# DearCaat/MHIM-MIL

Measured on AMD Instinct MI355X. Metric: patch-instances/sec through MHIM fwd+bwd, N=10k D=1024, higher is better.
Workload: dtype f32; 1 GPU; c2: MHIM(ABMIL) train step, one bag N=10000 D=1024 per GPU per step (teacher fwd + select + student fwd + bwd + Adam + EMA); rotating_bags_per_gpu=8, matrix_core_form=bf16x3, parallelism=dp1, launch=hipGraph replay, one graph per resident bag

## Files before the change

mhim_mil_amd/csrc/optim.hip:

```cpp
#include <math.h>
#include <stdlib.h>

#include "common.hpp"

namespace mhimx {

int reduce_flush(hipStream_t st, mhimx_reduce_list* list);

constexpr int HEAD_THREADS = 256;

MHIMX_DEV float blk_sum(float v, float* red) {
  v = wave_sum(v);
  __syncthreads();
  if ((threadIdx.x & 63) == 0) red[threadIdx.x >> 6] = v;
  __syncthreads();
  return red[0] + red[1] + red[2] + red[3];
}
MHIMX_DEV float blk_max(float v, float* red) {
  v = wave_max(v);
  __syncthreads();
  if ((threadIdx.x & 63) == 0) red[threadIdx.x >> 6] = v;
  __syncthreads();
  return fmaxf(fmaxf(red[0], red[1]), fmaxf(red[2], red[3]));
}

__global__ __launch_bounds__(HEAD_THREADS) void head_kernel(const float* __restrict__ z, const float* __restrict__ t,
                                                            const float* __restrict__ wp, const float* __restrict__ bp,
                                                            const int64_t* __restrict__ label, int E, int C, float temp_t,
                                                            float main_alpha, float aux_alpha, float inv_accum,
                                                            float* __restrict__ logits, float* __restrict__ losses,
                                                            float* __restrict__ g_z, float* __restrict__ d_wp,
                                                            float* __restrict__ d_bp, int accumulate,
                                                            const float* __restrict__ g_logits_in,
                                                            const float* __restrict__ g_cl_in) {
  __shared__ float red[4];
  __shared__ float lg[16], gl[16];
  const int tid = threadIdx.x;
  for (int c = 0; c < C; ++c) {
    float p = 0.f;
    for (int e = tid; e < E; e += HEAD_THREADS) p += wp[c * E + e] * z[e];
    p = blk_sum(p, red);
    if (tid == 0) lg[c] = p + (bp ? bp[c] : 0.f);
// ... 35 lines not shown
    losses[0] = main_alpha * ce + aux_alpha * cl;
    losses[1] = ce;
    losses[2] = cl;
  }
  for (int e = tid; e < E; e += HEAD_THREADS) {
    float g = 0.f;
    for (int c = 0; c < C; ++c) g += wp[c * E + e] * gl[c];
    if (aux) g += aux_alpha * inv_accum * (expf(z[e] - zmx) / zden - expf(t[e] / temp_t - tmx) / tden);
    g_z[e] = g;
    if (d_wp)
      for (int c = 0; c < C; ++c) {
        const float v = gl[c] * z[e];
        d_wp[c * E + e] = accumulate ? d_wp[c * E + e] + v : v;
      }
  }
  if (d_bp && tid < C) d_bp[tid] = accumulate ? d_bp[tid] + gl[tid] : gl[tid];
}

template <int Q>
__global__ __launch_bounds__(HEAD_THREADS) void head_fast_kernel(const float* __restrict__ z, const float* __restrict__ t,
                                                                 const float* __restrict__ wp, const float* __restrict__ bp,
                                                                 const int64_t* __restrict__ label, int E, int C, float temp_t,
                                                                 float main_alpha, float aux_alpha, float inv_accum,
                                                                 float* __restrict__ logits, float* __restrict__ losses,
                                                                 float* __restrict__ g_z, float* __restrict__ d_wp,
                                                                 float* __restrict__ d_bp, int accumulate,
                                                                 const float* __restrict__ g_logits_in,
                                                                 const float* __restrict__ g_cl_in, BagBatch bb) {
  __shared__ float red[8][4];
  if (blockIdx.z) {
    MHIMX_BAG(z); MHIMX_BAG(t); MHIMX_BAG(label); MHIMX_BAG(logits); MHIMX_BAG(losses); MHIMX_BAG(g_z); MHIMX_BAG(d_wp); MHIMX_BAG(d_bp);
    MHIMX_BAG(g_logits_in); MHIMX_BAG(g_cl_in);
  }
  const int tid = threadIdx.x, lane = tid & 63, wave = tid >> 6;
  const bool aux = (t != nullptr);
  float zv[Q], tv[Q], wv[4][Q], dw_old[4][Q];
#pragma unroll
  for (int q = 0; q < Q; ++q) {
    const int e = tid + q * HEAD_THREADS;
    const bool in = e < E;
    zv[q] = in ? z[e] : 0.f;
    tv[q] = (in && aux) ? t[e] : 0.f;
#pragma unroll
    for (int c = 0; c < 4; ++c) {
      wv[c][q] = (in && c < C) ? wp[c * E + e] : 0.f;
      dw_old[c][q] = (in && c < C && d_wp && accumulate) ? d_wp[c * E + e] : 0.f;
    }
  }
  const int y = label ? (int)label[0] : 0;
  float bpv[4], glin[4], dbp_old[4];
#pragma unroll
  for (int c = 0; c < 4; ++c) {
    bpv[c] = (bp && c < C) ? bp[c] : 0.f;
    glin[c] = (!label && g_logits_in && c < C) ? g_logits_in[c] : 0.f;
    dbp_old[c] = (d_bp && accumulate && c < C) ? d_bp[c] : 0.f;
  }
  if (g_cl_in) aux_alpha = g_cl_in[0];
  float p[4] = {0.f, 0.f, 0.f, 0.f}, a = -INFINITY, b = -INFINITY;
#pragma unroll
  for (int q = 0; q < Q; ++q) {
    const bool in = tid + q * HEAD_THREADS < E;
#pragma unroll
    for (int c = 0; c < 4; ++c) p[c] += wv[c][q] * zv[q];
    if (in) { a = fmaxf(a, zv[q]); b = fmaxf(b, tv[q] / temp_t); }
  }
#pragma unroll
  for (int c = 0; c < 4; ++c) p[c] = wave_sum(p[c]);
  a = wave_max(a);
  b = wave_max(b);
  if (lane == 0) {
#pragma unroll
    for (int c = 0; c < 4; ++c) red[c][wave] = p[c];
    red[4][wave] = a;
    red[5][wave] = b;
  }
  __syncthreads();
  float lg[4];
#pragma unroll
  for (int c = 0; c < 4; ++c) lg[c] = (red[c][0] + red[c][1] + red[c][2] + red[c][3]) + bpv[c];
  const float zmx = aux ? fmaxf(fmaxf(red[4][0], red[4][1]), fmaxf(red[4][2], red[4][3])) : 0.f;
  const float tmx = aux ? fmaxf(fmaxf(red[5][0], red[5][1]), fmaxf(red[5][2], red[5][3])) : 0.f;
  float ce = 0.f, gl[4] = {0.f, 0.f, 0.f, 0.f};
  if (label) {
    float mx = -INFINITY;
#pragma unroll
    for (int c = 0; c < 4; ++c) if (c < C) mx = fmaxf(mx, lg[c]);
    float den = 0.f;
#pragma unroll
    for (int c = 0; c < 4; ++c) if (c < C) den += expf(lg[c] - mx);
    float ly = lg[0];
#pragma unroll
    for (int c = 1; c < 4; ++c) if (c == y) ly = lg[c];
    ce = -(ly - mx - logf(den));
#pragma unroll
    for (int c = 0; c < 4; ++c) if (c < C) gl[c] = main_alpha * inv_accum * (expf(lg[c] - mx) / den - (c == y ? 1.f : 0.f));
  } else {
#pragma unroll
    for (int c = 0; c < 4; ++c) gl[c] = glin[c];
  }
  float cl = 0.f, zden = 1.f, tden = 1.f;
  float ez[Q], et[Q];
  if (aux) {
    float sa = 0.f, sb = 0.f;
#pragma unroll
    for (int q = 0; q < Q; ++q) {
      const bool in = tid + q * HEAD_THREADS < E;
      ez[q] = in ? expf(zv[q] - zmx) : 0.f;
      et[q] = in ? expf(tv[q] / temp_t - tmx) : 0.f;
      sa += ez[q];
      sb += et[q];
    }
    sa = wave_sum(sa);
    sb = wave_sum(sb);
    if (lane == 0) { red[6][wave] = sa; red[7][wave] = sb; }
    __syncthreads();
    zden = red[6][0] + red[6][1] + red[6][2] + red[6][3];
    tden = red[7][0] + red[7][1] + red[7][2] + red[7][3];
    const float lz = logf(zden);
    float acc = 0.f;
#pragma unroll
    for (int q = 0; q < Q; ++q)
      if (tid + q * HEAD_THREADS < E) acc += (et[q] / tden) * (zv[q] - zmx - lz);
    acc = wave_sum(acc);
    if (lane == 0) red[0][wave] = acc;
    __syncthreads();
    cl = -(red[0][0] + red[0][1] + red[0][2] + red[0][3]);
  }
  if (tid == 0) {
    for (int c = 0; c < C; ++c) logits[c] = lg[c];
    losses[0] = main_alpha * ce + aux_alpha * cl;
    losses[1] = ce;
    losses[2] = cl;
  }
#pragma unroll
  for (int q = 0; q < Q; ++q) {
    const int e = tid + q * HEAD_THREADS;
    if (e >= E) continue;
    float g = 0.f;
#pragma unroll
    for (int c = 0; c < 4; ++c) if (c < C) g += wv[c][q] * gl[c];
    if (aux) g += aux_alpha * inv_accum * (ez[q] / zden - et[q] / tden);
    g_z[e] = g;
    if (d_wp) {
#pragma unroll
      for (int c = 0; c < 4; ++c)
        if (c < C) {
          const float v = gl[c] * zv[q];
          d_wp[c * E + e] = accumulate ? dw_old[c][q] + v : v;
        }
    }
  }
  if (d_bp && tid < C) {
    float gv = gl[0], ov = dbp_old[0];
#pragma unroll
    for (int c = 1; c < 4; ++c) if (c == tid) { gv = gl[c]; ov = dbp_old[c]; }
    d_bp[tid] = accumulate ? ov + gv : gv;
  }
}

__global__ __launch_bounds__(HEAD_THREADS) void dsmil_head_kernel(const float* __restrict__ lb, const float* __restrict__ li,
                                                                  const int64_t* __restrict__ label, const float* __restrict__ Bs,
                                                                  const float* __restrict__ Bt, int C, int V, float temp_t,
                                                                  float main_alpha, float aux_alpha, float inv_accum,
                                                                  float* __restrict__ losses, float* __restrict__ g_lb,
                                                                  float* __restrict__ g_li, float* __restrict__ g_B,
                                                                  const float* __restrict__ g_cl_in) {
  __shared__ float red[4];
  const int tid = threadIdx.x;
  float ce = 0.f;
  if (label) {
    float mx = -INFINITY;
    for (int c = 0; c < C; ++c) mx = fmaxf(mx, 0.5f * (lb[c] + li[c]));
    float den = 0.f;
    for (int c = 0; c < C; ++c) den += expf(0.5f * (lb[c] + li[c]) - mx);
    const int y = (int)label[0];
    ce = -(0.5f * (lb[y] + li[y]) - mx - logf(den));
    if (tid < C) {
      const float g = 0.5f * main_alpha * inv_accum * (expf(0.5f * (lb[tid] + li[tid]) - mx) / den - (tid == y ? 1.f : 0.f));
      g_lb[tid] = g;
      g_li[tid] = g;
    }
  }
  if (g_cl_in) aux_alpha = g_cl_in[0];
  float cl = 0.f;
  if (Bt) {
    for (int c = 0; c < C; ++c) {
      const float* s = Bs + (int64_t)c * V;
      const float* t = Bt + (int64_t)c * V;
      float a = -INFINITY, b = -INFINITY;
      for (int e = tid; e < V; e += HEAD_THREADS) { a = fmaxf(a, s[e]); b = fmaxf(b, t[e] / temp_t); }
      const float smx = blk_max(a, red), tmx = blk_max(b, red);
      float sa = 0.f, sb = 0.f;
      for (int e = tid; e < V; e += HEAD_THREADS) { sa += expf(s[e] - smx); sb += expf(t[e] / temp_t - tmx); }
      const float sden = blk_sum(sa, red), tden = blk_sum(sb, red);
      const float ls = logf(sden);
      float acc = 0.f;
      for (int e = tid; e < V; e += HEAD_THREADS) {
        const float pt = expf(t[e] / temp_t - tmx) / tden;
        acc += pt * (s[e] - smx - ls);
        if (g_B) g_B[(int64_t)c * V + e] = aux_alpha * inv_accum / (float)C * (expf(s[e] - smx) / sden - pt);
      }
      cl -= blk_sum(acc, red) / (float)C;
    }
  } else if (g_B) {
    for (int i = tid; i < C * V; i += HEAD_THREADS) g_B[i] = 0.f;
  }
  if (tid == 0) {
    losses[0] = main_alpha * ce + aux_alpha * cl;
    losses[1] = ce;
    losses[2] = cl;
  }
}

constexpr int FOLD_MAX = 4;
struct FoldJobs { const float* parts[FOLD_MAX]; int64_t off[FOLD_MAX], n[FOLD_MAX]; int G[FOLD_MAX], accumulate[FOLD_MAX]; int count; };
struct OptimExtra { const float* lr_table; int64_t lr_len; const float* g_extra; int64_t n_extra, extra_pitch; float clip_norm;
                    const float* sq_parts; int n_parts; FoldJobs fold; int64_t extra_lo; int extra_only; };

MHIMX_DEV float4 fold_sum4(const float* __restrict__ parts, int64_t n, int64_t idx, int G) {
  float4 s0 = make_float4(0.f, 0.f, 0.f, 0.f), s1 = s0, s2 = s0, s3 = s0;
  auto ld = [&](int z) { return *reinterpret_cast<const float4*>(parts + (int64_t)z * n + idx); };
  auto add = [](float4& a, const float4& b) { a.x += b.x; a.y += b.y; a.z += b.z; a.w += b.w; };
  int z = 0;
  for (; z + 8 <= G; z += 8) {
    const float4 p0 = ld(z), p1 = ld(z + 1), p2 = ld(z + 2), p3 = ld(z + 3), p4 = ld(z + 4), p5 = ld(z + 5), p6 = ld(z + 6), p7 = ld(z + 7);
    add(s0, p0); add(s1, p1); add(s2, p2); add(s3, p3);
    add(s0, p4); add(s1, p5); add(s2, p6); add(s3, p7);
  }
  for (; z + 4 <= G; z += 4) { add(s0, ld(z)); add(s1, ld(z + 1)); add(s2, ld(z + 2)); add(s3, ld(z + 3)); }
  for (; z < G; ++z) add(s0, ld(z));
  return make_float4((s0.x + s1.x) + (s2.x + s3.x), (s0.y + s1.y) + (s2.y + s3.y), (s0.z + s1.z) + (s2.z + s3.z), (s0.w + s1.w) + (s2.w + s3.w));
}

__global__ __launch_bounds__(256) void grad_sumsq_kernel(const float* __restrict__ g, int64_t n, float gscale, OptimExtra ex, float* __restrict__ parts) {
  __shared__ float red[256];
  float a = 0.f;
  for (int64_t i = (int64_t)blockIdx.x * 256 + threadIdx.x; i < n; i += (int64_t)gridDim.x * 256) {
    const bool slabs = i >= ex.extra_lo;
    float v = (slabs && ex.extra_only) ? 0.f : g[i];
    if (slabs)
      for (int64_t z = 0; z < ex.n_extra; ++z) v += ex.g_extra[z * ex.extra_pitch + i];
    v *= gscale;
    a += v * v;
  }
  red[threadIdx.x] = a;
  __syncthreads();
  for (int o = 128; o > 0; o >>= 1) {
    if ((int)threadIdx.x < o) red[threadIdx.x] += red[threadIdx.x + o];
    __syncthreads();
  }
// ... 26 lines not shown
    }
  }
  if (threadIdx.x == 0) {
    int64_t step = step_host;
    if (step_dev) step = (int64_t)step_dev[0];
    if (ex.lr_table) {
      int64_t i = step - 1;
      i = i < 0 ? 0 : (i >= ex.lr_len ? ex.lr_len - 1 : i);
      lr = ex.lr_table[i];
    }
    if (step_dev || ex.lr_table) {
      const double t = (double)step;
      lr_over_bc1 = (float)((double)lr / (1.0 - exp(t * ln_beta1)));
      bc2s = (float)sqrt(1.0 - exp(t * ln_beta2));
    }
    float coef = 1.f;
    if (ex.clip_norm > 0.f) {
      coef = ex.clip_norm / (sqrtf(clip_red[0]) + 1e-6f);
      coef = coef > 1.f ? 1.f : coef;
    }
    sc[3] = coef;
    if (mm_table) {
      int64_t i = step - 1;
      i = i < 0 ? 0 : (i >= mm_len ? mm_len - 1 : i);
      mm = mm_table[i];
    }
    sc[0] = lr_over_bc1; sc[1] = bc2s; sc[2] = mm;
  }
  __syncthreads();
  lr_over_bc1 = sc[0];
  bc2s = sc[1];
  mm = sc[2];
  gscale *= sc[3];
  const int64_t n4 = n_all / 4;
  const bool vec_ok = ((reinterpret_cast<uintptr_t>(p) | reinterpret_cast<uintptr_t>(g) | reinterpret_cast<uintptr_t>(m) |
                        reinterpret_cast<uintptr_t>(v) | reinterpret_cast<uintptr_t>(teacher)) & 15) == 0;
  for (int64_t q = (int64_t)blockIdx.x * blockDim.x + threadIdx.x; q * 4 < n_all; q += (int64_t)gridDim.x * blockDim.x) {
    const int64_t i0 = q * 4;
    if (vec_ok && q < n4 && (i0 + 4 <= n_train || i0 >= n_train)) {
      float4 w = reinterpret_cast<float4*>(p)[q];
      if (i0 < n_train) {
        const bool slabs = i0 >= ex.extra_lo;
        float4 gi = (slabs && ex.extra_only) ? make_float4(0.f, 0.f, 0.f, 0.f) : reinterpret_cast<float4*>(g)[q];
        float4 mi = reinterpret_cast<float4*>(m)[q], vi = reinterpret_cast<float4*>(v)[q];
        for (int f = 0; f < ex.fold.count; ++f)
          if (i0 >= ex.fold.off[f] && i0 < ex.fold.off[f] + ex.fold.n[f]) {
            const float4 sv = fold_sum4(ex.fold.parts[f], ex.fold.n[f], i0 - ex.fold.off[f], ex.fold.G[f]);
            if (ex.fold.accumulate[f]) { gi.x += sv.x; gi.y += sv.y; gi.z += sv.z; gi.w += sv.w; }
            else gi = sv;
          }
        for (int64_t z = 0; slabs && z < ex.n_extra; ++z) {
          const float4 e = *reinterpret_cast<const float4*>(ex.g_extra + z * ex.extra_pitch + i0);
          gi.x += e.x; gi.y += e.y; gi.z += e.z; gi.w += e.w;
        }
        adam_one(w.x, gi.x, mi.x, vi.x, lr_over_bc1, bc2s, beta1, beta2, eps, wd, gscale);
        adam_one(w.y, gi.y, mi.y, vi.y, lr_over_bc1, bc2s, beta1, beta2, eps, wd, gscale);
        adam_one(w.z, gi.z, mi.z, vi.z, lr_over_bc1, bc2s, beta1, beta2, eps, wd, gscale);
        adam_one(w.w, gi.w, mi.w, vi.w, lr_over_bc1, bc2s, beta1, beta2, eps, wd, gscale);
        reinterpret_cast<float4*>(m)[q] = mi;
        reinterpret_cast<float4*>(v)[q] = vi;
        reinterpret_cast<float4*>(p)[q] = w;
        if (zero_grad) reinterpret_cast<float4*>(g)[q] = make_float4(0.f, 0.f, 0.f, 0.f);
      }
      if (teacher) {
        float4 t = reinterpret_cast<float4*>(teacher)[q];
        t.x = t.x * mm + w.x * (1.f - mm); t.y = t.y * mm + w.y * (1.f - mm);
        t.z = t.z * mm + w.z * (1.f - mm); t.w = t.w * mm + w.w * (1.f - mm);
        reinterpret_cast<float4*>(teacher)[q] = t;
      }
      continue;
    }
    for (int64_t i = i0; i < i0 + 4 && i < n_all; ++i) {
      float w = p[i];
      if (i < n_train) {
        const bool slabs = i >= ex.extra_lo;
        float gi = (slabs && ex.extra_only) ? 0.f : g[i], mi = m[i], vi = v[i];
        for (int64_t z = 0; slabs && z < ex.n_extra; ++z) gi += ex.g_extra[z * ex.extra_pitch + i];
        adam_one(w, gi, mi, vi, lr_over_bc1, bc2s, beta1, beta2, eps, wd, gscale);
        m[i] = mi;
        v[i] = vi;
        p[i] = w;
        if (zero_grad) g[i] = 0.f;
      }
      if (teacher) teacher[i] = teacher[i] * mm + w * (1.f - mm);
    }
  }
}

}

using namespace mhimx;

extern "C" int mhimx_head_fwd_bwd(void* stream, const float* z, const float* t, const float* wp, const float* bp,
                                  const int64_t* label_dev, int64_t E, int64_t C, float temp_t, float main_alpha,
                                  float aux_alpha, float inv_accum, float* logits, float* losses, float* g_z, float* d_wp,
                                  float* d_bp, int32_t accumulate, const float* g_logits_in, const float* g_cl_in) {
  MHIMX_CHECK_ARG(z && wp && logits && losses && g_z, "head: null args");
  MHIMX_CHECK_ARG(C > 0 && C <= 16 && E > 0, "head: bad dims");
  static const bool slow_head = getenv("MHIMX_HEAD_GENERIC") != nullptr;
  if (!slow_head && C <= 4 && E <= 2 * HEAD_THREADS)
    hipLaunchKernelGGL(head_fast_kernel<2>, bgrid(1), dim3(HEAD_THREADS), 0, (hipStream_t)stream, z, t, wp, bp, label_dev, (int)E, (int)C,
                     temp_t, main_alpha, aux_alpha, inv_accum, logits, losses, g_z, d_wp, d_bp, accumulate, g_logits_in, g_cl_in, cur_batch());
  else if (!slow_head && C <= 4 && E <= 4 * HEAD_THREADS)
    hipLaunchKernelGGL(head_fast_kernel<4>, bgrid(1), dim3(HEAD_THREADS), 0, (hipStream_t)stream, z, t, wp, bp, label_dev, (int)E, (int)C,
                     temp_t, main_alpha, aux_alpha, inv_accum, logits, losses, g_z, d_wp, d_bp, accumulate, g_logits_in, g_cl_in, cur_batch());
  else if (cur_batch().n > 0)
    return fail(-1, "head: a bag-batched launch takes the short-chain head (C <= 4, E <= 1024)");
  else
  hipLaunchKernelGGL(head_kernel, dim3(1), dim3(HEAD_THREADS), 0, (hipStream_t)stream, z, t, wp, bp, label_dev, (int)E, (int)C,
                     temp_t, main_alpha, aux_alpha, inv_accum, logits, losses, g_z, d_wp, d_bp, accumulate, g_logits_in, g_cl_in);
  MHIMX_LAUNCH_CHECK();
  return 0;
}

extern "C" int mhimx_dsmil_head(void* stream, const float* logits_bag, const float* logits_ins, const int64_t* label_dev,
                                const float* Bs, const float* Bt, int64_t C, int64_t V, float temp_t, float main_alpha,
                                float aux_alpha, float inv_accum, float* losses, float* g_logits_bag, float* g_logits_ins,
                                float* g_B, const float* g_cl_in) {
  MHIMX_CHECK_ARG(losses && Bs && C > 0 && C <= 16 && V > 0, "dsmil_head: bad args");
  MHIMX_CHECK_ARG(!label_dev || (logits_bag && logits_ins && g_logits_bag && g_logits_ins), "dsmil_head: label needs the logits and their gradients");
  hipLaunchKernelGGL(dsmil_head_kernel, dim3(1), dim3(HEAD_THREADS), 0, (hipStream_t)stream, logits_bag, logits_ins, label_dev, Bs, Bt,
                     (int)C, (int)V, temp_t, main_alpha, aux_alpha, inv_accum, losses, g_logits_bag, g_logits_ins, g_B, g_cl_in);
  MHIMX_LAUNCH_CHECK();
  return 0;
}

extern "C" int mhimx_optim_step(void* stream, const mhimx_optim_args* a) {
  MHIMX_CHECK_ARG(a, "optim_step: null args");
  MHIMX_CHECK_ARG(!a->mm_table || a->mm_len > 0, "optim_step: empty momentum schedule");
  MHIMX_CHECK_ARG(!a->lr_table || a->lr_len > 0, "optim_step: empty learning-rate schedule");
  MHIMX_CHECK_ARG(a->p && a->g && a->m && a->v && a->n_train >= 0 && a->n_all >= a->n_train && (a->step >= 1 || a->step_dev), "optim_step: bad args");
  MHIMX_CHECK_ARG(a->n_extra >= 0 && (a->n_extra == 0 || (a->g_extra && a->extra_pitch >= a->n_train && a->extra_pitch % 4 == 0 && aligned16(a->g_extra))),
                  "optim_step: gradient slabs need a 16-byte aligned base and a pitch >= n_train that is a multiple of 4");
  MHIMX_CHECK_ARG(!(a->clip_norm > 0.f) || (a->ws && a->ws_floats >= 1024), "optim_step: clipping needs a workspace of 1024 floats");
  MHIMX_CHECK_ARG(a->extra_lo >= 0 && a->extra_lo % 4 == 0 && (a->n_extra > 0 || (a->extra_lo == 0 && !a->extra_only)),
                  "optim_step: extra_lo (a multiple of 4) / extra_only describe the gradient slabs of g_extra");
  int64_t step = a->step < 1 ? 1 : a->step;
  if (a->n_all == 0) return 0;
  OptimExtra ex{a->lr_table, a->lr_len, a->g_extra, a->n_extra, a->extra_pitch, a->clip_norm > 0.f ? a->clip_norm : 0.f, a->ws, 0, {}, a->extra_lo, a->extra_only};
  if (a->fold) {
    mhimx_reduce_list* l = a->fold;
    MHIMX_CHECK_ARG(l->n >= 0 && l->n <= MHIMX_REDUCE_MAX, "optim_step: bad reduction list");
    const bool vec_ok = aligned16(a->p) && aligned16(a->g) && aligned16(a->m) && aligned16(a->v) && (!a->teacher || aligned16(a->teacher));
    if (!(a->clip_norm > 0.f) && vec_ok) {
      int kept = 0;
      for (int i = 0; i < l->n; ++i) {
        const mhimx_reduce_job& j = l->j[i];
        const int64_t n = j.K1 * j.K2, off = j.out - a->g;
        const bool take = j.kind == 1 && ex.fold.count < FOLD_MAX && j.G >= 1 && j.G <= 64 && j.ldo == j.K2 && n > 0 && n % 4 == 0 && aligned16(j.parts) &&
                          j.out >= a->g && off % 4 == 0 && off + n <= a->n_train / 4 * 4;
        if (take) {
          const int f = ex.fold.count++;
          ex.fold.parts[f] = j.parts; ex.fold.off[f] = off; ex.fold.n[f] = n; ex.fold.G[f] = (int)j.G; ex.fold.accumulate[f] = j.accumulate;
        } else {
          l->j[kept++] = j;
        }
      }
      l->n = kept;
    }
    if (l->n > 0 || l->side.pending || l->parked.pending)
      if (int r = reduce_flush((hipStream_t)stream, l)) return r;
  }
  if (ex.clip_norm > 0.f && a->n_train > 0) {
    const int64_t nb = cdiv(a->n_train, 1024) < 1024 ? cdiv(a->n_train, 1024) : 1024;
    ex.n_parts = (int)nb;
    hipLaunchKernelGGL(grad_sumsq_kernel, dim3((unsigned)nb), dim3(256), 0, (hipStream_t)stream, a->g, a->n_train, a->grad_scale, ex, a->ws);
    MHIMX_LAUNCH_CHECK();
  } else {
    ex.clip_norm = 0.f;
  }
  const double bc1 = 1.0 - pow((double)a->beta1, (double)step);
  const double bc2 = 1.0 - pow((double)a->beta2, (double)step);
  const int64_t blocks = cdiv(a->n_all, 1024) < 2048 ? cdiv(a->n_all, 1024) : 2048;
  hipLaunchKernelGGL(adam_ema_kernel, dim3((unsigned)blocks), dim3(256), 0, (hipStream_t)stream, a->p, a->g, a->m, a->v,
                     a->teacher, a->n_train, a->n_all, (float)((double)a->lr / bc1), (float)sqrt(bc2), a->beta1, a->beta2, a->eps, a->weight_decay,
                     a->grad_scale, a->ema_mm, a->zero_grad, a->step_dev, a->lr, a->mm_table, a->mm_len, step, log((double)a->beta1),
                     log((double)a->beta2), ex);
  MHIMX_LAUNCH_CHECK();
  return 0;
}

extern "C" int mhimx_adam_ema(void* stream, float* p, const float* g, float* m, float* v, float* teacher, int64_t n_train,
                              int64_t n_all, int64_t step, float lr, float beta1, float beta2, float eps, float weight_decay,
                              float grad_scale, float ema_mm, int32_t zero_grad, const uint64_t* step_dev,
                              const float* mm_table, int64_t mm_len) {
  mhimx_optim_args a{};
  a.p = p; a.g = const_cast<float*>(g); a.m = m; a.v = v; a.teacher = teacher; a.n_train = n_train; a.n_all = n_all; a.step = step;
  a.step_dev = step_dev; a.lr = lr; a.beta1 = beta1; a.beta2 = beta2; a.eps = eps; a.weight_decay = weight_decay; a.grad_scale = grad_scale;
  a.ema_mm = ema_mm; a.mm_table = mm_table; a.mm_len = mm_len; a.zero_grad = zero_grad;
  return mhimx_optim_step(stream, &a);
}

typedef float sc_f4 __attribute__((ext_vector_type(4)));
__global__ __launch_bounds__(256) void stream_copy_kernel(const sc_f4* __restrict__ src, sc_f4* __restrict__ dst, int64_t n4) {
  const int64_t stride = (int64_t)gridDim.x * 256;
  for (int64_t i = (int64_t)blockIdx.x * 256 + threadIdx.x; i < n4; i += stride) __builtin_nontemporal_store(__builtin_nontemporal_load(src + i), dst + i);
}
extern "C" int mhimx_stream_copy(void* stream, const float* src, float* dst, int64_t n_floats) {
  MHIMX_CHECK_ARG(src && dst && n_floats >= 0 && n_floats % 4 == 0 && aligned16(src) && aligned16(dst), "stream_copy: 16-byte aligned buffers, n % 4 == 0");
  if (n_floats == 0) return 0;
  const int64_t n4 = n_floats / 4;
  const int64_t blocks = cdiv(n4, 256) < (1 << 20) ? cdiv(n4, 256) : (1 << 20);
  hipLaunchKernelGGL(stream_copy_kernel, dim3((unsigned)blocks), dim3(256), 0, (hipStream_t)stream, reinterpret_cast<const sc_f4*>(src),
                     reinterpret_cast<sc_f4*>(dst), n4);
  MHIMX_LAUNCH_CHECK();
  return 0;
}

__global__ void tick_kernel(uint64_t* c) { c[0] += 1; }
extern "C" int mhimx_tick(void* stream, uint64_t* counter) {
  MHIMX_CHECK_ARG(counter, "tick: null counter");
  hipLaunchKernelGGL(tick_kernel, dim3(1), dim3(1), 0, (hipStream_t)stream, counter);
  MHIMX_LAUNCH_CHECK();
  return 0;
// ... 2 lines not shown
```

mhim_mil_amd/csrc/prep_jobs.hpp:

```cpp
#pragma once
#include "mma_tile.hpp"
#include "mca2_prep.hpp"

namespace mhimx {

typedef float pj_f4 __attribute__((ext_vector_type(4)));
typedef __bf16 pj_b8 __attribute__((ext_vector_type(8)));
MHIMX_DEV void pj_split(const float (&x)[8], pj_b8& hi, pj_b8& lo) {
#pragma unroll
  for (int i = 0; i < 8; ++i) {
    const __bf16 h = (__bf16)x[i];
    hi[i] = h;
    lo[i] = (__bf16)(x[i] - (float)h);
  }
}
MHIMX_DEV void pj_split2(const pj_f4& a, const pj_f4& b, pj_b8& hi, pj_b8& lo) {
  const float x[8] = {a[0], a[1], a[2], a[3], b[0], b[1], b[2], b[3]};
  pj_split(x, hi, lo);
}

constexpr int PREP_MERGE_MAX = 8;
struct PrepJobs { mhimx_prep_job j[MHIMX_PREP_MAX]; int first[MHIMX_PREP_MAX + 1]; int n; Merge2PrepArgs m2; int64_t m2_shift[PREP_MERGE_MAX]; };
constexpr int PREP_LDS_FLOATS = 6 * M2_E + 6 * 64;
static_assert(PREP_LDS_FLOATS >= 32 * 33, "the transpose tile fits the job LDS");

MHIMX_DEV void prep_job_block(const PrepJobs& pj, int block, float* lds) {
  int q = 0;
  while (q + 1 < pj.n && block >= pj.first[q + 1]) ++q;
  const mhimx_prep_job jb = pj.j[q];
  const int bid = block - pj.first[q], nblk = pj.first[q + 1] - pj.first[q];
  const int64_t R = jb.R, C = jb.C;
  if (jb.kind == 0) {
    float (*tile)[33] = reinterpret_cast<float(*)[33]>(lds);
    const int tx = threadIdx.x & 31, ty = threadIdx.x >> 5;
    const int64_t tiles_c = (C + 31) / 32, ntiles = ((R + 31) / 32) * tiles_c;
    for (int64_t t = bid; t < ntiles; t += nblk) {
      const int64_t r0 = (t / tiles_c) * 32, c0 = (t % tiles_c) * 32;
      for (int i = ty; i < 32; i += 8) {
        const int64_t r = r0 + i, c = c0 + tx;
        tile[i][tx] = (r < R && c < C) ? jb.in[r * C + c] : 0.f;
      }
      __syncthreads();
      for (int i = ty; i < 32; i += 8) {
        const int64_t c = c0 + i, r = r0 + tx;
        if (r < R && c < C) jb.out[c * R + r] = tile[tx][i];
      }
      __syncthreads();
    }
  } else if (jb.kind == 1) {
    const int64_t K8 = C / 8, n = R * K8;
    for (int64_t i = (int64_t)bid * 256 + threadIdx.x; i < n; i += (int64_t)nblk * 256) {
// ... 106 lines not shown
```

mhim_mil_amd/csrc/rows.hip:

```cpp
#include <math.h>
#include <string.h>

#include "mca2_rows.hpp"
#include "reduce_jobs.hpp"

namespace mhimx {

int gemm_nt(hipStream_t st, const mhimx_gemm_nt_args& g);
int gemm_tn(hipStream_t st, const mhimx_gemm_tn_args& g);
bool scorer_fused_ok(int64_t E, int64_t A, int gated, int prec, const float* T, const float* wa, const float* wp, int64_t C);
int scorer_fused_fwd(hipStream_t st, const float* T, int64_t M, const float* wa, const float* wa_frag, const float* ba, int act, const float* wc,
                     const float* bc, const float* wp, int C, float* u_pre, float* s_out, float* cproj, float* pm, float* pl,
                     float* pz, int max_parts, const int64_t* rows, const uint8_t* excl, const mhimx_prep_job* ride_jobs, int n_ride_jobs,
                     const void* merge_rows);
int merge2_fwd_rows_args(const mhimx_merge* m, const float* X, int64_t R, void* ws, int64_t ws_bytes, M2RowsFwd* out);
int prep_batch(hipStream_t st, const mhimx_prep_job* jobs, int n);
int scorer_fused_bwd(hipStream_t st, const float* T, int64_t M, const float* u_pre, const float* s_in, const float* stats,
                     const float* g_z, const float* z, const float* wc, int act, const float* wa_t, const float* wa_t_frag, float* du,
                     float* dT, float* dwc_part, float* dbc_part, int max_parts, const int64_t* rows, const void* pre_side, int64_t gate_row0,
                     void* img, const void* img_dact, float* img_part, int64_t img_rows);

constexpr int ROWS_THREADS = 256;
constexpr int MAX_PART = 512;
constexpr int TN_SLABS = 128;

MHIMX_DEV float sigmoidf_(float x) { return 1.f / (1.f + __expf(-x)); }

constexpr int FWD_WAVES = 16;
template <int EPL>
__global__ __launch_bounds__(64 * FWD_WAVES) void score_rows_fwd_kernel(
    const float* __restrict__ T, int64_t M, int E, int A, int act, int gated, const float* __restrict__ u_pre,
    const float* __restrict__ wc, const float* __restrict__ bc, const float* __restrict__ wp, int C,
    float* __restrict__ s_out, float* __restrict__ cproj, float* __restrict__ pm, float* __restrict__ pl,
    float* __restrict__ pz, float gdrop_p, uint64_t gdrop_seed, int64_t row0 ) {
  extern __shared__ __attribute__((aligned(16))) float sm[];
  constexpr int NWV = FWD_WAVES;
  const int lane = threadIdx.x & 63, wave = threadIdx.x >> 6;
  const int ldu = A * (1 + gated);
  const float bias_c = bc ? bc[0] : 0.f;

  float mw = -INFINITY, lw = 0.f, zacc[EPL];
#pragma unroll
  for (int q = 0; q < EPL; ++q) zacc[q] = 0.f;

  for (int64_t n = (int64_t)blockIdx.x * NWV + wave; n < M; n += (int64_t)gridDim.x * NWV) {
    const float* up = u_pre + n * ldu;
    float part = 0.f;
    const bool gdrop = gated && gdrop_p > 0.f;
    const uint32_t rkey = gdrop ? drop_row_key(gdrop_seed, (uint64_t)(row0 + n)) : 0u;
    const float ginv = gdrop ? 1.f / (1.f - gdrop_p) : 1.f;
    for (int j = lane; j < A; j += 64) {
      float u = act_fwd(up[j], act);
      if (gated) {
// ... 32 lines not shown
      lw += p;
#pragma unroll
      for (int q = 0; q < EPL; ++q) zacc[q] += p * hv[q];
    }
  }
  float* zs = sm;
  float* ms = sm + NWV * E;
  float* ls = ms + NWV;
#pragma unroll
  for (int q = 0; q < EPL; ++q) zs[wave * E + lane + 64 * q] = zacc[q];
  if (lane == 0) { ms[wave] = mw; ls[wave] = lw; }
  __syncthreads();
  float mb = ms[0];
#pragma unroll
  for (int i = 1; i < NWV; ++i) mb = fmaxf(mb, ms[i]);
  float w[NWV];
#pragma unroll
  for (int i = 0; i < NWV; ++i) w[i] = (ms[i] == -INFINITY) ? 0.f : __expf(ms[i] - mb);
  for (int e = threadIdx.x; e < E; e += 64 * NWV) {
    float a = 0.f;
#pragma unroll
    for (int i = 0; i < NWV; ++i) a += zs[i * E + e] * w[i];
    pz[(int64_t)blockIdx.x * E + e] = a;
  }
  if (threadIdx.x == 0) {
    float l = 0.f;
#pragma unroll
    for (int i = 0; i < NWV; ++i) l += ls[i] * w[i];
    pm[blockIdx.x] = mb;
    pl[blockIdx.x] = l;
  }
}

constexpr int FIN_THREADS = 1024;
__global__ __launch_bounds__(FIN_THREADS) void pool_finalize_kernel(const float* __restrict__ pm, const float* __restrict__ pl,
                                                                     const float* __restrict__ pz, int G, int E,
                                                                     float* __restrict__ stats, float* __restrict__ z,
                                                                     const float* __restrict__ s, const float* __restrict__ cproj,
                                                                     const float* __restrict__ bp, int C, int64_t M1,
                                                                     float* __restrict__ pscore, BagBatch bb) {
  __shared__ float red[16];
  __shared__ float wgt[2 * MAX_PART];
  __shared__ float acc16[16][64];
  if (blockIdx.z) {
    MHIMX_BAG(pm); MHIMX_BAG(pl); MHIMX_BAG(pz); MHIMX_BAG(stats); MHIMX_BAG(z); MHIMX_BAG(s); MHIMX_BAG(cproj); MHIMX_BAG(pscore);
  }
  const int lane = threadIdx.x & 63, wave = threadIdx.x >> 6;
  const int b1 = threadIdx.x;
  const float pm1 = b1 < G ? pm[b1] : -INFINITY, pl1 = b1 < G ? pl[b1] : 0.f;
  float m = wave_max(pm1);
  if (lane == 0) red[wave] = m;
  __syncthreads();
  float mx = red[0];
#pragma unroll
  for (int w = 1; w < 16; ++w) mx = fmaxf(mx, red[w]);
  __syncthreads();
  float lp = 0.f;
  if (b1 < G) {
    const float w = (pm1 == -INFINITY) ? 0.f : __expf(pm1 - mx);
    wgt[b1] = w;
    lp = pl1 * w;
  }
  lp = wave_sum(lp);
  if (lane == 0) red[wave] = lp;
  __syncthreads();
  float L = 0.f;
#pragma unroll
  for (int w = 0; w < 16; ++w) L += red[w];
  const int zblocks = (E + 63) / 64;
  if ((int)blockIdx.x >= zblocks) {
    const float invL = 1.f / L, b0 = bp ? bp[0] : 0.f;
    const int nb = (int)gridDim.x - zblocks;
    for (int64_t n = (int64_t)((int)blockIdx.x - zblocks) * FIN_THREADS + threadIdx.x; n < M1; n += (int64_t)nb * FIN_THREADS) {
      const float an = __expf(s[n] - mx) * invL;
      float cm = -INFINITY;
      for (int c = 0; c < C; ++c) cm = fmaxf(cm, an * cproj[n * C + c] + b0);
      float den = 0.f;
      for (int c = 0; c < C; ++c) den += expf((an * cproj[n * C + c] + b0) - cm);
      pscore[n] = 1.f / den;
    }
    return;
  }
  const int e = blockIdx.x * 64 + lane;
  float acc = 0.f;
  if (e < E) {
#pragma unroll 8
    for (int b = wave; b < G; b += 16) acc += pz[(int64_t)b * E + e] * wgt[b];
  }
  acc16[wave][lane] = acc;
  __syncthreads();
  if (wave == 0 && e < E) {
    float a = 0.f;
#pragma unroll
    for (int w = 0; w < 16; ++w) a += acc16[w][lane];
    z[e] = a / L;
  }
  if (blockIdx.x == 0 && threadIdx.x == 0) { stats[0] = mx; stats[1] = L; }
}

constexpr int FIN_MAXTOK = 6;
#ifdef MHIMX_FT_PROF
__device__ unsigned long long ft_prof[16];
#define FT_STAMP(i) do { __syncthreads(); if (threadIdx.x == 0 && blockIdx.x == 0) ft_prof[i] = wall_clock64(); } while (0)
#else
#define FT_STAMP(i)
#endif
__global__ __launch_bounds__(FIN_THREADS) void pool_finalize_tok_kernel(const float* __restrict__ pm, const float* __restrict__ pl,
                                                                         const float* __restrict__ pz, int G, int E, float* __restrict__ stats,
                                                                         float* __restrict__ z, const float* __restrict__ T,
                                                                         const int64_t* __restrict__ rows_tail, int64_t row0, int K,
                                                                         const float* __restrict__ wa, const float* __restrict__ wa_t,
                                                                         const float* __restrict__ ba, const float* __restrict__ wc,
                                                                         const float* __restrict__ bc, int A, int act,
                                                                         float* __restrict__ u_pre_tail, float* __restrict__ s_tail, BagBatch bb) {
  if (blockIdx.z) {
    MHIMX_BAG(pm); MHIMX_BAG(pl); MHIMX_BAG(pz); MHIMX_BAG(stats); MHIMX_BAG(z); MHIMX_BAG(T); MHIMX_BAG(rows_tail); MHIMX_BAG(wa_t); MHIMX_BAG(u_pre_tail);
    MHIMX_BAG(s_tail);
  }
  __shared__ float red[16];
  __shared__ float wgt[2 * MAX_PART];
  __shared__ float acc16[16][64];
  __shared__ __attribute__((aligned(16))) float tks[FIN_MAXTOK][512];
  __shared__ float up[8][FIN_MAXTOK][128];
  __shared__ float us[FIN_MAXTOK][128];
  __shared__ float stok[8];
  const int tid = threadIdx.x, lane = tid & 63, wave = tid >> 6;
  FT_STAMP(0);
  const float pm1 = tid < G ? pm[tid] : -INFINITY, pl1 = tid < G ? pl[tid] : 0.f;
  const int e = blockIdx.x * 64 + lane;
  float pzv[8];
// ... 642 lines not shown
  const int64_t G = 2 * MAX_PART;
  PoolWs t;
  t.pm = ar.take<float>(G);
  t.pl = ar.take<float>(G);
  t.pz = ar.take<float>(G * E);
  t.attn = ar.take<float>(M);
  t.du = ar.take<float>(M * A * (1 + gated));
  t.dwc_part = ar.take<float>(G * A);
  t.dbc_part = ar.take<float>(G);
  t.u_pre = ar.take<float>(M * A * (1 + gated));
  t.tn_ws = ar.take<float>((int64_t)TN_SLABS * A * E);
  t.nt_ws = ar.take<float>(4 * M * A);
  if (w) *w = t;
  return ar.off;
}

template <typename F>
static int dispatch_epl(int64_t E, F&& f) {
  switch (E) {
    case 256: return f(std::integral_constant<int, 4>());
    case 512: return f(std::integral_constant<int, 8>());
    case 1024: return f(std::integral_constant<int, 16>());
    default: return fail(-1, "token width E=%lld unsupported (256, 512 or 1024)", (long long)E);
  }
}

static int check_scorer(const mhimx_scorer* sc) {
  MHIMX_CHECK_ARG(sc && sc->wa && sc->wc, "scorer: null weights");
  MHIMX_CHECK_ARG(sc->A > 0 && sc->A <= 512 && sc->A % 4 == 0, "scorer: A must be a multiple of 4, <= 512");
  MHIMX_CHECK_ARG(!sc->gated || sc->wb, "scorer: gated needs wb");
  return 0;
}

int abmil_pool_fwd(hipStream_t st, const mhimx_scorer* sc, mhimx_pool_io* io) {
  if (int r = check_scorer(sc)) return r;
  MHIMX_CHECK_ARG(io && io->T1 && io->M1 > 0 && io->s && io->stats && io->z, "pool_fwd: null io");
  MHIMX_CHECK_ARG(io->M2 == 0 || io->T2, "pool_fwd: M2>0 needs T2");
  MHIMX_CHECK_ARG(!io->cproj || (io->wp && io->C > 0), "pool_fwd: cproj needs wp, C");
  MHIMX_CHECK_ARG(!io->rows1 || (io->M2 == 0 && scorer_fused_ok(sc->E, sc->A, sc->gated, sc->prec, io->T1, sc->wa, io->cproj ? io->wp : nullptr, io->C)),
                  "pool_fwd: gathered tokens (rows1) need the one-pass scorer (E = 512, A = 128, plain form, not f32) and a single segment");
  MHIMX_CHECK_ARG(!io->excl || scorer_fused_ok(sc->E, sc->A, sc->gated, sc->prec, io->T1, sc->wa, io->cproj ? io->wp : nullptr, io->C),
                  "pool_fwd: excluded rows (excl) need the one-pass scorer (E = 512, A = 128, plain form, not f32)");
  const int64_t M = io->M1 + io->M2, E = sc->E, A = sc->A;
  const int gated = sc->gated ? 1 : 0;
  Arena ar(io->ws, io->ws_bytes);
  PoolWs w;
  pool_ws_layout(ar, M, E, A, gated, &w);
  MHIMX_CHECK_ARG(ar.ok(), "pool_fwd: workspace too small (%lld < %lld)", (long long)io->ws_bytes, (long long)ar.off);
  float* u_pre = io->u_pre ? io->u_pre : w.u_pre;
  const int64_t ldu = A * (1 + gated);
  if (io->phase != 0) {
    const int64_t K = io->tail_tokens, Ms1 = io->M1 - K;
    MHIMX_CHECK_ARG((io->phase == 1 || io->phase == 2) && K >= 1 && K <= FIN_MAXTOK && Ms1 >= 1 && io->M2 == 0 && !io->cproj && !io->pscore && !io->excl &&
                        E == 512 && A == 128 && scorer_fused_ok(E, A, gated, sc->prec, io->T1, sc->wa, nullptr, 0),
                    "pool_fwd: the two-call forward takes the one-pass scorer shapes, one segment, 1..%d tail tokens, no class projections", FIN_MAXTOK);
    const int tiles = (int)cdiv(Ms1, 32);
    const int G1 = tiles < MAX_PART ? tiles : MAX_PART;
    if (io->phase == 1) {
      M2RowsFwd mfbuf;
      const void* mf = nullptr;
      io->rode_merge = 0;
      static const bool ride_ok = getenv("MHIMX_MERGE_FWD_RIDE") == nullptr || atoi(getenv("MHIMX_MERGE_FWD_RIDE")) != 0;
      if (io->ride_merge && ride_ok) {
        const int rc = merge2_fwd_rows_args(reinterpret_cast<const mhimx_merge*>(io->ride_merge), io->ride_X, io->ride_R, io->ride_ws, io->ride_ws_bytes,
                                            &mfbuf);
        if (rc < 0) return rc;
        if (rc == 0) { mf = &mfbuf; io->rode_merge = 1; }
      }
      const int g1 = scorer_fused_fwd(st, io->T1, Ms1, sc->wa, sc->wa_frag, sc->ba, sc->act, sc->wc, sc->bc, nullptr, 0, u_pre, io->s, nullptr, w.pm, w.pl,
                                      w.pz, MAX_PART, io->rows1, nullptr, io->ride_jobs, io->n_ride_jobs, mf);
      return g1 < 0 ? g1 : 0;
    }
    hipLaunchKernelGGL(pool_finalize_tok_kernel, bgrid((unsigned)cdiv(E, 64)), dim3(FIN_THREADS), 0, st, w.pm, w.pl, w.pz, G1, (int)E, io->stats, io->z, io->T1,
                       (io->rows1 && io->tail_row0 < 0) ? io->rows1 + Ms1 : nullptr, io->rows1 ? io->tail_row0 : Ms1, (int)K, sc->wa, io->tail_wa_t, sc->ba, sc->wc,
                       sc->bc, (int)A, sc->act, u_pre + Ms1 * ldu, io->s + Ms1, cur_batch());
    MHIMX_LAUNCH_CHECK();
    return 0;
  }

  const float* Ts[2] = {io->T1, io->T2};
  const int64_t Ms[2] = {io->M1, io->M2};
  int64_t off = 0;
  int G = 0;
  bool rode = false;
  for (int seg = 0; seg < 2; ++seg) {
    if (Ms[seg] == 0) continue;
    if (scorer_fused_ok(E, A, gated, sc->prec, Ts[seg], sc->wa, io->cproj ? io->wp : nullptr, io->C)) {
      const int g1 = scorer_fused_fwd(st, Ts[seg], Ms[seg], sc->wa, sc->wa_frag, sc->ba, sc->act, sc->wc, sc->bc, io->cproj ? io->wp : nullptr,
                                      (int)io->C, io->no_backward ? nullptr : u_pre + off * ldu, io->s + off, io->cproj ? io->cproj + off * io->C : nullptr,
                                      w.pm + G, w.pl + G, w.pz + (int64_t)G * E, MAX_PART, seg == 0 ? io->rows1 : nullptr,
                                      seg == 0 ? io->excl : nullptr, rode ? nullptr : io->ride_jobs, rode ? 0 : io->n_ride_jobs, nullptr);
      if (g1 < 0) return g1;
      rode = true;
      G += g1;
      off += Ms[seg];
      continue;
    }
    MHIMX_CHECK_ARG(cur_batch().n == 0, "pool_fwd: a bag-batched launch needs the one-pass scorer");
    mhimx_gemm_nt_args g = {};
    g.A = Ts[seg]; g.lda = E; g.B = sc->wa; g.ldb = E; g.C = u_pre + off * ldu; g.ldc = ldu;
    g.M = Ms[seg]; g.N = A; g.K = E; g.bias = sc->ba;
    g.ws = w.nt_ws; g.ws_floats = 4 * M * A;
    g.prec = sc->prec == MHIMX_PREC_F32 ? MHIMX_PREC_F32 : MHIMX_PREC_BF16X3;
    if (int r = gemm_nt(st, g)) return r;
    if (gated) {
      g.B = sc->wb; g.bias = sc->bb; g.C = u_pre + off * ldu + A;
      if (int r = gemm_nt(st, g)) return r;
    }
    int grid = (int)cdiv(Ms[seg], 5 * FWD_WAVES);
    if (grid < 1) grid = 1;
    if (grid > MAX_PART) grid = MAX_PART;
    const float* Tseg = Ts[seg];
    const int64_t Mseg = Ms[seg];
    int r = dispatch_epl(E, [&](auto epl) {
      constexpr int EPL = decltype(epl)::value;
      const size_t smem = (size_t)(FWD_WAVES * E + 2 * FWD_WAVES) * sizeof(float);
      if (smem > 48 * 1024)
        MHIMX_ONCE_PER_DEVICE(MHIMX_HIP(hipFuncSetAttribute((const void*)score_rows_fwd_kernel<EPL>, hipFuncAttributeMaxDynamicSharedMemorySize, (int)smem)));
      hipLaunchKernelGGL(score_rows_fwd_kernel<EPL>, dim3(grid), dim3(64 * FWD_WAVES), smem, st, Tseg, Mseg, (int)E, (int)A,
                         sc->act, gated, u_pre + off * ldu, sc->wc, sc->bc, io->cproj ? io->wp : nullptr, (int)io->C,
                         io->s + off, io->cproj ? io->cproj + off * io->C : nullptr, w.pm + G, w.pl + G,
                         w.pz + (int64_t)G * E, sc->gate_drop_p, sc->gate_drop_seed, off);
      MHIMX_LAUNCH_CHECK();
      return 0;
    });
    if (r) return r;
    G += grid;
    off += Ms[seg];
  }
  if (!rode && io->ride_jobs && io->n_ride_jobs > 0)
    if (int r = prep_batch(st, io->ride_jobs, io->n_ride_jobs)) return r;
  MHIMX_CHECK_ARG(!io->pscore || io->cproj, "pool_fwd: pscore needs cproj (and wp)");
  static_assert(2 * MAX_PART <= FIN_THREADS, "pool_finalize_kernel reads one partial per thread");
  const int64_t ps_blocks = io->pscore ? (cdiv(io->M1, FIN_THREADS) < 64 ? cdiv(io->M1, FIN_THREADS) : 64) : 0;
  hipLaunchKernelGGL(pool_finalize_kernel, bgrid((unsigned)(cdiv(E, 64) + ps_blocks)), dim3(FIN_THREADS), 0, st, w.pm, w.pl, w.pz, G, (int)E, io->stats,
                     io->z, io->s, io->cproj, io->bp, (int)io->C, io->M1, io->pscore, cur_batch());
  MHIMX_LAUNCH_CHECK();
  return 0;
}

int abmil_pool_bwd(hipStream_t st, const mhimx_scorer* sc, const mhimx_pool_io* io, const mhimx_pool_grad* gr) {
  if (int r = check_scorer(sc)) return r;
  MHIMX_CHECK_ARG(io && gr && gr->g_z && gr->dT1 && gr->d_wa && gr->d_wc && gr->wa_t, "pool_bwd: null args");
  MHIMX_CHECK_ARG(io->M2 == 0 || gr->dT2, "pool_bwd: M2>0 needs dT2");
  const int64_t M = io->M1 + io->M2, E = sc->E, A = sc->A;
  const int gated = sc->gated ? 1 : 0;
  MHIMX_CHECK_ARG(!gated || (gr->d_wb && gr->wb_t), "pool_bwd: gated needs d_wb, wb_t");
  Arena ar(io->ws, io->ws_bytes);
  PoolWs w;
  pool_ws_layout(ar, M, E, A, gated, &w);
  MHIMX_CHECK_ARG(ar.ok(), "pool_bwd: workspace too small");
  const float* u_pre = io->u_pre ? io->u_pre : w.u_pre;
  const int64_t ldu = A * (1 + gated);
  const float* Ts[2] = {io->T1, io->T2};
  float* dTs[2] = {gr->dT1, gr->dT2};
  const int64_t Ms[2] = {io->M1, io->M2};

  int64_t off = 0;
  int G = 0;
  const bool fused = scorer_fused_ok(E, A, gated, sc->prec, io->T1, gr->wa_t, nullptr, 0) && aligned16(gr->dT1) &&
                     (io->M2 == 0 || (aligned16(io->T2) && aligned16(gr->dT2))) && aligned16(u_pre) && aligned16(w.du);
  MHIMX_CHECK_ARG(!io->rows1 || (fused && io->M2 == 0), "pool_bwd: gathered tokens (rows1) need the one-pass backward and a single segment");
  MHIMX_CHECK_ARG(!gr->img || (fused && io->M2 == 0 && E == 512), "pool_bwd: the dPRE image (img) needs the one-pass backward and a single segment");
  MHIMX_CHECK_ARG(cur_batch().n == 0 || (fused && io->M2 == 0 && !gated && gr->defer && !gr->d_bc && !gr->d_ba && !gr->d_bb),
                  "pool_bwd: a bag-batched launch needs the one-pass backward with its reductions queued");
  for (int seg = 0; seg < 2 && fused; ++seg) {
    if (Ms[seg] == 0) continue;
    const void* pre_side = nullptr;
    int64_t gate_row0 = -1;
    if (seg == 0 && io->M2 == 0 && gr->defer && gr->defer->pre.pending == 1) {
      Merge2Side psd;
      memcpy(&psd, gr->defer->pre.blob, sizeof(psd));
      const int64_t d = psd.dz - dTs[0];
      if (psd.dz >= dTs[0] && d % E == 0) {
        pre_side = gr->defer->pre.blob;
        gate_row0 = d / E;
        gr->defer->pre.pending = 2;
      }
    }
    const int g1 = scorer_fused_bwd(st, Ts[seg], Ms[seg], u_pre + off * ldu, io->s + off, io->stats, gr->g_z, io->z, sc->wc, sc->act,
                                    gr->wa_t, gr->wa_t_frag, w.du + off * ldu, dTs[seg], w.dwc_part + (int64_t)G * A, w.dbc_part + G,
                                    MAX_PART, seg == 0 ? io->rows1 : nullptr, pre_side, gate_row0, seg == 0 ? gr->img : nullptr, gr->img_dact, gr->img_part,
                                    gr->img_rows);
    if (g1 < 0) return g1;
    G += g1;
    off += Ms[seg];
  }
  for (int seg = 0; seg < 2 && !fused; ++seg) {
    if (Ms[seg] == 0) continue;
    const int grid = grid_for_rows(Ms[seg]);
    const float* Tseg = Ts[seg];
    const int64_t Mseg = Ms[seg];
    int r = dispatch_epl(E, [&](auto epl) {
      constexpr int EPL = decltype(epl)::value;
      const size_t smem = (size_t)(4 * A + 8) * sizeof(float);
      hipLaunchKernelGGL(score_rows_bwd_kernel<EPL>, dim3(grid), dim3(ROWS_THREADS), smem, st, Tseg, Mseg, (int)E, (int)A,
                         sc->act, gated, u_pre + off * ldu, sc->wc, io->s + off, io->stats, gr->g_z, io->z,
                         w.du + off * ldu, w.attn + off, w.dwc_part + (int64_t)G * A, w.dbc_part + G, sc->gate_drop_p,
                         sc->gate_drop_seed, off);
      MHIMX_LAUNCH_CHECK();
      return 0;
    });
    if (r) return r;
    G += grid;
    off += Ms[seg];
  }
  if (!defer_push(gr->defer, reduce_job_parts(w.dwc_part, G, A, A, gr->d_wc, gr->accumulate)))
    hipLaunchKernelGGL(reduce_parts_kernel, dim3((unsigned)cdiv(A, 32)), dim3(RP_THREADS), 0, st, w.dwc_part, G, (int)A, (int)A, gr->d_wc, gr->accumulate);
  MHIMX_LAUNCH_CHECK();
  if (gr->d_bc) {
    if (!defer_push(gr->defer, reduce_job_parts(w.dbc_part, G, 1, 1, gr->d_bc, gr->accumulate)))
      hipLaunchKernelGGL(reduce_parts_kernel, dim3(1), dim3(RP_THREADS), 0, st, w.dbc_part, G, 1, 1, gr->d_bc, gr->accumulate);
    MHIMX_LAUNCH_CHECK();
  }
  off = 0;
  for (int seg = 0; seg < 2; ++seg) {
// ... 154 lines not shown
  MHIMX_LAUNCH_CHECK();
  return 0;
}

int colsum(hipStream_t st, const float* X, int64_t M, int64_t E, float* out, int accumulate, void* ws, int64_t ws_bytes) {
  MHIMX_CHECK_ARG(X && out && E > 0 && M >= 0, "colsum: bad args");
  const int64_t nrows = M > 0 ? M : 1, avail = ws ? ws_bytes / (E * 4) : 0;
  int64_t want = cdiv(nrows, 16) < 512 ? cdiv(nrows, 16) : 512;
  MHIMX_CHECK_ARG(avail >= (want < 128 ? want : 128), "colsum: workspace too small (need %lld bytes)", (long long)((want < 128 ? want : 128) * E * 4));
  if (want > avail) want = avail;
  const int64_t chunk = cdiv(M > 0 ? M : 1, want);
  const int gy = (int)cdiv(M > 0 ? M : 1, chunk);
  hipLaunchKernelGGL(colsum_part_kernel, dim3((unsigned)cdiv(E, 128), gy), dim3(128), 0, st, X, M, (int)E, chunk, (float*)ws);
  MHIMX_LAUNCH_CHECK();
  hipLaunchKernelGGL(reduce_parts_kernel, dim3((unsigned)cdiv(E, 32)), dim3(RP_THREADS), 0, st, (const float*)ws, gy, (int)E, (int)E, out, accumulate);
  MHIMX_LAUNCH_CHECK();
  return 0;
}

}

using namespace mhimx;

extern "C" int64_t mhimx_abmil_pool_ws_bytes(int64_t M, int64_t E, int64_t A, int32_t gated) {
  Arena ar(nullptr, 0);
  return pool_ws_layout(ar, M, E, A, gated ? 1 : 0, nullptr);
}
extern "C" int mhimx_abmil_pool_fwd(void* stream, const mhimx_scorer* sc, mhimx_pool_io* io) {
  return abmil_pool_fwd((hipStream_t)stream, sc, io);
}
extern "C" int mhimx_abmil_pool_bwd(void* stream, const mhimx_scorer* sc, const mhimx_pool_io* io, const mhimx_pool_grad* g) {
  return abmil_pool_bwd((hipStream_t)stream, sc, io, g);
}
extern "C" int mhimx_softmax_from_stats(void* stream, const float* s, const float* stats, float* attn, int64_t M) {
  if (M <= 0) return 0;
  hipLaunchKernelGGL(softmax_from_stats_kernel, bgrid((unsigned)(cdiv(M, 256) < 1024 ? cdiv(M, 256) : 1024)), dim3(256), 0,
                     (hipStream_t)stream, s, stats, attn, M, cur_batch());
  MHIMX_LAUNCH_CHECK();
  return 0;
}
extern "C" int mhimx_lse_merge(void* stream, const float* parts, int64_t W, int64_t E, float* stats, float* z) {
  MHIMX_CHECK_ARG(parts && stats && z && W >= 1 && E >= 1, "lse_merge: bad args");
  hipLaunchKernelGGL(lse_merge_kernel, dim3((unsigned)cdiv(E, 256)), dim3(256), 0, (hipStream_t)stream, parts, (int)W, (int)E, stats, z);
  MHIMX_LAUNCH_CHECK();
  return 0;
}
extern "C" int mhimx_pseudo_score(void* stream, const float* s, const float* stats, const float* cproj, const float* bp,
                                  float* score, float* attn_out, int64_t M, int64_t C) {
  MHIMX_CHECK_ARG((!s || stats) && cproj && score && C > 0, "pseudo_score: null args");
  if (M <= 0) return 0;
  hipLaunchKernelGGL(pseudo_score_kernel, dim3((unsigned)(cdiv(M, 256) < 1024 ? cdiv(M, 256) : 1024)), dim3(256), 0,
                     (hipStream_t)stream, s, stats, cproj, bp, score, attn_out, M, (int)C);
  MHIMX_LAUNCH_CHECK();
  return 0;
}
extern "C" int mhimx_act_bwd(void* stream, float* dH, const float* H, const float* pre, int64_t M, int64_t E, int32_t act,
                             float drop_p, uint64_t drop_seed, const uint8_t* drop_mask, const int64_t* rows, float* colsum_out,
                             int32_t accumulate, void* ws, int64_t ws_bytes, const uint64_t* drop_tick) {
  MHIMX_CHECK_ARG(dH && (H || pre), "act_bwd: null args");
  MHIMX_CHECK_ARG(act == MHIMX_ACT_NONE || act == MHIMX_ACT_RELU || pre, "act_bwd: gelu/tanh need the pre-activation");
  if (M <= 0) return 0;
  int64_t nblk = cdiv(M, 16);
  if (nblk > 1024) nblk = 1024;
  const int64_t chunk = cdiv(M, nblk);
  nblk = cdiv(M, chunk);
  MHIMX_CHECK_ARG(!colsum_out || (ws && ws_bytes >= nblk * E * 4), "act_bwd: workspace too small for the column sums (%lld bytes)",
// ... 133 lines not shown
```

mhim_mil_amd/csrc/scorer_fused.hip:

```cpp
#include <math.h>

#include "common.hpp"
#include "mca2_rows.hpp"
#include "prep_jobs.hpp"

namespace mhimx {

typedef float sf_f32x16 __attribute__((ext_vector_type(16)));
typedef float sf_f4 __attribute__((ext_vector_type(4)));
typedef __bf16 sf_b8 __attribute__((ext_vector_type(8)));

#ifdef MHIMX_SF_PROF
__device__ unsigned long long sf_prof[16];
#define SF_STAMP(i) do { __syncthreads(); if (threadIdx.x == 0 && blockIdx.x == 7) sf_prof[i] = wall_clock64(); } while (0)
#else
#define SF_STAMP(i)
#endif

constexpr int SF_ROWS = 32, SF_E = 512, SF_A = 128, SF_LD = SF_E + 4, SF_THREADS = 256;
constexpr int SF_MAXC = 4;
constexpr size_t SF_SMEM = (size_t)(SF_ROWS * SF_LD + 4 * SF_ROWS + 2 * SF_ROWS + SF_MAXC * SF_E + 2 * SF_ROWS) * sizeof(float);

MHIMX_DEV void sf_split(const sf_f4& a, const sf_f4& b, sf_b8& hi, sf_b8& lo) {
  const float x[8] = {a[0], a[1], a[2], a[3], b[0], b[1], b[2], b[3]};
#pragma unroll
  for (int i = 0; i < 8; ++i) {
    const __bf16 h = (__bf16)x[i];
    hi[i] = h;
    lo[i] = (__bf16)(x[i] - (float)h);
  }
}

MHIMX_DEV float sf_sum32(float v) {
  v += dpp_mov<0xB1, 0xf>(0.f, v);
  v += dpp_mov<0x4E, 0xf>(0.f, v);
// ... 220 lines not shown
        for (int q = 0; q < 16; ++q) {
          const sf_f4 hv = hr[8 * q], ww = w[8 * q];
          d += hv[0] * ww[0] + hv[1] * ww[1] + hv[2] * ww[2] + hv[3] * ww[3];
        }
        d += dpp_mov<0xB1, 0xf>(0.f, d);
        d += dpp_mov<0x4E, 0xf>(0.f, d);
        d += dpp_mov<0x141, 0xf>(0.f, d);
        if (seg == 0 && n < M) cproj[n * C + c] = d;
      }
    }
    __syncthreads();
    SF_STAMP(5);
  }
  if (tid == 0) { pm[bid] = m_run; pl[bid] = l_run; }
  pz[(int64_t)bid * SF_E + tid] = z0;
  pz[(int64_t)bid * SF_E + tid + SF_THREADS] = z1;
}

constexpr int SB_LD = SF_A + 4;
constexpr size_t SB_SMEM = (size_t)(SF_ROWS * SB_LD + SF_E + 3 * SF_ROWS + 2 * SF_A + 8 + 2 * SF_ROWS) * sizeof(float);
constexpr int SB_DLD = 1040;
constexpr size_t SB_SMEM_IMG = SB_SMEM + (size_t)SF_ROWS * SB_DLD;
MHIMX_DEV void sb_swap(float& a, float& b) { asm("s_nop 1\n\tv_permlane32_swap_b32 %0, %1" : "+v"(a), "+v"(b)); }

__global__ __launch_bounds__(SF_THREADS, 2) void scorer_fused_bwd_kernel(
    const float* __restrict__ T, int64_t M, const float* __restrict__ u_pre, const float* __restrict__ s_in,
    const float* __restrict__ stats, const float* __restrict__ g_z, const float* __restrict__ z, const float* __restrict__ wc, int act,
    const float* __restrict__ wat, const float* __restrict__ wat_frag, float* __restrict__ du, float* __restrict__ dT,
    float* __restrict__ dwc_part, float* __restrict__ dbc_part, int tiles,
    const int64_t* __restrict__ rows ,
    int n_main , Merge2Side pre,
    int64_t gate_row0 ,
    char* __restrict__ img ,
    const _Float16* __restrict__ dact, float* __restrict__ img_part, int64_t img_rows, BagBatch bb) {
  extern __shared__ __attribute__((aligned(16))) float sb_sm[];
  if (blockIdx.z) {
    MHIMX_BAG(T); MHIMX_BAG(u_pre); MHIMX_BAG(s_in); MHIMX_BAG(stats); MHIMX_BAG(g_z); MHIMX_BAG(z); MHIMX_BAG(du); MHIMX_BAG(dT); MHIMX_BAG(dwc_part);
    MHIMX_BAG(dbc_part); MHIMX_BAG(rows); MHIMX_BAG(wat); MHIMX_BAG(wat_frag); MHIMX_BAG(img); MHIMX_BAG(dact); MHIMX_BAG(img_part);
    bag_move(pre, bb);
  }
  if ((int)blockIdx.x >= n_main) {
    merge2_bwd_pre_body((int)blockIdx.x - n_main, sb_sm, pre.dz, pre.wo_t, pre.wkv, pre.k, pre.drop_p, pre.oseed, pre.tick, pre.d_bo, pre.accumulate,
                        pre.w, pre.rep, pre.w.gate + 1, (unsigned)pre.k);
    return;
  }
  const bool gated = gate_row0 >= 0;
  float* Ds = sb_sm;
  float* gzs = Ds + SF_ROWS * SB_LD;
  float* an_s = gzs + SF_E;
  float* gs_s = an_s + SF_ROWS;
  float* red = gs_s + SF_ROWS;
  float* dwc_s = red + SF_ROWS;
  int64_t* ridx = reinterpret_cast<int64_t*>(dwc_s + 2 * SF_A + 8);
  char* dact_s = reinterpret_cast<char*>(sb_sm) + SB_SMEM;
  const int tid = threadIdx.x, lane = tid & 63, wave = tid >> 6;
  const int r32 = lane & 31, kg = lane >> 5;
  float c0p = 0.f;
  for (int e = tid; e < SF_E; e += SF_THREADS) {
    const float g = g_z[e];
    gzs[e] = g;
    c0p += g * z[e];
  }
  c0p = wave_sum(c0p);
  if (lane == 0) red[wave] = c0p;
  __syncthreads();
  const float c0 = (red[0] + red[1]) + (red[2] + red[3]);
  const float mx = stats[0], invL = 1.f / stats[1];
  const int a_col = tid & (SF_A - 1), half = tid >> 7;
  const float wca = wc[a_col];
  float dwc_run = 0.f, dbc_run = 0.f;

  for (int tile = blockIdx.x; tile < tiles; tile += n_main) {
    const int64_t row0 = (int64_t)tile * SF_ROWS;
    if (rows) {
      if (tid < SF_ROWS) { const int64_t n = row0 + tid; ridx[tid] = rows[n < M ? n : M - 1]; }
      __syncthreads();
    }
    if (img) {
#pragma unroll
      for (int q = 0; q < SF_ROWS / 4; ++q) {
        const int r = wave + 4 * q;
        const int64_t n = row0 + r;
        const int64_t src = rows ? ridx[r] : (n < M ? n : M - 1);
        __builtin_amdgcn_global_load_lds((gptr_f)(reinterpret_cast<const char*>(dact + src * SF_E) + lane * 16), (lptr_f)(dact_s + r * SB_DLD), 16, 0, 0);
      }
    }
    float up[SF_ROWS / 2];
    {
      const int r = tid >> 3, seg = tid & 7;
      const int64_t n = row0 + r;
      const int64_t nc = n < M ? n : M - 1;
      const sf_f4* tr = reinterpret_cast<const sf_f4*>(T + (rows ? ridx[r] : nc) * SF_E) + seg;
      const sf_f4* gr = reinterpret_cast<const sf_f4*>(gzs) + seg;
      sf_f4 tv[16];
#pragma unroll
      for (int q = 0; q < 16; ++q) tv[q] = tr[8 * q];
#pragma unroll
      for (int k = 0; k < SF_ROWS / 2; ++k) {
        const int64_t nu = row0 + half + 2 * k;
// ... 191 lines not shown
  MHIMX_ONCE_PER_DEVICE(MHIMX_HIP(hipFuncSetAttribute((const void*)scorer_fused_kernel<true>, hipFuncAttributeMaxDynamicSharedMemorySize, (int)SF_SMEM)));
  MHIMX_ONCE_PER_DEVICE(MHIMX_HIP(hipFuncSetAttribute((const void*)scorer_fused_kernel<false>, hipFuncAttributeMaxDynamicSharedMemorySize, (int)SF_SMEM)));
  const int tiles = (int)cdiv(M, SF_ROWS);
  const int grid = tiles < max_parts ? tiles : max_parts;
  static_assert(SF_SMEM >= PREP_LDS_FLOATS * sizeof(float), "the riders' LDS is the scorer's");
  static_assert(SF_SMEM >= m2_fwd_smem(16), "the Merge row tiles' LDS is the scorer's");
  static_assert(SF_THREADS == 256 && SF_THREADS == M2_THREADS, "the preparation jobs and the Merge row tiles are written for 256 threads");
  PrepJobs rider = {};
  int ride_blocks = 0;
  MHIMX_CHECK_ARG(!(ride_jobs && n_ride_jobs > 0 && cur_batch().n > 0), "scorer: preparation jobs do not ride in a bag-batched launch");
  if (ride_jobs && n_ride_jobs > 0) {
    ride_blocks = prep_jobs_fill(ride_jobs, n_ride_jobs, &rider);
    if (ride_blocks < 0) return ride_blocks;
  }
  M2RowsFwd mf = {};
  int n_front = 0;
  if (merge_rows) {
    mf = *reinterpret_cast<const M2RowsFwd*>(merge_rows);
    n_front = mf.w.T;
  }
  if (wa_frag)
    hipLaunchKernelGGL(scorer_fused_kernel<true>, bgrid(n_front + grid + ride_blocks), dim3(SF_THREADS), SF_SMEM, st, T, M, wa, wa_frag, ba, act, wc, bc, wp, C, u_pre,
                       s_out, cproj, pm, pl, pz, tiles, rows, excl, grid, rider, n_front, mf, cur_batch());
  else
    hipLaunchKernelGGL(scorer_fused_kernel<false>, bgrid(n_front + grid + ride_blocks), dim3(SF_THREADS), SF_SMEM, st, T, M, wa, wa_frag, ba, act, wc, bc, wp, C, u_pre,
                       s_out, cproj, pm, pl, pz, tiles, rows, excl, grid, rider, n_front, mf, cur_batch());
  MHIMX_LAUNCH_CHECK();
  return grid;
}

int scorer_fused_bwd(hipStream_t st, const float* T, int64_t M, const float* u_pre, const float* s_in, const float* stats,
                     const float* g_z, const float* z, const float* wc, int act, const float* wa_t, const float* wa_t_frag, float* du,
                     float* dT, float* dwc_part, float* dbc_part, int max_parts, const int64_t* rows, const void* pre_side, int64_t gate_row0,
                     void* img, const void* img_dact, float* img_part, int64_t img_rows) {
    MHIMX_ONCE_PER_DEVICE(MHIMX_HIP(hipFuncSetAttribute((const void*)scorer_fused_bwd_kernel, hipFuncAttributeMaxDynamicSharedMemorySize, (int)SB_SMEM_IMG)));
  MHIMX_CHECK_ARG(!img || (img_dact && aligned16(img) && aligned16(img_dact) && img_rows >= 0 && img_rows <= M),
                  "scorer backward: the dPRE image needs the d out / d pre rows, 16-byte aligned buffers and img_rows <= M");
  const int tiles = (int)cdiv(M, SF_ROWS);
  const int grid = tiles < max_parts ? tiles : max_parts;
  static_assert(SB_SMEM >= M2_BWD_PRE_LDS * sizeof(float), "the riding Merge stage's LDS is the backward's");
  static_assert(SF_THREADS == M2_THREADS, "the riding Merge stage is written for 256 threads");
  Merge2Side pre = {};
  int ride = 0;
  if (pre_side) {
    pre = *reinterpret_cast<const Merge2Side*>(pre_side);
    ride = M2_BWD_PRE_BLOCKS;
  } else {
    gate_row0 = -1;
  }
  hipLaunchKernelGGL(scorer_fused_bwd_kernel, bgrid(grid + ride), dim3(SF_THREADS), img ? SB_SMEM_IMG : SB_SMEM, st, T, M, u_pre, s_in, stats, g_z, z, wc, act, wa_t,
                     wa_t_frag, du, dT, dwc_part, dbc_part, tiles, rows, grid, pre, gate_row0, (char*)img, (const _Float16*)img_dact, img_part, img_rows, cur_batch());
  MHIMX_LAUNCH_CHECK();
  return grid;
}

}
```

mhim_mil_amd/csrc/select.hip:

```cpp
#include "common.hpp"

namespace mhimx {

#ifdef MHIMX_SEL_PROF
__device__ unsigned long long sel_prof[32];
#define SEL_STAMP(i) do { __syncthreads(); if (threadIdx.x == 0) sel_prof[i] = wall_clock64(); } while (0)
#else
#define SEL_STAMP(i)
#endif

constexpr int SEL_THREADS = 1024;
constexpr int SEL_WAVES = SEL_THREADS / 64;

MHIMX_DEV uint32_t mono32(float f, bool largest) {
  uint32_t b = __float_as_uint(f);
  b = (b & 0x80000000u) ? ~b : (b | 0x80000000u);
  return largest ? b : ~b;
}

MHIMX_DEV uint32_t block_prefix(bool pred, uint32_t* wave_tot , uint32_t* total) {
  const int lane = threadIdx.x & 63, wave = threadIdx.x >> 6;
  const unsigned long long bal = __ballot(pred);
  const uint32_t in_wave = __popcll(bal & ((1ull << lane) - 1ull));
  if (lane == 0) wave_tot[wave] = __popcll(bal);
  __syncthreads();
  uint32_t base = 0, tot = 0;
#pragma unroll
  for (int w = 0; w < SEL_WAVES; ++w) {
    const uint32_t c = wave_tot[w];
    if (w < wave) base += c;
    tot += c;
  }
  __syncthreads();
// ... 293 lines not shown
    if (shift == 0) break;
    if (n_eq <= (uint32_t)SEL_LIST) {
      if (tid == 0) misc[4] = 0;
      __syncthreads();
#pragma unroll
      for (int j = 0; j < KPT; ++j)
        if (valid[j] && (key[j] & fixed_mask) == prefix) hist[atomicAdd(&misc[4], 1u)] = key[j];
      __syncthreads();
      for (uint32_t j = tid; j < n_eq; j += SEL_THREADS) {
        const uint32_t mine = hist[j];
        uint32_t g = 0, e = 0;
        for (uint32_t q = 0; q < n_eq; ++q) {
          const uint32_t o = hist[q];
          g += o > mine ? 1u : 0u;
          e += o == mine ? 1u : 0u;
        }
        if (g < remaining && remaining <= g + e) { misc[5] = mine; misc[6] = remaining - g; misc[7] = e; }
      }
      __syncthreads();
      prefix = misc[5];
      remaining = misc[6];
      n_eq = misc[7];
      break;
    }
    __syncthreads();
    shift = shift - SEL_DIGIT < 0 ? 0 : shift - SEL_DIGIT;
  }
  __syncthreads();
  *remaining_out = remaining;
  *n_eq_out = n_eq;
  return prefix;
}

template <int KPT, bool LEAN = false>
__global__ __launch_bounds__(SEL_THREADS) void select_small_kernel(
    const float* __restrict__ score, int N, int k, int n_sel, int largest, const int64_t* __restrict__ perm,
    const int64_t* __restrict__ other, int64_t n_other, int64_t* __restrict__ mask_ids, int64_t* __restrict__ len_keep_dev,
    int64_t* __restrict__ topk_out, int P, int use_rand, uint64_t rand_seed0, const uint64_t* __restrict__ tick, int merge_R,
    int64_t* __restrict__ rows_out,
    int64_t* __restrict__ rows_img ,
    int img_off, BagBatch bb ) {
  extern __shared__ __attribute__((aligned(16))) char smem_raw[];
  if (blockIdx.z) {
    MHIMX_BAG(score); MHIMX_BAG(perm); MHIMX_BAG(other); MHIMX_BAG(mask_ids); MHIMX_BAG(len_keep_dev); MHIMX_BAG(topk_out); MHIMX_BAG(rows_out);
    MHIMX_BAG(rows_img);
    rand_seed0 = bag_sel_seed(rand_seed0, bb);
  }
  const uint64_t rand_seed = eff_seed(rand_seed0, tick);
  uint64_t* keys = reinterpret_cast<uint64_t*>(smem_raw);
  uint64_t* sorted = keys + P;
  uint32_t* hist = reinterpret_cast<uint32_t*>(sorted + P);
  uint32_t* wave_tot = hist + SEL_COPIES * SEL_BINS;
  uint32_t* misc = wave_tot + SEL_WAVES;
  uint32_t* bitmap = misc + 8;
  uint32_t* rank = bitmap + 512;
  uint16_t* klist = reinterpret_cast<uint16_t*>(rank + P);
  uint16_t* stage = reinterpret_cast<uint16_t*>(smem_raw);
  const int tid = threadIdx.x;
  const bool lg = largest != 0;
  const int i0 = tid * KPT;

  SEL_STAMP(8);
  uint32_t key[KPT];
  bool valid[KPT];
#pragma unroll
  for (int j = 0; j < KPT; ++j) {
    valid[j] = (i0 + j) < N;
    key[j] = valid[j] ? mono32(score[i0 + j], lg) : 0u;
  }
  SEL_STAMP(0);
  for (int i = tid; i < 512; i += SEL_THREADS) bitmap[i] = 0;
  if (tid == 0) misc[2] = 0;

  uint32_t remaining, n_eq;
  const uint32_t T = radix_select_regs<KPT, false>(key, valid, (uint32_t)k, hist, wave_tot, misc, &remaining, &n_eq);

  SEL_STAMP(1);
  uint32_t eq_rank = 0;
  if (remaining != n_eq) {
    uint32_t neq = 0;
#pragma unroll
    for (int j = 0; j < KPT; ++j) neq += (valid[j] && key[j] == T) ? 1u : 0u;
    uint32_t tot;
    eq_rank = block_scan_excl(neq, wave_tot, &tot);
  }
  bool take[KPT];
  uint32_t ntake = 0;
#pragma unroll
  for (int j = 0; j < KPT; ++j) {
    bool t = valid[j] && key[j] > T;
    if (valid[j] && key[j] == T) { t = remaining == n_eq || eq_rank < remaining; ++eq_rank; }
    take[j] = t;
    ntake += t ? 1u : 0u;
  }
  {
    uint32_t tot;
    uint32_t pos = block_scan_excl(ntake, wave_tot, &tot);
#pragma unroll
    for (int j = 0; j < KPT; ++j)
      if (take[j]) keys[pos++] = ((uint64_t)key[j] << 32) | (uint64_t)(0xFFFFFFFFu - (uint32_t)(i0 + j));
  }
// ... 412 lines not shown
  hipLaunchKernelGGL(selm_hist_kernel<2>, dim3(G), dim3(SEL_THREADS), 0, st, score, N, largest, k, w);
  hipLaunchKernelGGL(selm_count_kernel, dim3(G), dim3(SEL_THREADS), 0, st, score, N, largest, k, chunk, w);
  hipLaunchKernelGGL(selm_gather_kernel, dim3(G), dim3(SEL_THREADS), 0, st, score, N, largest, chunk, w);
  (void)P;
  hipLaunchKernelGGL(selm_rank_kernel, dim3((unsigned)cdiv(k, SEL_THREADS), (unsigned)cdiv(k, SELM_SEG)), dim3(SEL_THREADS), 0, st, k, n_sel, perm, w);
  hipLaunchKernelGGL(selm_finish_kernel, dim3((unsigned)(cdiv(k, SEL_THREADS) < 16 ? 16 : cdiv(k, SEL_THREADS))), dim3(SEL_THREADS), 0, st, k, n_sel, N,
                     other, n_other, mask_ids, topk_sorted, w);
  hipLaunchKernelGGL(selm_keepcount_kernel, dim3(G), dim3(SEL_THREADS), 0, st, N, chunk, w);
  hipLaunchKernelGGL(selm_compact_kernel, dim3(G), dim3(SEL_THREADS), 0, st, N, chunk, (other != nullptr && n_other > 0) ? 1 : 0, mask_ids,
                     len_keep_dev, w);
  MHIMX_LAUNCH_CHECK();
  return 0;
}

static int select_impl(void* stream, const float* score, int64_t N, int64_t k, int64_t n_sel, int32_t largest,
                       const int64_t* perm, const int64_t* other, int64_t n_other, int64_t* mask_ids,
                       int64_t* len_keep_dev, int64_t* topk_sorted, void* ws, int64_t ws_bytes, int g_use_rand,
                       uint64_t g_rand_seed, const uint64_t* g_tick, int g_merge_R, int64_t* g_rows_out, int64_t* g_rows_img = nullptr,
                       int g_img_off = 0) {
  MHIMX_CHECK_ARG(score && (mask_ids || g_rows_out) && ws, "select_mask: null args");
  MHIMX_CHECK_ARG(!g_rows_img || (g_rows_out && N <= 16384 && next_pow2((int)k < 2 ? 2 : (int)k) <= 4096),
                  "select_rows_img: the image-order list comes from the one-workgroup select (N <= 16384, k <= 4096)");
  MHIMX_CHECK_ARG(!g_rows_out || N <= 16384, "select_rows: fused row list needs N <= 16384 (use select_mask + compose_ids)");
  MHIMX_CHECK_ARG(N > 0 && N <= (1ll << 24), "select_mask: N out of range");
  MHIMX_CHECK_ARG(k >= 1 && k <= N && k <= 16384, "select_mask: k=%lld out of range (1..min(N,16384))", (long long)k);
  MHIMX_CHECK_ARG(n_sel >= 0 && n_sel <= k, "select_mask: n_sel out of range");
  MHIMX_CHECK_ARG(ws_bytes >= N, "select_mask: workspace too small");
  const int P = next_pow2((int)k < 2 ? 2 : (int)k);
  if (N <= 16384 && P <= 4096) {
    const size_t sm = select_small_smem(P);
#define MHIMX_SEL_SMALL(KPT)                                                                                                   \
    hipLaunchKernelGGL(select_small_kernel<KPT>, bgrid(1), dim3(SEL_THREADS), sm, (hipStream_t)stream, score, (int)N, (int)k,   \
                       (int)n_sel, largest, perm, other, n_other, mask_ids, len_keep_dev, topk_sorted, P, g_use_rand,          \
                       g_rand_seed, g_tick, g_merge_R, g_rows_out, g_rows_img, g_img_off, cur_batch())
    MHIMX_ONCE_PER_DEVICE(
        MHIMX_HIP(hipFuncSetAttribute((const void*)select_small_kernel<16>, hipFuncAttributeMaxDynamicSharedMemorySize, (int)select_small_smem(4096)));
        MHIMX_HIP(hipFuncSetAttribute((const void*)select_small_kernel<10>, hipFuncAttributeMaxDynamicSharedMemorySize, (int)select_small_smem(4096)));
        MHIMX_HIP(hipFuncSetAttribute((const void*)select_small_kernel<4>, hipFuncAttributeMaxDynamicSharedMemorySize, (int)select_small_smem(4096))));
    const bool lean = g_use_rand && g_rows_out && !perm && !other && !mask_ids && !len_keep_dev && !topk_sorted && n_sel < k;
    if (lean) {
#define MHIMX_SEL_LEAN(KPT)                                                                                                    \
      hipLaunchKernelGGL((select_small_kernel<KPT, true>), bgrid(1), dim3(SEL_THREADS), sm, (hipStream_t)stream, score, (int)N, (int)k,   \
                         (int)n_sel, largest, perm, other, n_other, mask_ids, len_keep_dev, topk_sorted, P, g_use_rand,        \
                         g_rand_seed, g_tick, g_merge_R, g_rows_out, g_rows_img, g_img_off, cur_batch())
      MHIMX_ONCE_PER_DEVICE(
          MHIMX_HIP(hipFuncSetAttribute((const void*)select_small_kernel<16, true>, hipFuncAttributeMaxDynamicSharedMemorySize, (int)select_small_smem(4096)));
          MHIMX_HIP(hipFuncSetAttribute((const void*)select_small_kernel<10, true>, hipFuncAttributeMaxDynamicSharedMemorySize, (int)select_small_smem(4096)));
          MHIMX_HIP(hipFuncSetAttribute((const void*)select_small_kernel<4, true>, hipFuncAttributeMaxDynamicSharedMemorySize, (int)select_small_smem(4096))));
      if (N <= 4096) MHIMX_SEL_LEAN(4);
      else if (N <= 10240) MHIMX_SEL_LEAN(10);
      else MHIMX_SEL_LEAN(16);
#undef MHIMX_SEL_LEAN
    } else if (N <= 4096) MHIMX_SEL_SMALL(4);
    else if (N <= 10240) MHIMX_SEL_SMALL(10);
    else MHIMX_SEL_SMALL(16);
#undef MHIMX_SEL_SMALL
    MHIMX_LAUNCH_CHECK();
    return 0;
  }
  MHIMX_CHECK_ARG(cur_batch().n == 0, "select: a bag-batched launch takes the one-workgroup select (N <= 16384, k <= 4096)");
  const size_t smem = select_smem(P);
    MHIMX_ONCE_PER_DEVICE(MHIMX_HIP(hipFuncSetAttribute((const void*)select_kernel<false>, hipFuncAttributeMaxDynamicSharedMemorySize, (int)select_smem(16384))); MHIMX_HIP(hipFuncSetAttribute((const void*)select_kernel<true>, hipFuncAttributeMaxDynamicSharedMemorySize, (int)select_smem(16384))));
  MHIMX_CHECK_ARG(!g_use_rand && !g_rows_out, "select: the random-subset forms need N <= 16384 and k <= 4096");
  if (N > 16384 && ws_bytes >= mhimx_select_ws_bytes(N) && mask_ids)
    return select_multi((hipStream_t)stream, score, N, (int)k, (int)n_sel, largest, perm, other, n_other, mask_ids, len_keep_dev, topk_sorted, ws, P);
  hipLaunchKernelGGL(select_kernel<false>, dim3(1), dim3(SEL_THREADS), smem, (hipStream_t)stream, score, N, (int)k, (int)n_sel,
                     largest, perm, other, n_other, mask_ids, len_keep_dev, topk_sorted, (uint8_t*)ws, (float*)nullptr, P);
  MHIMX_LAUNCH_CHECK();
  return 0;
}

extern "C" int mhimx_select_mask(void* stream, const float* score, int64_t N, int64_t k, int64_t n_sel, int32_t largest,
                                 const int64_t* perm, const int64_t* other, int64_t n_other, int64_t* mask_ids,
                                 int64_t* len_keep_dev, int64_t* topk_sorted, void* ws, int64_t ws_bytes) {
  return select_impl(stream, score, N, k, n_sel, largest, perm, other, n_other, mask_ids, len_keep_dev, topk_sorted, ws, ws_bytes,
                     0, 0, nullptr, 0, nullptr);
}

extern "C" int mhimx_select_rows(void* stream, const float* score, int64_t N, int64_t k, int64_t n_sel, int32_t largest,
                                 uint64_t rand_seed, const uint64_t* tick, int64_t merge_R, int64_t* rows_out, int64_t* mask_ids,
                                 void* ws, int64_t ws_bytes, int32_t merge_first) {
  MHIMX_CHECK_ARG(rows_out && merge_R >= 0 && merge_R <= N - n_sel, "select_rows: bad args");
  return select_impl(stream, score, N, k, n_sel, largest, nullptr, nullptr, 0, mask_ids, nullptr, nullptr, ws, ws_bytes,
                     merge_first ? 2 : 1, rand_seed, tick, (int)merge_R, rows_out);
}

extern "C" int mhimx_select_rows_img(void* stream, const float* score, int64_t N, int64_t k, int64_t n_sel, int32_t largest, uint64_t rand_seed,
                                     const uint64_t* tick, int64_t merge_R, int64_t* rows_out, int64_t* rows_img, int64_t img_merge_off, void* ws,
                                     int64_t ws_bytes, int32_t merge_first) {
  MHIMX_CHECK_ARG(rows_out && rows_img && merge_R >= 0 && merge_R <= N - n_sel && img_merge_off >= N - n_sel - merge_R && img_merge_off % 32 == 0 &&
                      img_merge_off <= 32768,
                  "select_rows_img: bad args (the merged rows' image position is a multiple of 32 behind the rows that stay)");
  return select_impl(stream, score, N, k, n_sel, largest, nullptr, nullptr, 0, nullptr, nullptr, nullptr, ws, ws_bytes, merge_first ? 2 : 1, rand_seed, tick,
                     (int)merge_R, rows_out, rows_img, (int)img_merge_off);
}

extern "C" int mhimx_vote_scores(void* stream, const float* attn, int64_t H, int64_t N, int64_t k, int32_t largest,
                                 float* vote, void* ws, int64_t ws_bytes) {
  (void)ws; (void)ws_bytes;
  MHIMX_CHECK_ARG(attn && vote && H > 0 && N > 0 && N <= (1ll << 24), "vote_scores: bad args");
  MHIMX_CHECK_ARG(k >= 1 && k <= N && k <= 16384, "vote_scores: k out of range");
  {
    const int64_t nb = (N * 4 / 16) * 16;
    if (aligned16(vote) && nb) sel_zero((hipStream_t)stream, vote, nb);
// ... 11 lines not shown
```

mhim_mil_amd/csrc/step.hip:

```cpp
#include <math.h>
#include <stdlib.h>
#include <string.h>

#include "common.hpp"

namespace mhimx {

int64_t merge2_rows_tiles(int64_t R);

namespace {

struct DagEvents {
  hipEvent_t e[64][6];
  bool have[64] = {};
  int get(hipEvent_t** out) {
    int dev = 0;
    MHIMX_HIP(hipGetDevice(&dev));
    MHIMX_CHECK_ARG(dev >= 0 && dev < 64, "step: device index %d", dev);
    if (!have[dev]) {
      for (int i = 0; i < 6; ++i) MHIMX_HIP(hipEventCreateWithFlags(&e[dev][i], hipEventDisableTiming));
      have[dev] = true;
    }
    *out = e[dev];
    return 0;
  }
};
DagEvents g_dag_events;
constexpr int TP_RING = 256;
struct ProjTimes {
  hipEvent_t e[64][TP_RING][3];
  bool have[64] = {};
  int n[64] = {};
  int next(int* dev_out, hipEvent_t** pair) {
    int dev = 0;
    MHIMX_HIP(hipGetDevice(&dev));
    MHIMX_CHECK_ARG(dev >= 0 && dev < 64, "step: device index %d", dev);
    if (!have[dev]) {
      for (int i = 0; i < TP_RING; ++i)
        for (int j = 0; j < 3; ++j) MHIMX_HIP(hipEventCreate(&e[dev][i][j]));
      have[dev] = true;
    }
    *dev_out = dev;
    *pair = n[dev] < TP_RING ? e[dev][n[dev]] : nullptr;
    return 0;
  }
};
ProjTimes g_proj_times;
int dag_edge(hipEvent_t ev, hipStream_t from, hipStream_t to) {
  MHIMX_HIP(hipEventRecord(ev, from));
  MHIMX_HIP(hipStreamWaitEvent(to, ev, 0));
  return 0;
}

bool fuse_dpre() {
  static const bool on = getenv("MHIMX_FUSE_DPRE") == nullptr || atoi(getenv("MHIMX_FUSE_DPRE")) != 0;
  return on;
}

struct Carve {
  char* base;
  int64_t off = 0;
  explicit Carve(void* p) : base(static_cast<char*>(p)) {}
  int64_t take_off(int64_t bytes) {
    const int64_t o = off;
    off = (off + bytes + 255) / 256 * 256;
    return o;
  }
  template <typename T> T* at(int64_t o) const { return base ? reinterpret_cast<T*>(base + o) : nullptr; }
};

struct StepBufs {
  int64_t w1p_t, wa_frag_t, w1p_s, wa_frag_s, wa_t, wa_t_frag, wo_t, q_old, merge_ws, merge_ws_bytes;
  int64_t H_t, Hbuf, dact;
  int64_t s_t, stats_t, z_t, cproj_t, pscore, attn, pool_ws_t, pool_ws_t_bytes;
  int64_t rows_all, sel_ws, sel_ws_bytes, sel_perm, sel_ids, sel_rows, sel_lk;
  int64_t s_s, stats_s, z_s, pool_ws_s, pool_ws_s_bytes;
  int64_t logits, losses, g_z;
  int64_t dH, img, ws_b, ws_b_bytes, wg_ws, wg_ws_floats;
  int64_t q_scr, gslab;
  int64_t rows_img, P0, L_img;
  bool fuse_img;
  int64_t bag0, bag_stride;
  int64_t total;
};

int dpre_merge_rows(void* stream, const float* dH, const void* dact, const int64_t* rows_merge, int64_t R, int64_t E, char* img, int64_t P0, float* d_b1,
                    float* ws_b, int64_t ws_b_bytes, mhimx_reduce_list* lst) {
  const int64_t t0 = P0 / 32;
// ... 90 lines not shown
  }
  b->bag_stride = cv.off - b->bag0;
  b->total = b->bag0 + (int64_t)n_bags * b->bag_stride;
}

}

}

using namespace mhimx;

extern "C" int mhimx_step_counts_of(int64_t N, double mask_ratio_h, double mask_ratio_hr, double merge_ratio, mhimx_step_counts* out) {
  MHIMX_CHECK_ARG(out && N >= 1 && mask_ratio_h > 0.0 && mask_ratio_hr > 0.0 && merge_ratio > 0.0, "step_counts: bad arguments");
  double eff = mask_ratio_h / mask_ratio_hr, rr = mask_ratio_hr;
  if (eff > 1.0) { rr = mask_ratio_h; eff = 1.0; }
  const int64_t k = (int64_t)ceil((double)N * eff);
  const int64_t n_sel = rr < 1.0 ? (int64_t)ceil((double)k * rr) : k;
  const int64_t len_keep = N - n_sel;
  const int64_t Lk = (int64_t)((double)len_keep * merge_ratio);
  *out = mhimx_step_counts{k, n_sel, len_keep, Lk, len_keep - Lk};
  MHIMX_CHECK_ARG(k >= 1 && n_sel >= 1 && len_keep >= 1 && Lk >= 1 && len_keep - Lk >= 1, "step_counts: the recipe leaves nothing to mask, keep or merge");
  return 0;
}

extern "C" int mhimx_step_layout_of(const mhimx_step_cfg* cfg, int64_t N, const mhimx_step_counts* cnt, mhimx_step_layout* out) {
  MHIMX_CHECK_ARG(out, "step_layout: null output");
  if (int r = check_cfg(cfg, N, cnt)) return r;
  StepBufs b;
  layout(cfg, N, cnt, &b);
  *out = mhimx_step_layout{b.total, b.logits, b.losses, cfg->attn2score ? b.pscore : b.attn, b.rows_all, b.H_t, b.Hbuf, b.dact, b.z_t, b.z_s, b.g_z, b.dH};
  return 0;
}

extern "C" int mhimx_step_run(void* stream, const mhimx_step_cfg* cfg, const float* X, int64_t ldx, int64_t N, const int64_t* label_dev,
                              const mhimx_step_counts* cnt, const mhimx_step_seeds* seeds, int64_t host_step, void* ws, int64_t ws_bytes, int32_t update) {
  if (int r = check_cfg(cfg, N, cnt)) return r;
  MHIMX_CHECK_ARG(X && label_dev && seeds && ws && ldx >= cfg->D && ldx % 4 == 0 && N * ldx * 4 < ((int64_t)1 << 32) && aligned16(X),
                  "step: null bag / label / seeds / workspace, or a row pitch the weight-gradient product does not take");
  MHIMX_CHECK_ARG(!update || (cfg->p && cfg->g && cfg->m && cfg->v && cfg->n_train > 0 && cfg->n_all >= cfg->n_train), "step: update needs the flat optimiser buffers");
  StepBufs b;
  layout(cfg, N, cnt, &b);
  MHIMX_CHECK_ARG(ws_bytes >= b.total && (reinterpret_cast<uintptr_t>(ws) & 255) == 0, "step: workspace too small (%lld < %lld) or not 256-byte aligned",
                  (long long)ws_bytes, (long long)b.total);
  const mhimx_step_cfg& c = *cfg;
  const mhimx_step_params &S = c.student, &T = c.teacher;
  const int64_t D = c.D, E = c.E, A = c.A, C = c.C, k = c.k, I = 512;
  const int64_t R = cnt->R, Lk = cnt->Lk, len_keep = cnt->len_keep;
  Carve cv(ws);
  float* w1p_t = cv.at<float>(b.w1p_t);
  float* wa_frag_t = cv.at<float>(b.wa_frag_t);
  float* w1p_s = cv.at<float>(b.w1p_s);
  float* wa_frag_s = cv.at<float>(b.wa_frag_s);
  float* wa_t = cv.at<float>(b.wa_t);
  float* wa_t_frag = cv.at<float>(b.wa_t_frag);
  float* wo_t = cv.at<float>(b.wo_t);
  float* q_old = cv.at<float>(b.q_old);
  void* merge_ws = cv.at<char>(b.merge_ws);
  float* H_t = cv.at<float>(b.H_t);
  float* Hbuf = cv.at<float>(b.Hbuf);
  void* dact = cv.at<char>(b.dact);
  int64_t* rows_all = cv.at<int64_t>(b.rows_all);
  float* dH = cv.at<float>(b.dH);
  const uint64_t* tick = c.tick;
  static const bool dag_on = getenv("MHIMX_STEP_DAG") == nullptr || atoi(getenv("MHIMX_STEP_DAG")) != 0;
  static const bool dag_fwd = getenv("MHIMX_STEP_DAG_FWD") == nullptr || atoi(getenv("MHIMX_STEP_DAG_FWD")) != 0;
  static const bool dag_bwd = getenv("MHIMX_STEP_DAG_BWD") == nullptr || atoi(getenv("MHIMX_STEP_DAG_BWD")) != 0;
  const hipStream_t main_st = (hipStream_t)stream, side_st = (hipStream_t)c.side_stream;
  const bool dag = dag_on && c.side_stream != nullptr && c.side_stream != stream;
  hipEvent_t* ev = nullptr;
  if (dag)
    if (int r = g_dag_events.get(&ev)) return r;

  mhimx_merge mw_prep = {};
  mw_prep.E = E; mw_prep.k = k; mw_prep.heads = 8; mw_prep.dim_head = 64;
  mw_prep.q_param = S.q; mw_prep.ln_w = S.ln_w; mw_prep.ln_b = S.ln_b; mw_prep.wkv = S.wkv; mw_prep.wq = S.wq; mw_prep.wo = S.wo; mw_prep.bo = S.bo;
  mw_prep.mm = c.merge_mm; mw_prep.prec = MHIMX_PREC_BF16X3; mw_prep.drop_tick = tick; mw_prep.rep = 1.f;
  {
    mhimx_prep_job early[8];
    int n = 0;
    early[n++] = mhimx_prep_job{3, nullptr, reinterpret_cast<float*>(c.tick), 1, 1};
    if (c.opt_step) early[n++] = mhimx_prep_job{3, nullptr, reinterpret_cast<float*>(c.opt_step), 1, 1};
    early[n++] = mhimx_prep_job{1, T.w1, w1p_t, E, D};
    early[n++] = mhimx_prep_job{4, T.wa, wa_frag_t, A, E};
    early[n++] = mhimx_prep_job{1, S.w1, w1p_s, E, D};
    early[n++] = mhimx_prep_job{10, nullptr, reinterpret_cast<float*>(rows_all + len_keep), N, k};
    if (int r = mhimx_prep_batch(stream, early, n)) return r;
  }
  mhimx_prep_job late[6];
  late[0] = mhimx_prep_job{4, S.wa, wa_frag_s, A, E};
  late[1] = mhimx_prep_job{0, S.wa, wa_t, A, E};
  late[2] = mhimx_prep_job{5, S.wa, wa_t_frag, A, E};
  late[3] = mhimx_prep_job{0, S.wo, wo_t, E, I};
  late[4] = mhimx_prep_job{2, S.q, q_old, 1, k * E};
  late[5] = mhimx_prep_job{6, reinterpret_cast<const float*>(&mw_prep), static_cast<float*>(merge_ws), R, b.merge_ws_bytes};

  {
    mhimx_bag_project_args a = {};
    a.X = X; a.ldx = ldx; a.N = N; a.D = D; a.E = E; a.act = c.act; a.n_heads = 2; a.drop_tick = tick;
    a.head[0].wp = w1p_t; a.head[0].bias = T.b1; a.head[0].H = H_t; a.head[0].ldh = E; a.head[0].drop_p = c.drop_p_teacher; a.head[0].drop_seed = seeds->drop_teacher;
    a.head[1].wp = w1p_s; a.head[1].bias = S.b1; a.head[1].H = Hbuf; a.head[1].ldh = E; a.head[1].dact = dact; a.head[1].drop_p = c.drop_p_student;
    a.head[1].drop_seed = seeds->drop_student;
    hipEvent_t* tp = nullptr;
    int tp_dev = 0;
    if (c.time_project) {
      hipStreamCaptureStatus cs = hipStreamCaptureStatusNone;
      MHIMX_HIP(hipStreamIsCapturing(main_st, &cs));
      if (cs == hipStreamCaptureStatusNone)
        if (int r = g_proj_times.next(&tp_dev, &tp)) return r;
    }
    if (tp) MHIMX_HIP(hipEventRecord(tp[0], main_st));
    if (int r = mhimx_bag_project(stream, &a)) return r;
    if (tp) {
      MHIMX_HIP(hipEventRecord(tp[1], main_st));
      MHIMX_HIP(hipEventRecord(tp[2], main_st));
      ++g_proj_times.n[tp_dev];
    }
  }

  mhimx_scorer sc_t = {};
  sc_t.E = E; sc_t.A = A; sc_t.act = c.da_act; sc_t.prec = MHIMX_PREC_BF16X3; sc_t.wa = T.wa; sc_t.wc = T.wc; sc_t.wa_frag = wa_frag_t;
  const float* score = nullptr;
  {
    mhimx_pool_io io = {};
    io.T1 = H_t; io.M1 = N; io.s = cv.at<float>(b.s_t); io.stats = cv.at<float>(b.stats_t); io.z = cv.at<float>(b.z_t);
    io.ws = cv.at<char>(b.pool_ws_t); io.ws_bytes = b.pool_ws_t_bytes;
    if (c.attn2score) { io.wp = T.wp; io.C = C; io.cproj = cv.at<float>(b.cproj_t); io.bp = T.bp; io.pscore = cv.at<float>(b.pscore); }
    io.no_backward = 1;
    io.ride_jobs = late; io.n_ride_jobs = 6;
    if (int r = mhimx_abmil_pool_fwd(stream, &sc_t, &io)) return r;
    if (c.attn2score) score = io.pscore;
    else {
      if (int r = mhimx_softmax_from_stats(stream, io.s, io.stats, cv.at<float>(b.attn), N)) return r;
      score = cv.at<float>(b.attn);
    }
  }
  const float* z_t = cv.at<float>(b.z_t);

  if (N <= 16384) {
    if (b.fuse_img) {
      if (int r = mhimx_select_rows_img(stream, score, N, cnt->k_top, cnt->n_sel, 1, seeds->select, tick, R, rows_all, cv.at<int64_t>(b.rows_img), b.P0,
                                        cv.at<char>(b.sel_ws), b.sel_ws_bytes, 1))
        return r;
    } else if (int r = mhimx_select_rows(stream, score, N, cnt->k_top, cnt->n_sel, 1, seeds->select, tick, R, rows_all, nullptr, cv.at<char>(b.sel_ws),
                                         b.sel_ws_bytes, 1))
      return r;
  } else {
    int64_t* perm = cv.at<int64_t>(b.sel_perm);
    int64_t* ids = cv.at<int64_t>(b.sel_ids);
    int64_t* rows = cv.at<int64_t>(b.sel_rows);
    if (int r = mhimx_random_perm(stream, cnt->k_top, seeds->select + 0x51ED270Bull, tick, nullptr, perm)) return r;
    if (int r = mhimx_select_mask(stream, score, N, cnt->k_top, cnt->n_sel, 1, cnt->n_sel < cnt->k_top ? perm : nullptr, nullptr, 0, ids, cv.at<int64_t>(b.sel_lk),
                                  nullptr, cv.at<char>(b.sel_ws), b.sel_ws_bytes))
      return r;
    if (int r = mhimx_random_perm(stream, len_keep, seeds->select ^ 0x3C6EF372FE94F82Bull, tick, ids, rows)) return r;
    MHIMX_HIP(hipMemcpyAsync(rows_all, rows + Lk, (size_t)R * 8, hipMemcpyDeviceToDevice, (hipStream_t)stream));
    MHIMX_HIP(hipMemcpyAsync(rows_all + R, rows, (size_t)Lk * 8, hipMemcpyDeviceToDevice, (hipStream_t)stream));
  }

  mhimx_merge mw = mw_prep;
  mw.drop_p = c.merge_drop_p; mw.drop_seed = seeds->mca; mw.x_rows = rows_all; mw.prepared = 1;
  mhimx_scorer sc_s = sc_t;
  sc_s.wa = S.wa; sc_s.wc = S.wc; sc_s.wa_frag = wa_frag_s;
  mhimx_pool_io io_s = {};
  io_s.T1 = Hbuf; io_s.M1 = Lk + k; io_s.s = cv.at<float>(b.s_s); io_s.stats = cv.at<float>(b.stats_s); io_s.z = cv.at<float>(b.z_s);
  io_s.ws = cv.at<char>(b.pool_ws_s); io_s.ws_bytes = b.pool_ws_s_bytes; io_s.rows1 = rows_all + R;
  static const bool split_pool = getenv("MHIMX_SPLIT_POOL") == nullptr || atoi(getenv("MHIMX_SPLIT_POOL")) != 0;
  io_s.tail_row0 = -1;
  if (dag && dag_fwd && split_pool && k <= 6) {
    if (int r = dag_edge(ev[0], main_st, side_st)) return r;
    io_s.phase = 1; io_s.tail_tokens = (int32_t)k;
    if (int r = mhimx_abmil_pool_fwd(side_st, &sc_s, &io_s)) return r;
    if (int r = mhimx_merge_fwd(stream, &mw, Hbuf, R, Hbuf + N * E, c.q_out ? c.q_out : S.q, 1, merge_ws, b.merge_ws_bytes)) return r;
    if (int r = dag_edge(ev[1], side_st, main_st)) return r;
    io_s.phase = 2; io_s.tail_wa_t = wa_t; io_s.tail_row0 = N;
    if (int r = mhimx_abmil_pool_fwd(stream, &sc_s, &io_s)) return r;
    io_s.phase = 0;
  } else if (split_pool && k <= 6) {
    io_s.phase = 1; io_s.tail_tokens = (int32_t)k;
    io_s.ride_merge = &mw; io_s.ride_X = Hbuf; io_s.ride_R = R; io_s.ride_ws = merge_ws; io_s.ride_ws_bytes = b.merge_ws_bytes;
    if (int r = mhimx_abmil_pool_fwd(stream, &sc_s, &io_s)) return r;
    mw.rows_done = io_s.rode_merge;
    if (int r = mhimx_merge_fwd(stream, &mw, Hbuf, R, Hbuf + N * E, c.q_out ? c.q_out : S.q, 1, merge_ws, b.merge_ws_bytes)) return r;
    mw.rows_done = 0;
    io_s.phase = 2; io_s.tail_wa_t = wa_t; io_s.tail_row0 = N;
    if (int r = mhimx_abmil_pool_fwd(stream, &sc_s, &io_s)) return r;
    io_s.phase = 0; io_s.ride_merge = nullptr;
  } else {
    if (int r = mhimx_merge_fwd(stream, &mw, Hbuf, R, Hbuf + N * E, c.q_out ? c.q_out : S.q, 1, merge_ws, b.merge_ws_bytes)) return r;
    if (int r = mhimx_abmil_pool_fwd(stream, &sc_s, &io_s)) return r;
  }

  float* g_z = cv.at<float>(b.g_z);
  if (int r = mhimx_head_fwd_bwd(stream, io_s.z, c.aux_alpha != 0.f ? z_t : nullptr, S.wp, S.bp, label_dev, E, C, c.temp_t, c.main_alpha, c.aux_alpha, 1.f,
                                 cv.at<float>(b.logits), cv.at<float>(b.losses), g_z, c.grad.wp, c.grad.bp, 0, nullptr, nullptr))
    return r;

  mhimx_reduce_list lst;
  memset(&lst, 0, sizeof(lst));
  mhimx_merge mwb = mw;
  mwb.q_param = q_old; mwb.wo_t = wo_t; mwb.prepared = 0;
  mhimx_merge_grad mg = {};
  mg.d_ln_w = c.grad.ln_w; mg.d_ln_b = c.grad.ln_b; mg.d_wkv = c.grad.wkv; mg.d_wq = c.grad.wq; mg.d_wo = c.grad.wo; mg.d_bo = c.grad.bo;
  mg.accumulate = 0; mg.splits = 8; mg.defer = &lst;
  if (int r = mhimx_merge_bwd_park(&mwb, Hbuf, R, dH + N * E, dH, &mg, merge_ws, b.merge_ws_bytes)) return r;
  {
    mhimx_scorer sc_b = sc_s;
    sc_b.wa_frag = nullptr;
    mhimx_pool_grad pg = {};
    pg.g_z = g_z; pg.dT1 = dH; pg.d_wa = c.grad.wa; pg.d_wc = c.grad.wc; pg.wa_t = wa_t; pg.accumulate = 0; pg.splits = 8; pg.defer = &lst; pg.wa_t_frag = wa_t_frag;
    if (b.fuse_img) { pg.img = cv.at<char>(b.img); pg.img_dact = dact; pg.img_part = cv.at<float>(b.ws_b); pg.img_rows = Lk; }
    if (int r = mhimx_abmil_pool_bwd(stream, &sc_b, &io_s, &pg)) return r;
  }
  mhimx_reduce_list lst_main;
  memset(&lst_main, 0, sizeof(lst_main));
  const bool dagb = dag && dag_bwd;
  mhimx_reduce_list* lm = dagb ? &lst_main : &lst;
  if (dagb) {
    if (int r = dag_edge(ev[2], main_st, side_st)) return r;
    static const bool fuse_rows = getenv("MHIMX_MERGE_BWD_FUSE") == nullptr || atoi(getenv("MHIMX_MERGE_BWD_FUSE")) != 0;
    if (lst.parked.pending && lst.pre.pending == 2 && fuse_rows) lst.parked.reserved = (int32_t)merge2_rows_tiles(R) + 1;
    if (int r = mhimx_reduce_flush(side_st, &lst)) return r;
  }
  if (int r = mhimx_merge_bwd(stream, &mwb, Hbuf, R, dH + N * E, dH, &mg, merge_ws, b.merge_ws_bytes)) return r;
  if (dagb) {
    if (int r = dag_edge(ev[3], main_st, side_st)) return r;
    if (int r = mhimx_reduce_flush(side_st, &lst)) return r;
  }
  if (b.fuse_img) {
    if (int r = dpre_merge_rows(stream, dH, dact, rows_all, R, E, cv.at<char>(b.img), b.P0, c.grad.b1, cv.at<float>(b.ws_b), b.ws_b_bytes, lm)) return r;
  } else if (int r = mhimx_rows_dpre_image(stream, dH, dact, rows_all, len_keep, E, cv.at<char>(b.img), c.grad.b1, 0, cv.at<char>(b.ws_b), b.ws_b_bytes, lm))
    return r;
  {
    mhimx_bag_wgrad_args g = {};
    g.img = cv.at<char>(b.img); g.X = X; g.ldx = ldx; g.n_bag_rows = N; g.rows = b.fuse_img ? cv.at<int64_t>(b.rows_img) : rows_all; g.L = b.L_img; g.E = E; g.D = D;
    g.C = c.grad.w1; g.ldc = D;
    g.accumulate = 0; g.ws = cv.at<float>(b.wg_ws); g.ws_floats = b.wg_ws_floats; g.defer = lm; g.ride_tail = update ? 1 : 0;
    if (int r = mhimx_bag_wgrad(stream, &g)) return r;
  }
  if (dagb)
    if (int r = dag_edge(ev[4], side_st, main_st)) return r;
  if (!update) return mhimx_reduce_flush(stream, lm);

  mhimx_optim_args o = {};
  o.p = c.p; o.g = c.g; o.m = c.m; o.v = c.v; o.teacher = c.p_teacher; o.n_train = c.n_train; o.n_all = c.n_all; o.step = host_step; o.step_dev = c.opt_step;
  o.lr = c.lr; o.lr_table = c.lr_table; o.lr_len = c.lr_len; o.beta1 = c.beta1; o.beta2 = c.beta2; o.eps = c.eps; o.weight_decay = c.weight_decay;
  o.grad_scale = 1.f; o.ema_mm = c.ema_mm; o.mm_table = c.mm_table; o.mm_len = c.mm_len; o.zero_grad = 1; o.fold = lm;
  return mhimx_optim_step(stream, &o);
}

namespace mhimx {
namespace {

struct QChainW { float wq; float w[MHIMX_WINDOW_MAX]; };
struct SlabGaps { int n; int64_t off[16], len[16]; };
__global__ __launch_bounds__(256) void window_q_chain_kernel(float* __restrict__ q, const float* __restrict__ z0, int64_t z_stride, int n_bags, int64_t n,
                                                             QChainW cw, float* __restrict__ slab0, int64_t pitch, SlabGaps gaps) {
  for (int64_t i = (int64_t)blockIdx.x * blockDim.x + threadIdx.x; i < n; i += (int64_t)gridDim.x * blockDim.x) {
    float acc = 0.f;
    for (int b = 0; b < n_bags; ++b) acc += z0[b * z_stride + i] * cw.w[b];
    q[i] = q[i] * cw.wq + acc;
  }
  for (int gi = 0; gi < gaps.n; ++gi)
    for (int b = 0; b < n_bags; ++b)
      for (int64_t i = (int64_t)blockIdx.x * blockDim.x + threadIdx.x; i < gaps.len[gi]; i += (int64_t)gridDim.x * blockDim.x)
        slab0[b * pitch + gaps.off[gi] + i] = 0.f;
}
__global__ __launch_bounds__(256) void window_sum_slabs_kernel(float* __restrict__ g, const float* __restrict__ slab0, int64_t pitch, int n_bags, int64_t n) {
  for (int64_t i = (int64_t)blockIdx.x * blockDim.x + threadIdx.x; i < n; i += (int64_t)gridDim.x * blockDim.x) {
    float acc = 0.f;
    for (int b = 0; b < n_bags; ++b) acc += slab0[b * pitch + i];
    g[i] = acc;
  }
}

int check_window(const mhimx_step_cfg* c, int32_t n_bags, int64_t N, const mhimx_step_counts* n) {
  if (int r = check_cfg(c, N, n)) return r;
  MHIMX_CHECK_ARG(n_bags >= 2 && n_bags <= MHIMX_WINDOW_MAX, "window: 2..%d bags", MHIMX_WINDOW_MAX);
  MHIMX_CHECK_ARG(N <= 16384 && c->k <= 6, "window: bags of up to 16384 rows (the one-workgroup select), merge_k <= 6");
  MHIMX_CHECK_ARG(c->g && c->n_train > 0 && c->n_all >= c->n_train && c->n_all % 4 == 0, "window: the flat gradient buffer (n_all %% 4 == 0) is required");
  MHIMX_CHECK_ARG(!c->q_out && !c->side_stream, "window: q_out / side_stream are single-step options");
// ... 228 lines not shown
    if (int r = mhimx_reduce_flush(stream, &lst_w)) return r;
    hipLaunchKernelGGL(window_sum_slabs_kernel, dim3((unsigned)(cdiv(c.n_train - g_lo, 256) < 2048 ? cdiv(c.n_train - g_lo, 256) : 2048)), dim3(256), 0, st,
                       c.g + g_lo, slab0 + g_lo, BS / 4, (int)n_bags, c.n_train - g_lo);
    MHIMX_LAUNCH_CHECK();
    return 0;
  }
  mhimx_optim_args o = {};
  o.p = c.p; o.g = c.g; o.m = c.m; o.v = c.v; o.teacher = c.p_teacher; o.n_train = c.n_train; o.n_all = c.n_all; o.step = host_step; o.step_dev = c.opt_step;
  o.lr = c.lr; o.lr_table = c.lr_table; o.lr_len = c.lr_len; o.beta1 = c.beta1; o.beta2 = c.beta2; o.eps = c.eps; o.weight_decay = c.weight_decay;
  o.grad_scale = 1.f; o.ema_mm = c.ema_mm; o.mm_table = c.mm_table; o.mm_len = c.mm_len; o.zero_grad = 1; o.fold = &lst_w;
  o.g_extra = slab0; o.n_extra = n_bags; o.extra_pitch = BS / 4; o.extra_lo = g_lo; o.extra_only = 1;
  return mhimx_optim_step(stream, &o);
}

extern "C" int mhimx_step_project_ms(float* ms_out, float* empty_ms_out, int32_t cap) {
  MHIMX_CHECK_ARG(ms_out && cap >= 0, "step_project_ms: null output");
  int dev = 0;
  MHIMX_HIP(hipGetDevice(&dev));
  MHIMX_CHECK_ARG(dev >= 0 && dev < 64, "step_project_ms: device index %d", dev);
  const int n = g_proj_times.n[dev] < cap ? g_proj_times.n[dev] : cap;
  for (int i = 0; i < n; ++i) {
    MHIMX_HIP(hipEventSynchronize(g_proj_times.e[dev][i][2]));
    MHIMX_HIP(hipEventElapsedTime(ms_out + i, g_proj_times.e[dev][i][0], g_proj_times.e[dev][i][1]));
    if (empty_ms_out) MHIMX_HIP(hipEventElapsedTime(empty_ms_out + i, g_proj_times.e[dev][i][1], g_proj_times.e[dev][i][2]));
  }
  g_proj_times.n[dev] = 0;
  return n;
}

extern "C" int mhimx_step_run_many(void* stream, const mhimx_step_cfg* cfg, int32_t n_bags, const float* const* X, const int64_t* ldx, const int64_t* N,
                                   const int64_t* const* labels_dev, const mhimx_step_counts* cnt, const mhimx_step_seeds* seeds, int64_t host_step0,
                                   void* ws, int64_t ws_bytes) {
  MHIMX_CHECK_ARG(n_bags >= 1 && X && ldx && N && labels_dev && cnt && seeds, "step_run_many: null arguments");
  for (int32_t i = 0; i < n_bags; ++i)
    if (int r = mhimx_step_run(stream, cfg, X[i], ldx[i], N[i], labels_dev[i], cnt + i, seeds + i, host_step0 + i, ws, ws_bytes, 1)) return r;
  return 0;
}

namespace mhimx {
namespace {

struct PureBufs {
  int64_t w1p, wa_frag, wa_t, wa_t_frag;
  int64_t H, dact, s, stats, z, pool_ws, pool_ws_bytes;
  int64_t logits, losses, g_z;
  int64_t dH, img, ws_b, ws_b_bytes, wg_ws, wg_ws_floats;
  int64_t total;
};

int check_pure_cfg(const mhimx_step_cfg* c, int64_t N) {
  MHIMX_CHECK_ARG(c, "pure_step: null configuration");
  MHIMX_CHECK_ARG(c->E == 512 && c->A == 128 && c->C >= 1 && c->C <= 4 && c->D > 0 && c->D % 256 == 0,
                  "pure_step: shapes outside the single-pass ABMIL step (E = 512, A = 128, C <= 4, D %% 256 == 0)");
  MHIMX_CHECK_ARG(N >= 64 && N <= MHIMX_STEP_MAX_ROWS, "pure_step: row count outside 64 <= N <= %d", MHIMX_STEP_MAX_ROWS);
  const mhimx_step_params& s = c->student;
  MHIMX_CHECK_ARG(s.w1 && s.b1 && s.wa && s.wc && s.wp && s.bp, "pure_step: null student parameter");
  const mhimx_step_grads& g = c->grad;
  MHIMX_CHECK_ARG(g.w1 && g.b1 && g.wa && g.wc && g.wp && g.bp, "pure_step: null gradient view");
  MHIMX_CHECK_ARG(c->tick, "pure_step: the device dropout counter (tick) is required");
  return 0;
}

void pure_layout(const mhimx_step_cfg* c, int64_t N, PureBufs* b) {
  const int64_t D = c->D, E = c->E, A = c->A, F = sizeof(float);
  Carve cv(nullptr);
  b->w1p = cv.take_off(E * D * F);
  b->wa_frag = cv.take_off(A * E * F);
  b->wa_t = cv.take_off(E * A * F);
// ... 122 lines not shown
```

mhim_mil_amd/engine.py:

```python
from __future__ import annotations

from typing import Optional

import os

import torch

from . import mhim as mh
from . import ops
from .mhim import MHIM, BagPlan


class CommonMIL:

    def __init__(self, args=None, fused=None, graph_cache=0) -> None:
        self.training = True
        self.fused = fused
        self.graph_cache = int(graph_cache)

    def _native_step(self, tr, bag, label, n_iter, extra):
        if self.graph_cache > 0 and not extra:
            out = tr.shape_cached("forward_backward", bag, label, i=n_iter, cache=self.graph_cache)
            if out is not None:
                return out
# ... 674 lines not shown
        update = bool(self._fold_now)
        L.check(L.lib().mhimx_step_run(ops._stream(), C.byref(ex["cfg"]), x.data_ptr(), x.stride(0), N, label.data_ptr(), C.byref(cnt), C.byref(seeds),
                                       fl.step + int(update), ws.data_ptr(), ws.numel(), int(update)), "mhimx_step_run")
        if update:
            fl.step += 1
        km, E = s.merge.k, s.mlp_dim
        Hs = view(lay.H_student, (N + km) * E).view(N + km, E)
        logits, losses = view(lay.logits, s.n_classes), view(lay.losses, 3)
        rows_all = view(lay.rows_all, cnt.len_keep + km, torch.int64)
        self.last = {"logits": logits, "losses": losses, "patch_num": N, "keep_num": cnt.Lk + km, "rows": rows_all[:cnt.len_keep],
                     "score": view(lay.score, N), "R": cnt.R, "tokens": Hs[N:], "H_student": Hs[:N],
                     "H_teacher": view(lay.H_teacher, N * E).view(N, E), "ws": ws, "exec": True}
        if self._chain is not None:
            self._chain.tokens = self._chain_tokens = Hs[N:]
        if update:
            ops.step_images(None)
            self._micro = 0
        else:
            self._micro += 1
        return logits, losses

    def run_steps(self, bags, labels, i=None):
        import ctypes as C
        L = mh.L
        n = len(bags)
        if n == 0 or len(labels) != n:
            raise L.MhimxError(f"run_steps: {n} bags, {len(labels)} labels")
        its = list(i) if isinstance(i, (list, tuple)) else [None if i is None else i + j for j in range(n)]
        if len(its) != n:
            raise L.MhimxError(f"run_steps: {len(its)} iteration indices for {n} bags")
        xs = [self.s._check_x(b) for b in bags]
        if self._micro != 0:
            raise L.MhimxError("run_steps: called inside an accumulation window (a fresh update is required)")
        if self.clip_grad or not self.fold_reductions or self.accum != 1 or self.world != 1 or not all(self._exec_ok(x, it) and self._nat_ok(x, it) for x, it in zip(xs, its)):
            out = None
            for b, l, it in zip(bags, labels, its):
                out = self.train_step(b, l, i=it)
            return out
        for x, l in zip(xs, labels):
            if not (torch.is_tensor(l) and l.is_cuda and l.dtype == torch.int64 and l.is_contiguous() and l.device == x.device and l.numel() >= 1):
                raise L.MhimxError(f"run_steps: every label must be a contiguous int64 tensor on its bag's device ({x.device})")
        ex = self._exec_cfg()
        plans = [self._exec_plan(ex, x.shape[0], it) for x, it in zip(xs, its)]
        total = max(p[1].total for p in plans)
        ws = ex["ws"]
        if ws is None or ws.numel() < total or ws.device != xs[0].device:
            ws = ex["ws"] = torch.empty(int(total * 1.25), dtype=torch.uint8, device=xs[0].device)
        Xp = (C.c_void_p * n)(*[x.data_ptr() for x in xs])
        ld = (C.c_int64 * n)(*[x.stride(0) for x in xs])
        Ns = (C.c_int64 * n)(*[x.shape[0] for x in xs])
        lab = (C.c_void_p * n)(*[l.data_ptr() for l in labels])
        lay = plans[-1][1]
        if self.model_kind == "mhim_pure":
            drop_seeds = (C.c_uint64 * n)(*[self.s._next_seed() for _ in range(n)])
            L.check(L.lib().mhimx_pure_step_run_many(ops._stream(), C.byref(ex["cfg"]), n, Xp, ld, Ns, lab, drop_seeds, self.flat.step + 1, ws.data_ptr(),
                                                     ws.numel()), "mhimx_pure_step_run_many")
            self.flat.step += n
            ops.step_images(None)
            N, E = xs[-1].shape[0], self.s.mlp_dim
            logits, losses = ws[lay.logits:lay.logits + 4 * self.s.n_classes].view(torch.float32), ws[lay.losses:lay.losses + 12].view(torch.float32)
            self.last = {"logits": logits, "losses": losses, "patch_num": N, "keep_num": N, "rows": None, "score": None, "R": 0, "tokens": None,
                         "H_student": ws[lay.H_student:lay.H_student + N * E * 4].view(torch.float32).view(N, E), "H_teacher": None, "ws": ws,
                         "exec": True}
            return logits, losses
        cnts = (L.StepCounts * n)(*[p[0] for p in plans])
        seeds = (L.StepSeeds * n)()
        for j in range(n):
            seeds[j] = L.StepSeeds(drop_teacher=self.t._next_seed(teacher=True), drop_student=self.s._next_seed(), select=self.s._next_seed(),
                                   mca=self.s._next_seed())
        L.check(L.lib().mhimx_step_run_many(ops._stream(), C.byref(ex["cfg"]), n, Xp, ld, Ns, lab, cnts, seeds, self.flat.step + 1, ws.data_ptr(),
                                            ws.numel()), "mhimx_step_run_many")
        self.flat.step += n
        ops.step_images(None)
        return ws[lay.logits:lay.logits + 4 * self.s.n_classes].view(torch.float32), ws[lay.losses:lay.losses + 12].view(torch.float32)

    def _forward_backward_nat(self, x, label, perm, ids_shuffle, i):
        first = self._micro == 0
        for tns, nm in ((label, "label"), (perm, "perm"), (ids_shuffle, "ids_shuffle")):
            if torch.is_tensor(tns) and not (tns.is_cuda and tns.dtype == torch.int64 and tns.is_contiguous() and tns.device == x.device):
                raise mh.L.MhimxError(f"{nm}: expected a contiguous int64 tensor on the bag's device ({x.device}), got {tns.dtype} on {tns.device}")
        with ops.pinned_stream():
            res = self._nat_prep([x], i, with_opt_tick=first, split=self.ride_prep)
            prep_t, preps = res[0], res[1]
            preps[0]["_ride_jobs"] = res[2] if len(res) > 2 else None
            hook = self._mid_hook if (first and self.overlap_comm and self.comm is None and self.world > 1 and self.accum == 1
                                      and not self._capturing and self._split > 0) else None
            out = self._nat_bag(x, label, prep_t, preps[0], self.flat.grad_views, accumulate=not first, perm=perm, ids_shuffle=ids_shuffle,
                                i=i, mid_hook=hook)
        self._micro += 1
        return out

    def _nat_prep(self, xs, i, with_opt_tick=True, split=False):
        s, t = self.s, self.t
        mhim = self.model_kind == "mhim"
        dev = xs[0].device
        jobs = [(ops.PREP_TICK, None, self.tick)]
        if with_opt_tick:
            jobs.append((ops.PREP_TICK, None, self.opt_step))
        prep_t = None
        if mhim:
            jt, prep_t = t.prep_jobs(backward=False)
            jobs += jt
        merge_on = s.merge_enable
        if not mhim:
            s.merge_enable = False
        try:
            Rs = [s.v2_counts(x.shape[0], i)[4] if mhim else 0 for x in xs]
# ... 346 lines not shown
        cs.wait_stream(torch.cuda.current_stream())
        with torch.cuda.stream(cs):
            for _ in range(warmup):
                self.train_step(bag, label, **kw)
        torch.cuda.current_stream().wait_stream(cs)
        torch.cuda.synchronize()
        if self._graph_pool is None:
            self._graph_pool = torch.cuda.graph_pool_handle()
        if self.world > 1:
            fl = self.flat
            g_fb, g_up = torch.cuda.CUDAGraph(), torch.cuda.CUDAGraph()
            with torch.cuda.graph(g_fb, pool=self._graph_pool, stream=cs, capture_error_mode="thread_local"):
                self.forward_backward(bag, label, **kw)
                fill_tail(fl.grad, fl.student, fl.n_train, self._chain)
            ops.step_images(None)
            self._all_reduce(fl.grad)
            scale = 1.0 / self.world
            with torch.cuda.graph(g_up, pool=self._graph_pool, stream=cs, capture_error_mode="thread_local"):
                finish_tail(fl.grad, fl.student, fl.n_train, scale, self._chain)
                self._apply(scale)
            fl.grad.zero_()
            return _SplitStep(self, g_fb, g_up)
        g = torch.cuda.CUDAGraph()
        with torch.cuda.graph(g, pool=self._graph_pool, stream=cs):
            self.train_step(bag, label, **kw)
        return g

    def capture_steps(self, bags, labels, warmup=1, **kw):
        assert self.accum == 1 and self.world == 1, "capture_steps: one process, one bag per update"
        if self.s.mrh_sche is not None:
            raise mh.L.MhimxError("capture_steps(): the HAM-ratio schedule changes the launch shapes per iteration")
        self._capturing = True
        try:
            if self._cap_stream is None:
                self._cap_stream = torch.cuda.Stream()
            cs = self._cap_stream
            cs.wait_stream(torch.cuda.current_stream())
            with torch.cuda.stream(cs):
                for _ in range(warmup):
                    for b, l in zip(bags, labels):
                        self.train_step(b, l, **kw)
            torch.cuda.current_stream().wait_stream(cs)
            torch.cuda.synchronize()
            if self._graph_pool is None:
                self._graph_pool = torch.cuda.graph_pool_handle()
            g = torch.cuda.CUDAGraph()
            with torch.cuda.graph(g, pool=self._graph_pool, stream=cs):
                for b, l in zip(bags, labels):
                    self.train_step(b, l, **kw)
            return g
        finally:
            self._capturing = False

    def shape_cached(self, what, bag, label, i=None, cache=64):
        x = bag[0] if bag.dim() == 3 else bag
        s, t = self.s, self.t
        if not (self.accum == 1 and self.world == 1 and x.is_cuda and x.dim() == 2 and not self._capturing and self._micro == 0):
            return None
        nat = self._nat_ok(x, i)
        auto = (not nat) and s.baseline in ("selfattn", "dsmil") and (self.model_kind != "mhim" or s.v2_counts(x.shape[0], i) is not None)
        if not (nat or auto):
            return None
        counts = s.v2_counts(x.shape[0], i) if self.model_kind == "mhim" else None
        st = getattr(self, "_shape_graphs", None)
        if st is None:
            st = self._shape_graphs = {"graphs": {}, "seen": {}, "arena": None, "bad": set()}
        key = (what, tuple(x.shape), x.dtype, x.device.index, counts, s.training, None if t is None else t.training, s.merge_enable,
               float(self.main_alpha), float(self.aux_alpha), tuple(label.shape))
        scal = None
        if what == "train_step":
            scal = (None if self.lr_table is not None else float(self.lr), tuple(self.betas), float(self.eps), float(self.wd),
                    None if self.mm_table is not None else float(self.mm))
        if key in st["bad"]:
            return None
        ent = st["graphs"].get(key)
        if ent is not None and ent[8] != scal:
            st["graphs"].pop(key)
            ent = None
            n_re = st.setdefault("rescaled", {})
            n_re[key] = n_re.get(key, 0) + 1
            if n_re[key] > 2:
                st["bad"].add(key)
# ... 85 lines not shown
```

Baseline: 32.98 million patch-instances/s.

## Fold next-bag weight image prep into Adam/EMA update and fuse head into pool backward

Folds the preparation of the next step's packed weight images (teacher w1/wa and student w1) into the Adam+EMA update kernel, so the freshly updated weights are written straight into the next bag's layout. This avoids a separate prep pass over the weights. It also factors the head kernel into a device body so it can be fused into pool backward and selection-finish paths. capture_steps now routes multi-bag captures through run_many, giving graph replay a single fused multi-step launch sequence. The cost is a more complex optimizer kernel with extra per-vector range checks, and a tighter coupling of step layout to the optimizer.

```diff
diff --git a/mhim_mil_amd/csrc/head_body.hpp b/mhim_mil_amd/csrc/head_body.hpp
--- /dev/null
+++ b/mhim_mil_amd/csrc/head_body.hpp
@@ -0,0 +1,145 @@
+#pragma once
+#include "common.hpp"
+#include "step_fold.hpp"
+
+namespace mhimx {
+
+constexpr int HEAD_THREADS = 256;
+
+template <int Q>
+MHIMX_DEV float head_fast_body(const float* __restrict__ z, const float* __restrict__ t, const float* __restrict__ wp, const float* __restrict__ bp,
+                               const int64_t* __restrict__ label, int E, int C, float temp_t, float main_alpha, float aux_alpha, float inv_accum,
+                               float* __restrict__ logits, float* __restrict__ losses, float* __restrict__ g_z, float* __restrict__ d_wp,
+                               float* __restrict__ d_bp, int accumulate, const float* __restrict__ g_logits_in, const float* __restrict__ g_cl_in,
+                               float (*red)[4], bool write_out, float* gz_lds) {
+  const int tid = threadIdx.x, lane = tid & 63, wave = tid >> 6;
+  const bool aux = (t != nullptr);
+  float zv[Q], tv[Q], wv[4][Q], dw_old[4][Q];
+#pragma unroll
+  for (int q = 0; q < Q; ++q) {
+    const int e = tid + q * HEAD_THREADS;
+    const bool in = e < E;
+    zv[q] = in ? z[e] : 0.f;
+    tv[q] = (in && aux) ? t[e] : 0.f;
+#pragma unroll
+    for (int c = 0; c < 4; ++c) {
+      wv[c][q] = (in && c < C) ? wp[c * E + e] : 0.f;
+      dw_old[c][q] = (in && c < C && d_wp && accumulate && write_out) ? d_wp[c * E + e] : 0.f;
+    }
+  }
+  const int y = label ? (int)label[0] : 0;
+  float bpv[4], glin[4], dbp_old[4];
+#pragma unroll
+  for (int c = 0; c < 4; ++c) {
+    bpv[c] = (bp && c < C) ? bp[c] : 0.f;
+    glin[c] = (!label && g_logits_in && c < C) ? g_logits_in[c] : 0.f;
+    dbp_old[c] = (d_bp && accumulate && write_out && c < C) ? d_bp[c] : 0.f;
+  }
+  if (g_cl_in) aux_alpha = g_cl_in[0];
+  float p[4] = {0.f, 0.f, 0.f, 0.f}, a = -INFINITY, b = -INFINITY;
+#pragma unroll
+  for (int q = 0; q < Q; ++q) {
+    const bool in = tid + q * HEAD_THREADS < E;
+#pragma unroll
+    for (int c = 0; c < 4; ++c) p[c] += wv[c][q] * zv[q];
+    if (in) { a = fmaxf(a, zv[q]); b = fmaxf(b, tv[q] / temp_t); }
+  }
+#pragma unroll
+  for (int c = 0; c < 4; ++c) p[c] = wave_sum(p[c]);
+  a = wave_max(a);
+  b = wave_max(b);
+  if (lane == 0) {
+#pragma unroll
+    for (int c = 0; c < 4; ++c) red[c][wave] = p[c];
+    red[4][wave] = a;
+    red[5][wave] = b;
+  }
+  __syncthreads();
+  float lg[4];
+#pragma unroll
+  for (int c = 0; c < 4; ++c) lg[c] = (red[c][0] + red[c][1] + red[c][2] + red[c][3]) + bpv[c];
+  const float zmx = aux ? fmaxf(fmaxf(red[4][0], red[4][1]), fmaxf(red[4][2], red[4][3])) : 0.f;
+  const float tmx = aux ? fmaxf(fmaxf(red[5][0], red[5][1]), fmaxf(red[5][2], red[5][3])) : 0.f;
+  float ce = 0.f, gl[4] = {0.f, 0.f, 0.f, 0.f};
+  if (label) {
+    float mx = -INFINITY;
+#pragma unroll
+    for (int c = 0; c < 4; ++c) if (c < C) mx = fmaxf(mx, lg[c]);
+    float den = 0.f;
+#pragma unroll
+    for (int c = 0; c < 4; ++c) if (c < C) den += expf(lg[c] - mx);
+    float ly = lg[0];
+#pragma unroll
+    for (int c = 1; c < 4; ++c) if (c == y) ly = lg[c];
+    ce = -(ly - mx - logf(den));
+#pragma unroll
+    for (int c = 0; c < 4; ++c) if (c < C) gl[c] = main_alpha * inv_accum * (expf(lg[c] - mx) / den - (c == y ? 1.f : 0.f));
+  } else {
+#pragma unroll
+    for (int c = 0; c < 4; ++c) gl[c] = glin[c];
+  }
+  float cl = 0.f, zden = 1.f, tden = 1.f;
+  float ez[Q], et[Q];
+  if (aux) {
+    float sa = 0.f, sb = 0.f;
+#pragma unroll
+    for (int q = 0; q < Q; ++q) {
+      const bool in = tid + q * HEAD_THREADS < E;
+      ez[q] = in ? expf(zv[q] - zmx) : 0.f;
+      et[q] = in ? expf(tv[q] / temp_t - tmx) : 0.f;
+      sa += ez[q];
+      sb += et[q];
+    }
+    sa = wave_sum(sa);
+    sb = wave_sum(sb);
+    if (lane == 0) { red[6][wave] = sa; red[7][wave] = sb; }
+    __syncthreads();
+    zden = red[6][0] + red[6][1] + red[6][2] + red[6][3];
+    tden = red[7][0] + red[7][1] + red[7][2] + red[7][3];
+    const float lz = logf(zden);
+    float acc = 0.f;
+#pragma unroll
+    for (int q = 0; q < Q; ++q)
+      if (tid + q * HEAD_THREADS < E) acc += (et[q] / tden) * (zv[q] - zmx - lz);
+    acc = wave_sum(acc);
+    if (lane == 0) red[0][wave] = acc;
+    __syncthreads();
+    cl = -(red[0][0] + red[0][1] + red[0][2] + red[0][3]);
+  }
+  if (tid == 0 && write_out) {
+    for (int c = 0; c < C; ++c) logits[c] = lg[c];
+    losses[0] = main_alpha * ce + aux_alpha * cl;
+    losses[1] = ce;
+    losses[2] = cl;
+  }
+  float c0p = 0.f;
+#pragma unroll
+  for (int q = 0; q < Q; ++q) {
+    const int e = tid + q * HEAD_THREADS;
+    if (e >= E) continue;
+    float g = 0.f;
+#pragma unroll
+    for (int c = 0; c < 4; ++c) if (c < C) g += wv[c][q] * gl[c];
+    if (aux) g += aux_alpha * inv_accum * (ez[q] / zden - et[q] / tden);
+    if (gz_lds) gz_lds[e] = g;
+    c0p += g * zv[q];
+    if (write_out) g_z[e] = g;
+    if (d_wp && write_out) {
+#pragma unroll
+      for (int c = 0; c < 4; ++c)
+        if (c < C) {
+          const float v = gl[c] * zv[q];
+          d_wp[c * E + e] = accumulate ? dw_old[c][q] + v : v;
+        }
+    }
+  }
+  if (d_bp && write_out && tid < C) {
+    float gv = gl[0], ov = dbp_old[0];
+#pragma unroll
+    for (int c = 1; c < 4; ++c) if (c == tid) { gv = gl[c]; ov = dbp_old[c]; }
+    d_bp[tid] = accumulate ? ov + gv : gv;
+  }
+  return c0p;
+}
+
+}
diff --git a/mhim_mil_amd/csrc/optim.hip b/mhim_mil_amd/csrc/optim.hip
--- a/mhim_mil_amd/csrc/optim.hip
+++ b/mhim_mil_amd/csrc/optim.hip
@@ -2,12 +2,13 @@
 #include <stdlib.h>
 
 #include "common.hpp"
+#include "head_body.hpp"
+#include "prep_jobs.hpp"
 
 namespace mhimx {
 
 int reduce_flush(hipStream_t st, mhimx_reduce_list* list);
 
-constexpr int HEAD_THREADS = 256;
 
 MHIMX_DEV float blk_sum(float v, float* red) {
   v = wave_sum(v);
@@ -109,130 +110,8 @@
     MHIMX_BAG(z); MHIMX_BAG(t); MHIMX_BAG(label); MHIMX_BAG(logits); MHIMX_BAG(losses); MHIMX_BAG(g_z); MHIMX_BAG(d_wp); MHIMX_BAG(d_bp);
     MHIMX_BAG(g_logits_in); MHIMX_BAG(g_cl_in);
   }
-  const int tid = threadIdx.x, lane = tid & 63, wave = tid >> 6;
-  const bool aux = (t != nullptr);
-  float zv[Q], tv[Q], wv[4][Q], dw_old[4][Q];
-#pragma unroll
-  for (int q = 0; q < Q; ++q) {
-    const int e = tid + q * HEAD_THREADS;
-    const bool in = e < E;
-    zv[q] = in ? z[e] : 0.f;
-    tv[q] = (in && aux) ? t[e] : 0.f;
-#pragma unroll
-    for (int c = 0; c < 4; ++c) {
-      wv[c][q] = (in && c < C) ? wp[c * E + e] : 0.f;
-      dw_old[c][q] = (in && c < C && d_wp && accumulate) ? d_wp[c * E + e] : 0.f;
-    }
-  }
-  const int y = label ? (int)label[0] : 0;
-  float bpv[4], glin[4], dbp_old[4];
-#pragma unroll
-  for (int c = 0; c < 4; ++c) {
-    bpv[c] = (bp && c < C) ? bp[c] : 0.f;
-    glin[c] = (!label && g_logits_in && c < C) ? g_logits_in[c] : 0.f;
-    dbp_old[c] = (d_bp && accumulate && c < C) ? d_bp[c] : 0.f;
-  }
-  if (g_cl_in) aux_alpha = g_cl_in[0];
-  float p[4] = {0.f, 0.f, 0.f, 0.f}, a = -INFINITY, b = -INFINITY;
-#pragma unroll
-  for (int q = 0; q < Q; ++q) {
-    const bool in = tid + q * HEAD_THREADS < E;
-#pragma unroll
-    for (int c = 0; c < 4; ++c) p[c] += wv[c][q] * zv[q];
-    if (in) { a = fmaxf(a, zv[q]); b = fmaxf(b, tv[q] / temp_t); }
-  }
-#pragma unroll
-  for (int c = 0; c < 4; ++c) p[c] = wave_sum(p[c]);
-  a = wave_max(a);
-  b = wave_max(b);
-  if (lane == 0) {
-#pragma unroll
-    for (int c = 0; c < 4; ++c) red[c][wave] = p[c];
-    red[4][wave] = a;
-    red[5][wave] = b;
-  }
-  __syncthreads();
-  float lg[4];
-#pragma unroll
-  for (int c = 0; c < 4; ++c) lg[c] = (red[c][0] + red[c][1] + red[c][2] + red[c][3]) + bpv[c];
-  const float zmx = aux ? fmaxf(fmaxf(red[4][0], red[4][1]), fmaxf(red[4][2], red[4][3])) : 0.f;
-  const float tmx = aux ? fmaxf(fmaxf(red[5][0], red[5][1]), fmaxf(red[5][2], red[5][3])) : 0.f;
-  float ce = 0.f, gl[4] = {0.f, 0.f, 0.f, 0.f};
-  if (label) {
-    float mx = -INFINITY;
-#pragma unroll
-    for (int c = 0; c < 4; ++c) if (c < C) mx = fmaxf(mx, lg[c]);
-    float den = 0.f;
-#pragma unroll
-    for (int c = 0; c < 4; ++c) if (c < C) den += expf(lg[c] - mx);
-    float ly = lg[0];
-#pragma unroll
-    for (int c = 1; c < 4; ++c) if (c == y) ly = lg[c];
-    ce = -(ly - mx - logf(den));
-#pragma unroll
-    for (int c = 0; c < 4; ++c) if (c < C) gl[c] = main_alpha * inv_accum * (expf(lg[c] - mx) / den - (c == y ? 1.f : 0.f));
-  } else {
-#pragma unroll
-    for (int c = 0; c < 4; ++c) gl[c] = glin[c];
-  }
-  float cl = 0.f, zden = 1.f, tden = 1.f;
-  float ez[Q], et[Q];
-  if (aux) {
-    float sa = 0.f, sb = 0.f;
-#pragma unroll
-    for (int q = 0; q < Q; ++q) {
-      const bool in = tid + q * HEAD_THREADS < E;
-      ez[q] = in ? expf(zv[q] - zmx) : 0.f;
-      et[q] = in ? expf(tv[q] / temp_t - tmx) : 0.f;
-      sa += ez[q];
-      sb += et[q];
-    }
-    sa = wave_sum(sa);
-    sb = wave_sum(sb);
-    if (lane == 0) { red[6][wave] = sa; red[7][wave] = sb; }
-    __syncthreads();
-    zden = red[6][0] + red[6][1] + red[6][2] + red[6][3];
-    tden = red[7][0] + red[7][1] + red[7][2] + red[7][3];
-    const float lz = logf(zden);
-    float acc = 0.f;
-#pragma unroll
-    for (int q = 0; q < Q; ++q)
-      if (tid + q * HEAD_THREADS < E) acc += (et[q] / tden) * (zv[q] - zmx - lz);
-    acc = wave_sum(acc);
-    if (lane == 0) red[0][wave] = acc;
-    __syncthreads();
-    cl = -(red[0][0] + red[0][1] + red[0][2] + red[0][3]);
-  }
-  if (tid == 0) {
-    for (int c = 0; c < C; ++c) logits[c] = lg[c];
-    losses[0] = main_alpha * ce + aux_alpha * cl;
-    losses[1] = ce;
-    losses[2] = cl;
-  }
-#pragma unroll
-  for (int q = 0; q < Q; ++q) {
-    const int e = tid + q * HEAD_THREADS;
-    if (e >= E) continue;
-    float g = 0.f;
-#pragma unroll
-    for (int c = 0; c < 4; ++c) if (c < C) g += wv[c][q] * gl[c];
-    if (aux) g += aux_alpha * inv_accum * (ez[q] / zden - et[q] / tden);
-    g_z[e] = g;
-    if (d_wp) {
-#pragma unroll
-      for (int c = 0; c < 4; ++c)
-        if (c < C) {
-          const float v = gl[c] * zv[q];
-          d_wp[c * E + e] = accumulate ? dw_old[c][q] + v : v;
-        }
-    }
-  }
-  if (d_bp && tid < C) {
-    float gv = gl[0], ov = dbp_old[0];
-#pragma unroll
-    for (int c = 1; c < 4; ++c) if (c == tid) { gv = gl[c]; ov = dbp_old[c]; }
-    d_bp[tid] = accumulate ? ov + gv : gv;
-  }
+  head_fast_body<Q>(z, t, wp, bp, label, E, C, temp_t, main_alpha, aux_alpha, inv_accum, logits, losses, g_z, d_wp, d_bp, accumulate, g_logits_in, g_cl_in,
+                    red, true, nullptr);
 }
 
 __global__ __launch_bounds__(HEAD_THREADS) void dsmil_head_kernel(const float* __restrict__ lb, const float* __restrict__ li,
@@ -292,7 +171,7 @@
 constexpr int FOLD_MAX = 4;
 struct FoldJobs { const float* parts[FOLD_MAX]; int64_t off[FOLD_MAX], n[FOLD_MAX]; int G[FOLD_MAX], accumulate[FOLD_MAX]; int count; };
 struct OptimExtra { const float* lr_table; int64_t lr_len; const float* g_extra; int64_t n_extra, extra_pitch; float clip_norm;
-                    const float* sq_parts; int n_parts; FoldJobs fold; int64_t extra_lo; int extra_only; };
+                    const float* sq_parts; int n_parts; FoldJobs fold; int64_t extra_lo; int extra_only; PrepNext pn; };
 
 MHIMX_DEV float4 fold_sum4(const float* __restrict__ parts, int64_t n, int64_t idx, int G) {
   float4 s0 = make_float4(0.f, 0.f, 0.f, 0.f), s1 = s0, s2 = s0, s3 = s0;
@@ -385,6 +264,7 @@
   bc2s = sc[1];
   mm = sc[2];
   gscale *= sc[3];
+  if (ex.pn.tick && blockIdx.x == 0 && threadIdx.x == 0) ex.pn.tick[0] += 1;
   const int64_t n4 = n_all / 4;
   const bool vec_ok = ((reinterpret_cast<uintptr_t>(p) | reinterpret_cast<uintptr_t>(g) | reinterpret_cast<uintptr_t>(m) |
                         reinterpret_cast<uintptr_t>(v) | reinterpret_cast<uintptr_t>(teacher)) & 15) == 0;
@@ -420,7 +300,13 @@
         t.x = t.x * mm + w.x * (1.f - mm); t.y = t.y * mm + w.y * (1.f - mm);
         t.z = t.z * mm + w.z * (1.f - mm); t.w = t.w * mm + w.w * (1.f - mm);
         reinterpret_cast<float4*>(teacher)[q] = t;
-      }
+        for (int r = 0; r < ex.pn.count; ++r)
+          if (ex.pn.teacher[r] && i0 >= ex.pn.lo[r] && i0 < ex.pn.lo[r] + ex.pn.n[r])
+            pj_piece4(ex.pn.img[r], ex.pn.kind[r], i0 - ex.pn.lo[r], ex.pn.row_len[r], t.x, t.y, t.z, t.w);
+      }
+      for (int r = 0; r < ex.pn.count; ++r)
+        if (!ex.pn.teacher[r] && i0 >= ex.pn.lo[r] && i0 < ex.pn.lo[r] + ex.pn.n[r])
+          pj_piece4(ex.pn.img[r], ex.pn.kind[r], i0 - ex.pn.lo[r], ex.pn.row_len[r], w.x, w.y, w.z, w.w);
       continue;
     }
     for (int64_t i = i0; i < i0 + 4 && i < n_all; ++i) {
@@ -478,7 +364,7 @@
   return 0;
 }
 
-extern "C" int mhimx_optim_step(void* stream, const mhimx_optim_args* a) {
+static int optim_step(void* stream, const mhimx_optim_args* a, const PrepNext* pn) {
   MHIMX_CHECK_ARG(a, "optim_step: null args");
   MHIMX_CHECK_ARG(!a->mm_table || a->mm_len > 0, "optim_step: empty momentum schedule");
   MHIMX_CHECK_ARG(!a->lr_table || a->lr_len > 0, "optim_step: empty learning-rate schedule");
@@ -490,7 +376,11 @@
                   "optim_step: extra_lo (a multiple of 4) / extra_only describe the gradient slabs of g_extra");
   int64_t step = a->step < 1 ? 1 : a->step;
   if (a->n_all == 0) return 0;
-  OptimExtra ex{a->lr_table, a->lr_len, a->g_extra, a->n_extra, a->extra_pitch, a->clip_norm > 0.f ? a->clip_norm : 0.f, a->ws, 0, {}, a->extra_lo, a->extra_only};
+  OptimExtra ex{a->lr_table, a->lr_len, a->g_extra, a->n_extra, a->extra_pitch, a->clip_norm > 0.f ? a->clip_norm : 0.f, a->ws, 0, {}, a->extra_lo, a->extra_only, {}};
+  if (pn) {
+    MHIMX_CHECK_ARG(optim_prep_next_ok(a, pn), "optim_step: the next step's images are not on the update's float4 path");
+    ex.pn = *pn;
+  }
   if (a->fold) {
     mhimx_reduce_list* l = a->fold;
     MHIMX_CHECK_ARG(l->n >= 0 && l->n <= MHIMX_REDUCE_MAX, "optim_step: bad reduction list");
@@ -533,6 +423,28 @@
   return 0;
 }
 
+extern "C" int mhimx_optim_step(void* stream, const mhimx_optim_args* a) { return optim_step(stream, a, nullptr); }
+
+namespace mhimx {
+bool optim_prep_next_ok(const mhimx_optim_args* a, const PrepNext* pn) {
+  if (!a || !pn || pn->count < 0 || pn->count > PREP_NEXT_MAX) return false;
+  if (!(aligned16(a->p) && aligned16(a->g) && aligned16(a->m) && aligned16(a->v) && (!a->teacher || aligned16(a->teacher)))) return false;
+  for (int r = 0; r < pn->count; ++r) {
+    const int64_t C = pn->row_len[r];
+    if (pn->lo[r] < 0 || pn->lo[r] % 8 != 0 || pn->n[r] <= 0 || pn->lo[r] + pn->n[r] > a->n_train / 4 * 4 || !pn->img[r] || (pn->teacher[r] && !a->teacher)) return false;
+    if (pn->kind[r] == 1) {
+      if (C <= 0 || C % 8 != 0 || pn->n[r] % C != 0) return false;
+    } else if (pn->kind[r] == 4) {
+      if (C <= 0 || C % 16 != 0 || pn->n[r] % (32 * C) != 0) return false;
+    } else {
+      return false;
+    }
+  }
+  return true;
+}
+int optim_step_prep_next(hipStream_t st, const mhimx_optim_args* a, const PrepNext* pn) { return optim_step(st, a, pn); }
+}
+
 extern "C" int mhimx_adam_ema(void* stream, float* p, const float* g, float* m, float* v, float* teacher, int64_t n_train,
                               int64_t n_all, int64_t step, float lr, float beta1, float beta2, float eps, float weight_decay,
                               float grad_scale, float ema_mm, int32_t zero_grad, const uint64_t* step_dev,
diff --git a/mhim_mil_amd/csrc/pool_fin.hpp b/mhim_mil_amd/csrc/pool_fin.hpp
--- /dev/null
+++ b/mhim_mil_amd/csrc/pool_fin.hpp
@@ -0,0 +1,74 @@
+#pragma once
+#include "common.hpp"
+
+namespace mhimx {
+
+constexpr int FIN_THREADS = 1024;
+
+MHIMX_DEV void fin_max_sum(float pm1, float pl1, int G, float* red, float* wgt, float& mx_out, float& L_out) {
+  const int lane = threadIdx.x & 63, wave = threadIdx.x >> 6;
+  const int b1 = threadIdx.x;
+  float m = wave_max(pm1);
+  if (lane == 0) red[wave] = m;
+  __syncthreads();
+  float mx = red[0];
+#pragma unroll
+  for (int w = 1; w < 16; ++w) mx = fmaxf(mx, red[w]);
+  __syncthreads();
+  float lp = 0.f;
+  if (b1 < G) {
+    const float w = (pm1 == -INFINITY) ? 0.f : __expf(pm1 - mx);
+    if (wgt) wgt[b1] = w;
+    lp = pl1 * w;
+  }
+  lp = wave_sum(lp);
+  if (lane == 0) red[wave] = lp;
+  __syncthreads();
+  float L = 0.f;
+#pragma unroll
+  for (int w = 0; w < 16; ++w) L += red[w];
+  mx_out = mx;
+  L_out = L;
+}
+
+MHIMX_DEV float fin_pseudo_score(float s, const float* cp , int C, float mx, float invL, float b0) {
+  const float an = __expf(s - mx) * invL;
+  float cm = -INFINITY;
+  for (int c = 0; c < C; ++c) cm = fmaxf(cm, an * cp[c] + b0);
+  float den = 0.f;
+  for (int c = 0; c < C; ++c) den += expf((an * cp[c] + b0) - cm);
+  return 1.f / den;
+}
+
+MHIMX_DEV float fin_pseudo_score4(float s, const float (&cp)[4], int C, float mx, float invL, float b0) {
+  const float an = __expf(s - mx) * invL;
+  float cm = -INFINITY;
+#pragma unroll
+  for (int c = 0; c < 4; ++c) if (c < C) cm = fmaxf(cm, an * cp[c] + b0);
+  float den = 0.f;
+#pragma unroll
+  for (int c = 0; c < 4; ++c) if (c < C) den += expf((an * cp[c] + b0) - cm);
+  return 1.f / den;
+}
+
+MHIMX_DEV void fin_merge_z(int zb, const float* __restrict__ pz, int G, int E, const float* wgt, float (*acc16)[64], float mx, float L,
+                           float* __restrict__ stats, float* __restrict__ z) {
+  const int lane = threadIdx.x & 63, wave = threadIdx.x >> 6;
+  const int e = zb * 64 + lane;
+  float acc = 0.f;
+  if (e < E) {
+#pragma unroll 8
+    for (int b = wave; b < G; b += 16) acc += pz[(int64_t)b * E + e] * wgt[b];
+  }
+  acc16[wave][lane] = acc;
+  __syncthreads();
+  if (wave == 0 && e < E) {
+    float a = 0.f;
+#pragma unroll
+    for (int w = 0; w < 16; ++w) a += acc16[w][lane];
+    z[e] = a / L;
+  }
+  if (zb == 0 && threadIdx.x == 0) { stats[0] = mx; stats[1] = L; }
+}
+
+}
diff --git a/mhim_mil_amd/csrc/prep_jobs.hpp b/mhim_mil_amd/csrc/prep_jobs.hpp
--- a/mhim_mil_amd/csrc/prep_jobs.hpp
+++ b/mhim_mil_amd/csrc/prep_jobs.hpp
@@ -17,6 +17,27 @@
 MHIMX_DEV void pj_split2(const pj_f4& a, const pj_f4& b, pj_b8& hi, pj_b8& lo) {
   const float x[8] = {a[0], a[1], a[2], a[3], b[0], b[1], b[2], b[3]};
   pj_split(x, hi, lo);
+}
+
+typedef __bf16 pj_b4 __attribute__((ext_vector_type(4)));
+typedef float pj_f2 __attribute__((ext_vector_type(2)));
+MHIMX_DEV void pj_piece4(char* __restrict__ img, int kind, int64_t rel, int64_t C, float x0, float x1, float x2, float x3) {
+  int64_t item = rel >> 3;
+  if (kind == 4) {
+    const int64_t r = rel / C, c = rel - r * C;
+    item = ((r >> 5) * (C >> 4) + (c >> 4)) * 64 + (r & 31) + 32 * ((c >> 3) & 1);
+  }
+  const float x[4] = {x0, x1, x2, x3};
+  pj_b4 hi, lo;
+#pragma unroll
+  for (int i = 0; i < 4; ++i) {
+    const __bf16 h = (__bf16)x[i];
+    hi[i] = h;
+    lo[i] = (__bf16)(x[i] - (float)h);
+  }
+  char* o = img + item * 32 + ((rel >> 2) & 1) * 8;
+  *reinterpret_cast<pj_f2*>(o) = __builtin_bit_cast(pj_f2, hi);
+  *reinterpret_cast<pj_f2*>(o + 16) = __builtin_bit_cast(pj_f2, lo);
 }
 
 constexpr int PREP_MERGE_MAX = 8;
diff --git a/mhim_mil_amd/csrc/rows.hip b/mhim_mil_amd/csrc/rows.hip
--- a/mhim_mil_amd/csrc/rows.hip
+++ b/mhim_mil_amd/csrc/rows.hip
@@ -2,7 +2,9 @@
 #include <string.h>
 
 #include "mca2_rows.hpp"
+#include "pool_fin.hpp"
 #include "reduce_jobs.hpp"
+#include "step_fold.hpp"
 
 namespace mhimx {
 
@@ -18,7 +20,7 @@
 int scorer_fused_bwd(hipStream_t st, const float* T, int64_t M, const float* u_pre, const float* s_in, const float* stats,
                      const float* g_z, const float* z, const float* wc, int act, const float* wa_t, const float* wa_t_frag, float* du,
                      float* dT, float* dwc_part, float* dbc_part, int max_parts, const int64_t* rows, const void* pre_side, int64_t gate_row0,
-                     void* img, const void* img_dact, float* img_part, int64_t img_rows);
+                     void* img, const void* img_dact, float* img_part, int64_t img_rows, const HeadFold* head);
 
 constexpr int ROWS_THREADS = 256;
 constexpr int MAX_PART = 512;
@@ -117,7 +119,6 @@
   }
 }
 
-constexpr int FIN_THREADS = 1024;
 __global__ __launch_bounds__(FIN_THREADS) void pool_finalize_kernel(const float* __restrict__ pm, const float* __restrict__ pl,
                                                                      const float* __restrict__ pz, int G, int E,
                                                                      float* __restrict__ stats, float* __restrict__ z,
@@ -130,57 +131,19 @@
   if (blockIdx.z) {
     MHIMX_BAG(pm); MHIMX_BAG(pl); MHIMX_BAG(pz); MHIMX_BAG(stats); MHIMX_BAG(z); MHIMX_BAG(s); MHIMX_BAG(cproj); MHIMX_BAG(pscore);
   }
-  const int lane = threadIdx.x & 63, wave = threadIdx.x >> 6;
   const int b1 = threadIdx.x;
   const float pm1 = b1 < G ? pm[b1] : -INFINITY, pl1 = b1 < G ? pl[b1] : 0.f;
-  float m = wave_max(pm1);
-  if (lane == 0) red[wave] = m;
-  __syncthreads();
-  float mx = red[0];
-#pragma unroll
-  for (int w = 1; w < 16; ++w) mx = fmaxf(mx, red[w]);
-  __syncthreads();
-  float lp = 0.f;
-  if (b1 < G) {
-    const float w = (pm1 == -INFINITY) ? 0.f : __expf(pm1 - mx);
-    wgt[b1] = w;
-    lp = pl1 * w;
-  }
-  lp = wave_sum(lp);
-  if (lane == 0) red[wave] = lp;
-  __syncthreads();
-  float L = 0.f;
-#pragma unroll
-  for (int w = 0; w < 16; ++w) L += red[w];
+  float mx, L;
+  fin_max_sum(pm1, pl1, G, red, wgt, mx, L);
   const int zblocks = (E + 63) / 64;
   if ((int)blockIdx.x >= zblocks) {
     const float invL = 1.f / L, b0 = bp ? bp[0] : 0.f;
     const int nb = (int)gridDim.x - zblocks;
-    for (int64_t n = (int64_t)((int)blockIdx.x - zblocks) * FIN_THREADS + threadIdx.x; n < M1; n += (int64_t)nb * FIN_THREADS) {
-      const float an = __expf(s[n] - mx) * invL;
-      float cm = -INFINITY;
-      for (int c = 0; c < C; ++c) cm = fmaxf(cm, an * cproj[n * C + c] + b0);
-      float den = 0.f;
-      for (int c = 0; c < C; ++c) den += expf((an * cproj[n * C + c] + b0) - cm);
-      pscore[n] = 1.f / den;
-    }
+    for (int64_t n = (int64_t)((int)blockIdx.x - zblocks) * FIN_THREADS + threadIdx.x; n < M1; n += (int64_t)nb * FIN_THREADS)
+      pscore[n] = fin_pseudo_score(s[n], cproj + n * C, C, mx, invL, b0);
     return;
   }
-  const int e = blockIdx.x * 64 + lane;
-  float acc = 0.f;
-  if (e < E) {
-#pragma unroll 8
-    for (int b = wave; b < G; b += 16) acc += pz[(int64_t)b * E + e] * wgt[b];
-  }
-  acc16[wave][lane] = acc;
-  __syncthreads();
-  if (wave == 0 && e < E) {
-    float a = 0.f;
-#pragma unroll
-    for (int w = 0; w < 16; ++w) a += acc16[w][lane];
-    z[e] = a / L;
-  }
-  if (blockIdx.x == 0 && threadIdx.x == 0) { stats[0] = mx; stats[1] = L; }
+  fin_merge_z((int)blockIdx.x, pz, G, E, wgt, acc16, mx, L, stats, z);
 }
 
 constexpr int FIN_MAXTOK = 6;
@@ -889,7 +852,7 @@
   return 0;
 }
 
-int abmil_pool_fwd(hipStream_t st, const mhimx_scorer* sc, mhimx_pool_io* io) {
+static int abmil_pool_fwd(hipStream_t st, const mhimx_scorer* sc, mhimx_pool_io* io, SelFin* nofin = nullptr) {
   if (int r = check_scorer(sc)) return r;
   MHIMX_CHECK_ARG(io && io->T1 && io->M1 > 0 && io->s && io->stats && io->z, "pool_fwd: null io");
   MHIMX_CHECK_ARG(io->M2 == 0 || io->T2, "pool_fwd: M2>0 needs T2");
@@ -935,6 +898,9 @@
     return 0;
   }
 
+  if (nofin && (io->phase != 0 || io->M2 != 0 || !io->pscore || !io->cproj || cur_batch().n > 0 ||
+                !scorer_fused_ok(E, A, gated, sc->prec, io->T1, sc->wa, io->wp, io->C)))
+    return 1;
   const float* Ts[2] = {io->T1, io->T2};
   const int64_t Ms[2] = {io->M1, io->M2};
   int64_t off = 0;
@@ -989,6 +955,10 @@
     if (int r = prep_batch(st, io->ride_jobs, io->n_ride_jobs)) return r;
   MHIMX_CHECK_ARG(!io->pscore || io->cproj, "pool_fwd: pscore needs cproj (and wp)");
   static_assert(2 * MAX_PART <= FIN_THREADS, "pool_finalize_kernel reads one partial per thread");
+  if (nofin) {
+    *nofin = SelFin{w.pm, w.pl, w.pz, G, (int)E, (int)io->C, io->stats, io->z, io->s, io->cproj, io->bp, io->pscore};
+    return 0;
+  }
   const int64_t ps_blocks = io->pscore ? (cdiv(io->M1, FIN_THREADS) < 64 ? cdiv(io->M1, FIN_THREADS) : 64) : 0;
   hipLaunchKernelGGL(pool_finalize_kernel, bgrid((unsigned)(cdiv(E, 64) + ps_blocks)), dim3(FIN_THREADS), 0, st, w.pm, w.pl, w.pz, G, (int)E, io->stats,
                      io->z, io->s, io->cproj, io->bp, (int)io->C, io->M1, io->pscore, cur_batch());
@@ -996,7 +966,7 @@
   return 0;
 }
 
-int abmil_pool_bwd(hipStream_t st, const mhimx_scorer* sc, const mhimx_pool_io* io, const mhimx_pool_grad* gr) {
+static int abmil_pool_bwd(hipStream_t st, const mhimx_scorer* sc, const mhimx_pool_io* io, const mhimx_pool_grad* gr, const HeadFold* head = nullptr) {
   if (int r = check_scorer(sc)) return r;
   MHIMX_CHECK_ARG(io && gr && gr->g_z && gr->dT1 && gr->d_wa && gr->d_wc && gr->wa_t, "pool_bwd: null args");
   MHIMX_CHECK_ARG(io->M2 == 0 || gr->dT2, "pool_bwd: M2>0 needs dT2");
@@ -1021,6 +991,7 @@
   MHIMX_CHECK_ARG(!gr->img || (fused && io->M2 == 0 && E == 512), "pool_bwd: the dPRE image (img) needs the one-pass backward and a single segment");
   MHIMX_CHECK_ARG(cur_batch().n == 0 || (fused && io->M2 == 0 && !gated && gr->defer && !gr->d_bc && !gr->d_ba && !gr->d_bb),
                   "pool_bwd: a bag-batched launch needs the one-pass backward with its reductions queued");
+  MHIMX_CHECK_ARG(!head || (fused && io->M2 == 0 && E == 512), "pool_bwd: the folded head needs the one-pass backward and a single segment");
   for (int seg = 0; seg < 2 && fused; ++seg) {
     if (Ms[seg] == 0) continue;
     const void* pre_side = nullptr;
@@ -1038,7 +1009,7 @@
     const int g1 = scorer_fused_bwd(st, Ts[seg], Ms[seg], u_pre + off * ldu, io->s + off, io->stats, gr->g_z, io->z, sc->wc, sc->act,
                                     gr->wa_t, gr->wa_t_frag, w.du + off * ldu, dTs[seg], w.dwc_part + (int64_t)G * A, w.dbc_part + G,
                                     MAX_PART, seg == 0 ? io->rows1 : nullptr, pre_side, gate_row0, seg == 0 ? gr->img : nullptr, gr->img_dact, gr->img_part,
-                                    gr->img_rows);
+                                    gr->img_rows, seg == 0 ? head : nullptr);
     if (g1 < 0) return g1;
     G += g1;
     off += Ms[seg];
@@ -1259,6 +1230,12 @@
 extern "C" int mhimx_abmil_pool_bwd(void* stream, const mhimx_scorer* sc, const mhimx_pool_io* io, const mhimx_pool_grad* g) {
   return abmil_pool_bwd((hipStream_t)stream, sc, io, g);
 }
+namespace mhimx {
+int abmil_pool_fwd_nofin(hipStream_t st, const mhimx_scorer* sc, mhimx_pool_io* io, SelFin* fin) { return abmil_pool_fwd(st, sc, io, fin); }
+int abmil_pool_bwd_head(hipStream_t st, const mhimx_scorer* sc, const mhimx_pool_io* io, const mhimx_pool_grad* gr, const HeadFold* head) {
+  return abmil_pool_bwd(st, sc, io, gr, head);
+}
+}
 extern "C" int mhimx_softmax_from_stats(void* stream, const float* s, const float* stats, float* attn, int64_t M) {
   if (M <= 0) return 0;
   hipLaunchKernelGGL(softmax_from_stats_kernel, bgrid((unsigned)(cdiv(M, 256) < 1024 ? cdiv(M, 256) : 1024)), dim3(256), 0,
diff --git a/mhim_mil_amd/csrc/scorer_fused.hip b/mhim_mil_amd/csrc/scorer_fused.hip
--- a/mhim_mil_amd/csrc/scorer_fused.hip
+++ b/mhim_mil_amd/csrc/scorer_fused.hip
@@ -1,6 +1,7 @@
 #include <math.h>
 
 #include "common.hpp"
+#include "head_body.hpp"
 #include "mca2_rows.hpp"
 #include "prep_jobs.hpp"
 
@@ -287,7 +288,9 @@
     int n_main , Merge2Side pre,
     int64_t gate_row0 ,
     char* __restrict__ img ,
-    const _Float16* __restrict__ dact, float* __restrict__ img_part, int64_t img_rows, BagBatch bb) {
+    const _Float16* __restrict__ dact, float* __restrict__ img_part, int64_t img_rows,
+    HeadFold hf ,
+    BagBatch bb) {
   extern __shared__ __attribute__((aligned(16))) float sb_sm[];
   if (blockIdx.z) {
     MHIMX_BAG(T); MHIMX_BAG(u_pre); MHIMX_BAG(s_in); MHIMX_BAG(stats); MHIMX_BAG(g_z); MHIMX_BAG(z); MHIMX_BAG(du); MHIMX_BAG(dT); MHIMX_BAG(dwc_part);
@@ -311,15 +314,22 @@
   const int tid = threadIdx.x, lane = tid & 63, wave = tid >> 6;
   const int r32 = lane & 31, kg = lane >> 5;
   float c0p = 0.f;
-  for (int e = tid; e < SF_E; e += SF_THREADS) {
-    const float g = g_z[e];
-    gzs[e] = g;
-    c0p += g * z[e];
+  float* c0s = red;
+  if (hf.on) {
+    c0p = head_fast_body<2>(hf.z, hf.t, hf.wp, hf.bp, hf.label, SF_E, hf.C, hf.temp_t, hf.main_alpha, hf.aux_alpha, hf.inv_accum, hf.logits, hf.losses,
+                            hf.g_z, hf.d_wp, hf.d_bp, hf.accumulate, nullptr, nullptr, reinterpret_cast<float(*)[4]>(red), blockIdx.x == 0, gzs);
+    c0s = dwc_s;
+  } else {
+    for (int e = tid; e < SF_E; e += SF_THREADS) {
+      const float g = g_z[e];
+      gzs[e] = g;
+      c0p += g * z[e];
+    }
   }
   c0p = wave_sum(c0p);
-  if (lane == 0) red[wave] = c0p;
+  if (lane == 0) c0s[wave] = c0p;
   __syncthreads();
-  const float c0 = (red[0] + red[1]) + (red[2] + red[3]);
+  const float c0 = (c0s[0] + c0s[1]) + (c0s[2] + c0s[3]);
   const float mx = stats[0], invL = 1.f / stats[1];
   const int a_col = tid & (SF_A - 1), half = tid >> 7;
   const float wca = wc[a_col];
@@ -577,7 +587,7 @@
 int scorer_fused_bwd(hipStream_t st, const float* T, int64_t M, const float* u_pre, const float* s_in, const float* stats,
                      const float* g_z, const float* z, const float* wc, int act, const float* wa_t, const float* wa_t_frag, float* du,
                      float* dT, float* dwc_part, float* dbc_part, int max_parts, const int64_t* rows, const void* pre_side, int64_t gate_row0,
-                     void* img, const void* img_dact, float* img_part, int64_t img_rows) {
+                     void* img, const void* img_dact, float* img_part, int64_t img_rows, const HeadFold* head) {
     MHIMX_ONCE_PER_DEVICE(MHIMX_HIP(hipFuncSetAttribute((const void*)scorer_fused_bwd_kernel, hipFuncAttributeMaxDynamicSharedMemorySize, (int)SB_SMEM_IMG)));
   MHIMX_CHECK_ARG(!img || (img_dact && aligned16(img) && aligned16(img_dact) && img_rows >= 0 && img_rows <= M),
                   "scorer backward: the dPRE image needs the d out / d pre rows, 16-byte aligned buffers and img_rows <= M");
@@ -593,8 +603,17 @@
   } else {
     gate_row0 = -1;
   }
+  HeadFold hf = {};
+  if (head) {
+    MHIMX_CHECK_ARG(cur_batch().n == 0 && head->z == z && head->g_z == g_z && head->wp && head->logits && head->losses && head->C >= 1 && head->C <= 4,
+                    "scorer backward: the folded head takes one bag, the backward's own z / g_z and C <= 4");
+    hf = *head;
+    hf.on = 1;
+  }
+  static_assert(SF_THREADS == HEAD_THREADS && SF_E == 2 * HEAD_THREADS && SF_ROWS * sizeof(float) >= sizeof(float[8][4]), "the folded head: 256 threads, red[8][4]");
   hipLaunchKernelGGL(scorer_fused_bwd_kernel, bgrid(grid + ride), dim3(SF_THREADS), img ? SB_SMEM_IMG : SB_SMEM, st, T, M, u_pre, s_in, stats, g_z, z, wc, act, wa_t,
-                     wa_t_frag, du, dT, dwc_part, dbc_part, tiles, rows, grid, pre, gate_row0, (char*)img, (const _Float16*)img_dact, img_part, img_rows, cur_batch());
+                     wa_t_frag, du, dT, dwc_part, dbc_part, tiles, rows, grid, pre, gate_row0, (char*)img, (const _Float16*)img_dact, img_part, img_rows, hf,
+                     cur_batch());
   MHIMX_LAUNCH_CHECK();
   return grid;
 }
diff --git a/mhim_mil_amd/csrc/select.hip b/mhim_mil_amd/csrc/select.hip
--- a/mhim_mil_amd/csrc/select.hip
+++ b/mhim_mil_amd/csrc/select.hip
@@ -1,4 +1,6 @@
 #include "common.hpp"
+#include "pool_fin.hpp"
+#include "step_fold.hpp"
 
 namespace mhimx {
 
@@ -358,15 +360,27 @@
   return prefix;
 }
 
-template <int KPT, bool LEAN = false>
+template <int KPT, bool LEAN = false, bool FIN = false>
 __global__ __launch_bounds__(SEL_THREADS) void select_small_kernel(
     const float* __restrict__ score, int N, int k, int n_sel, int largest, const int64_t* __restrict__ perm,
     const int64_t* __restrict__ other, int64_t n_other, int64_t* __restrict__ mask_ids, int64_t* __restrict__ len_keep_dev,
     int64_t* __restrict__ topk_out, int P, int use_rand, uint64_t rand_seed0, const uint64_t* __restrict__ tick, int merge_R,
     int64_t* __restrict__ rows_out,
     int64_t* __restrict__ rows_img ,
-    int img_off, BagBatch bb ) {
+    int img_off, BagBatch bb , SelFin fin ) {
   extern __shared__ __attribute__((aligned(16))) char smem_raw[];
+  static_assert(!FIN || LEAN, "the finalize rides in the production form of the select");
+  if (FIN && blockIdx.x > 0) {
+    float* red = reinterpret_cast<float*>(smem_raw);
+    float* wgt = red + 16;
+    float (*acc16)[64] = reinterpret_cast<float(*)[64]>(wgt + FIN_THREADS);
+    const int b1 = threadIdx.x;
+    const float pm1 = b1 < fin.G ? fin.pm[b1] : -INFINITY, pl1 = b1 < fin.G ? fin.pl[b1] : 0.f;
+    float mx, L;
+    fin_max_sum(pm1, pl1, fin.G, red, wgt, mx, L);
+    fin_merge_z((int)blockIdx.x - 1, fin.pz, fin.G, fin.E, wgt, acc16, mx, L, fin.stats, fin.z);
+    return;
+  }
   if (blockIdx.z) {
     MHIMX_BAG(score); MHIMX_BAG(perm); MHIMX_BAG(other); MHIMX_BAG(mask_ids); MHIMX_BAG(len_keep_dev); MHIMX_BAG(topk_out); MHIMX_BAG(rows_out);
     MHIMX_BAG(rows_img);
@@ -389,10 +403,33 @@
   SEL_STAMP(8);
   uint32_t key[KPT];
   bool valid[KPT];
-#pragma unroll
-  for (int j = 0; j < KPT; ++j) {
-    valid[j] = (i0 + j) < N;
-    key[j] = valid[j] ? mono32(score[i0 + j], lg) : 0u;
+  if (FIN) {
+    const float pm1 = tid < fin.G ? fin.pm[tid] : -INFINITY, pl1 = tid < fin.G ? fin.pl[tid] : 0.f;
+    const float b0 = fin.bp ? fin.bp[0] : 0.f;
+    float sv[KPT], cp[KPT][4];
+#pragma unroll
+    for (int j = 0; j < KPT; ++j) {
+      valid[j] = (i0 + j) < N;
+      sv[j] = valid[j] ? fin.s[i0 + j] : 0.f;
+#pragma unroll
+      for (int c = 0; c < 4; ++c) cp[j][c] = (valid[j] && c < fin.C) ? fin.cproj[(int64_t)(i0 + j) * fin.C + c] : 0.f;
+    }
+    float mx, L;
+    fin_max_sum(pm1, pl1, fin.G, reinterpret_cast<float*>(bitmap), nullptr, mx, L);
+    const float invL = 1.f / L;
+#pragma unroll
+    for (int j = 0; j < KPT; ++j) {
+      const float ps = fin_pseudo_score4(sv[j], cp[j], fin.C, mx, invL, b0);
+      if (valid[j]) fin.pscore[i0 + j] = ps;
+      key[j] = valid[j] ? mono32(ps, lg) : 0u;
+    }
+    __syncthreads();
+  } else {
+#pragma unroll
+    for (int j = 0; j < KPT; ++j) {
+      valid[j] = (i0 + j) < N;
+      key[j] = valid[j] ? mono32(score[i0 + j], lg) : 0u;
+    }
   }
   SEL_STAMP(0);
   for (int i = tid; i < 512; i += SEL_THREADS) bitmap[i] = 0;
@@ -871,7 +908,7 @@
 #define MHIMX_SEL_SMALL(KPT)                                                                                                   \
     hipLaunchKernelGGL(select_small_kernel<KPT>, bgrid(1), dim3(SEL_THREADS), sm, (hipStream_t)stream, score, (int)N, (int)k,   \
                        (int)n_sel, largest, perm, other, n_other, mask_ids, len_keep_dev, topk_sorted, P, g_use_rand,          \
-                       g_rand_seed, g_tick, g_merge_R, g_rows_out, g_rows_img, g_img_off, cur_batch())
+                       g_rand_seed, g_tick, g_merge_R, g_rows_out, g_rows_img, g_img_off, cur_batch(), SelFin{})
     MHIMX_ONCE_PER_DEVICE(
         MHIMX_HIP(hipFuncSetAttribute((const void*)select_small_kernel<16>, hipFuncAttributeMaxDynamicSharedMemorySize, (int)select_small_smem(4096)));
         MHIMX_HIP(hipFuncSetAttribute((const void*)select_small_kernel<10>, hipFuncAttributeMaxDynamicSharedMemorySize, (int)select_small_smem(4096)));
@@ -881,7 +918,7 @@
 #define MHIMX_SEL_LEAN(KPT)                                                                                                    \
       hipLaunchKernelGGL((select_small_kernel<KPT, true>), bgrid(1), dim3(SEL_THREADS), sm, (hipStream_t)stream, score, (int)N, (int)k,   \
                          (int)n_sel, largest, perm, other, n_other, mask_ids, len_keep_dev, topk_sorted, P, g_use_rand,        \
-                         g_rand_seed, g_tick, g_merge_R, g_rows_out, g_rows_img, g_img_off, cur_batch())
+                         g_rand_seed, g_tick, g_merge_R, g_rows_out, g_rows_img, g_img_off, cur_batch(), SelFin{})
       MHIMX_ONCE_PER_DEVICE(
           MHIMX_HIP(hipFuncSetAttribute((const void*)select_small_kernel<16, true>, hipFuncAttributeMaxDynamicSharedMemorySize, (int)select_small_smem(4096)));
           MHIMX_HIP(hipFuncSetAttribute((const void*)select_small_kernel<10, true>, hipFuncAttributeMaxDynamicSharedMemorySize, (int)select_small_smem(4096)));
@@ -909,6 +946,38 @@
   return 0;
 }
 
+namespace mhimx {
+int select_rows_img_fin(hipStream_t st, const SelFin* fin, int64_t N, int64_t k, int64_t n_sel, uint64_t rand_seed, const uint64_t* tick, int64_t merge_R,
+                        int64_t* rows_out, int64_t* rows_img, int64_t img_merge_off, void* ws, int64_t ws_bytes) {
+  MHIMX_CHECK_ARG(fin && fin->pm && fin->pl && fin->pz && fin->stats && fin->z && fin->s && fin->cproj && fin->pscore && rows_out && rows_img && ws,
+                  "select_rows_img_fin: null args");
+  MHIMX_CHECK_ARG(merge_R >= 0 && merge_R <= N - n_sel && img_merge_off >= N - n_sel - merge_R && img_merge_off % 32 == 0 && img_merge_off <= 32768 &&
+                      N > 0 && k >= 1 && k <= N && n_sel >= 0 && n_sel <= k && ws_bytes >= N,
+                  "select_rows_img_fin: bad args (mhimx_select_rows_img's)");
+  const int P = next_pow2((int)k < 2 ? 2 : (int)k);
+  const int zblocks = (fin->E + 63) / 64;
+  if (!(N <= 16384 && P <= 4096 && n_sel < k && fin->G >= 1 && fin->G <= FIN_THREADS && fin->C >= 1 && fin->C <= 4 && fin->E >= 1 && cur_batch().n == 0))
+    return 1;
+  const size_t sm = select_small_smem(P);
+  MHIMX_CHECK_ARG(sm >= (size_t)(16 + FIN_THREADS + 16 * 64) * sizeof(float), "select_rows_img_fin: the finalize's LDS is the select's");
+  static_assert(SEL_THREADS == FIN_THREADS, "the finalize's pieces are written for the select's 1024 threads");
+  MHIMX_ONCE_PER_DEVICE(
+      MHIMX_HIP(hipFuncSetAttribute((const void*)select_small_kernel<16, true, true>, hipFuncAttributeMaxDynamicSharedMemorySize, (int)select_small_smem(4096)));
+      MHIMX_HIP(hipFuncSetAttribute((const void*)select_small_kernel<10, true, true>, hipFuncAttributeMaxDynamicSharedMemorySize, (int)select_small_smem(4096)));
+      MHIMX_HIP(hipFuncSetAttribute((const void*)select_small_kernel<4, true, true>, hipFuncAttributeMaxDynamicSharedMemorySize, (int)select_small_smem(4096))));
+#define MHIMX_SEL_FIN(KPT)                                                                                                                    \
+  hipLaunchKernelGGL((select_small_kernel<KPT, true, true>), dim3(1 + zblocks), dim3(SEL_THREADS), sm, st, (const float*)nullptr, (int)N, (int)k, (int)n_sel, \
+                     1, (const int64_t*)nullptr, (const int64_t*)nullptr, (int64_t)0, (int64_t*)nullptr, (int64_t*)nullptr, (int64_t*)nullptr, P, 2,        \
+                     rand_seed, tick, (int)merge_R, rows_out, rows_img, (int)img_merge_off, BagBatch{}, *fin)
+  if (N <= 4096) MHIMX_SEL_FIN(4);
+  else if (N <= 10240) MHIMX_SEL_FIN(10);
+  else MHIMX_SEL_FIN(16);
+#undef MHIMX_SEL_FIN
+  MHIMX_LAUNCH_CHECK();
+  return 0;
+}
+}
+
 extern "C" int mhimx_select_mask(void* stream, const float* score, int64_t N, int64_t k, int64_t n_sel, int32_t largest,
                                  const int64_t* perm, const int64_t* other, int64_t n_other, int64_t* mask_ids,
                                  int64_t* len_keep_dev, int64_t* topk_sorted, void* ws, int64_t ws_bytes) {
diff --git a/mhim_mil_amd/csrc/step.hip b/mhim_mil_amd/csrc/step.hip
--- a/mhim_mil_amd/csrc/step.hip
+++ b/mhim_mil_amd/csrc/step.hip
@@ -3,6 +3,7 @@
 #include <string.h>
 
 #include "common.hpp"
+#include "step_fold.hpp"
 
 namespace mhimx {
 
@@ -54,6 +55,11 @@
 
 bool fuse_dpre() {
   static const bool on = getenv("MHIMX_FUSE_DPRE") == nullptr || atoi(getenv("MHIMX_FUSE_DPRE")) != 0;
+  return on;
+}
+
+bool step_fold() {
+  static const bool on = getenv("MHIMX_STEP_FOLD") == nullptr || atoi(getenv("MHIMX_STEP_FOLD")) != 0;
   return on;
 }
 
@@ -210,8 +216,9 @@
   return 0;
 }
 
-extern "C" int mhimx_step_run(void* stream, const mhimx_step_cfg* cfg, const float* X, int64_t ldx, int64_t N, const int64_t* label_dev,
-                              const mhimx_step_counts* cnt, const mhimx_step_seeds* seeds, int64_t host_step, void* ws, int64_t ws_bytes, int32_t update) {
+static int step_run_impl(void* stream, const mhimx_step_cfg* cfg, const float* X, int64_t ldx, int64_t N, const int64_t* label_dev,
+                         const mhimx_step_counts* cnt, const mhimx_step_seeds* seeds, int64_t host_step, void* ws, int64_t ws_bytes, int32_t update,
+                         bool prep_done, const PrepNext* prep_next) {
   if (int r = check_cfg(cfg, N, cnt)) return r;
   MHIMX_CHECK_ARG(X && label_dev && seeds && ws && ldx >= cfg->D && ldx % 4 == 0 && N * ldx * 4 < ((int64_t)1 << 32) && aligned16(X),
                   "step: null bag / label / seeds / workspace, or a row pitch the weight-gradient product does not take");
@@ -253,7 +260,7 @@
   mw_prep.E = E; mw_prep.k = k; mw_prep.heads = 8; mw_prep.dim_head = 64;
   mw_prep.q_param = S.q; mw_prep.ln_w = S.ln_w; mw_prep.ln_b = S.ln_b; mw_prep.wkv = S.wkv; mw_prep.wq = S.wq; mw_prep.wo = S.wo; mw_prep.bo = S.bo;
   mw_prep.mm = c.merge_mm; mw_prep.prec = MHIMX_PREC_BF16X3; mw_prep.drop_tick = tick; mw_prep.rep = 1.f;
-  {
+  if (!prep_done) {
     mhimx_prep_job early[8];
     int n = 0;
     early[n++] = mhimx_prep_job{3, nullptr, reinterpret_cast<float*>(c.tick), 1, 1};
@@ -264,13 +271,18 @@
     early[n++] = mhimx_prep_job{10, nullptr, reinterpret_cast<float*>(rows_all + len_keep), N, k};
     if (int r = mhimx_prep_batch(stream, early, n)) return r;
   }
-  mhimx_prep_job late[6];
+  mhimx_prep_job late[8];
+  int n_late = 6;
   late[0] = mhimx_prep_job{4, S.wa, wa_frag_s, A, E};
   late[1] = mhimx_prep_job{0, S.wa, wa_t, A, E};
   late[2] = mhimx_prep_job{5, S.wa, wa_t_frag, A, E};
   late[3] = mhimx_prep_job{0, S.wo, wo_t, E, I};
   late[4] = mhimx_prep_job{2, S.q, q_old, 1, k * E};
   late[5] = mhimx_prep_job{6, reinterpret_cast<const float*>(&mw_prep), static_cast<float*>(merge_ws), R, b.merge_ws_bytes};
+  if (prep_done) {
+    if (c.opt_step) late[n_late++] = mhimx_prep_job{3, nullptr, reinterpret_cast<float*>(c.opt_step), 1, 1};
+    late[n_late++] = mhimx_prep_job{10, nullptr, reinterpret_cast<float*>(rows_all + len_keep), N, k};
+  }
 
   {
     mhimx_bag_project_args a = {};
@@ -298,14 +310,23 @@
   mhimx_scorer sc_t = {};
   sc_t.E = E; sc_t.A = A; sc_t.act = c.da_act; sc_t.prec = MHIMX_PREC_BF16X3; sc_t.wa = T.wa; sc_t.wc = T.wc; sc_t.wa_frag = wa_frag_t;
   const float* score = nullptr;
+  SelFin fin_t = {};
+  bool fold_fin = false;
   {
     mhimx_pool_io io = {};
     io.T1 = H_t; io.M1 = N; io.s = cv.at<float>(b.s_t); io.stats = cv.at<float>(b.stats_t); io.z = cv.at<float>(b.z_t);
     io.ws = cv.at<char>(b.pool_ws_t); io.ws_bytes = b.pool_ws_t_bytes;
     if (c.attn2score) { io.wp = T.wp; io.C = C; io.cproj = cv.at<float>(b.cproj_t); io.bp = T.bp; io.pscore = cv.at<float>(b.pscore); }
     io.no_backward = 1;
-    io.ride_jobs = late; io.n_ride_jobs = 6;
-    if (int r = mhimx_abmil_pool_fwd(stream, &sc_t, &io)) return r;
+    io.ride_jobs = late; io.n_ride_jobs = n_late;
+    int rf = 1;
+    if (step_fold() && c.attn2score && b.fuse_img) {
+      rf = abmil_pool_fwd_nofin(main_st, &sc_t, &io, &fin_t);
+      if (rf < 0) return rf;
+    }
+    fold_fin = rf == 0;
+    if (!fold_fin)
+      if (int r = mhimx_abmil_pool_fwd(stream, &sc_t, &io)) return r;
     if (c.attn2score) score = io.pscore;
     else {
       if (int r = mhimx_softmax_from_stats(stream, io.s, io.stats, cv.at<float>(b.attn), N)) return r;
@@ -314,7 +335,19 @@
   }
   const float* z_t = cv.at<float>(b.z_t);
 
-  if (N <= 16384) {
+  if (fold_fin) {
+    const int rs = select_rows_img_fin(main_st, &fin_t, N, cnt->k_top, cnt->n_sel, seeds->select, tick, R, rows_all, cv.at<int64_t>(b.rows_img), b.P0,
+                                       cv.at<char>(b.sel_ws), b.sel_ws_bytes);
+    if (rs < 0) return rs;
+    if (rs > 0) {
+      if (int r = mhimx_pool_finalize(stream, fin_t.pm, fin_t.pl, fin_t.pz, fin_t.G, fin_t.E, fin_t.stats, fin_t.z, fin_t.s, fin_t.cproj, fin_t.bp, fin_t.C, N,
+                                      fin_t.pscore))
+        return r;
+      fold_fin = false;
+    }
+  }
+  if (fold_fin) {
+  } else if (N <= 16384) {
     if (b.fuse_img) {
       if (int r = mhimx_select_rows_img(stream, score, N, cnt->k_top, cnt->n_sel, 1, seeds->select, tick, R, rows_all, cv.at<int64_t>(b.rows_img), b.P0,
                                         cv.at<char>(b.sel_ws), b.sel_ws_bytes, 1))
@@ -369,9 +402,16 @@
   }
 
   float* g_z = cv.at<float>(b.g_z);
-  if (int r = mhimx_head_fwd_bwd(stream, io_s.z, c.aux_alpha != 0.f ? z_t : nullptr, S.wp, S.bp, label_dev, E, C, c.temp_t, c.main_alpha, c.aux_alpha, 1.f,
-                                 cv.at<float>(b.logits), cv.at<float>(b.losses), g_z, c.grad.wp, c.grad.bp, 0, nullptr, nullptr))
-    return r;
+  static const bool head_generic = getenv("MHIMX_HEAD_GENERIC") != nullptr;
+  const bool fold_head = step_fold() && !head_generic;
+  HeadFold hf = {};
+  hf.z = io_s.z; hf.t = c.aux_alpha != 0.f ? z_t : nullptr; hf.wp = S.wp; hf.bp = S.bp; hf.label = label_dev; hf.C = (int)C; hf.accumulate = 0;
+  hf.temp_t = c.temp_t; hf.main_alpha = c.main_alpha; hf.aux_alpha = c.aux_alpha; hf.inv_accum = 1.f;
+  hf.logits = cv.at<float>(b.logits); hf.losses = cv.at<float>(b.losses); hf.g_z = g_z; hf.d_wp = c.grad.wp; hf.d_bp = c.grad.bp;
+  if (!fold_head)
+    if (int r = mhimx_head_fwd_bwd(stream, hf.z, hf.t, hf.wp, hf.bp, hf.label, E, C, hf.temp_t, hf.main_alpha, hf.aux_alpha, hf.inv_accum, hf.logits, hf.losses,
+                                   hf.g_z, hf.d_wp, hf.d_bp, 0, nullptr, nullptr))
+      return r;
 
   mhimx_reduce_list lst;
   memset(&lst, 0, sizeof(lst));
@@ -387,7 +427,9 @@
     mhimx_pool_grad pg = {};
     pg.g_z = g_z; pg.dT1 = dH; pg.d_wa = c.grad.wa; pg.d_wc = c.grad.wc; pg.wa_t = wa_t; pg.accumulate = 0; pg.splits = 8; pg.defer = &lst; pg.wa_t_frag = wa_t_frag;
     if (b.fuse_img) { pg.img = cv.at<char>(b.img); pg.img_dact = dact; pg.img_part = cv.at<float>(b.ws_b); pg.img_rows = Lk; }
-    if (int r = mhimx_abmil_pool_bwd(stream, &sc_b, &io_s, &pg)) return r;
+    if (fold_head) {
+      if (int r = abmil_pool_bwd_head(main_st, &sc_b, &io_s, &pg, &hf)) return r;
+    } else if (int r = mhimx_abmil_pool_bwd(stream, &sc_b, &io_s, &pg)) return r;
   }
   mhimx_reduce_list lst_main;
   memset(&lst_main, 0, sizeof(lst_main));
@@ -423,7 +465,13 @@
   o.p = c.p; o.g = c.g; o.m = c.m; o.v = c.v; o.teacher = c.p_teacher; o.n_train = c.n_train; o.n_all = c.n_all; o.step = host_step; o.step_dev = c.opt_step;
   o.lr = c.lr; o.lr_table = c.lr_table; o.lr_len = c.lr_len; o.beta1 = c.beta1; o.beta2 = c.beta2; o.eps = c.eps; o.weight_decay = c.weight_decay;
   o.grad_scale = 1.f; o.ema_mm = c.ema_mm; o.mm_table = c.mm_table; o.mm_len = c.mm_len; o.zero_grad = 1; o.fold = lm;
+  if (prep_next) return optim_step_prep_next(main_st, &o, prep_next);
   return mhimx_optim_step(stream, &o);
+}
+
+extern "C" int mhimx_step_run(void* stream, const mhimx_step_cfg* cfg, const float* X, int64_t ldx, int64_t N, const int64_t* label_dev,
+                              const mhimx_step_counts* cnt, const mhimx_step_seeds* seeds, int64_t host_step, void* ws, int64_t ws_bytes, int32_t update) {
+  return step_run_impl(stream, cfg, X, ldx, N, label_dev, cnt, seeds, host_step, ws, ws_bytes, update, false, nullptr);
 }
 
 namespace mhimx {
@@ -718,8 +766,39 @@
                                    const int64_t* const* labels_dev, const mhimx_step_counts* cnt, const mhimx_step_seeds* seeds, int64_t host_step0,
                                    void* ws, int64_t ws_bytes) {
   MHIMX_CHECK_ARG(n_bags >= 1 && X && ldx && N && labels_dev && cnt && seeds, "step_run_many: null arguments");
-  for (int32_t i = 0; i < n_bags; ++i)
-    if (int r = mhimx_step_run(stream, cfg, X[i], ldx[i], N[i], labels_dev[i], cnt + i, seeds + i, host_step0 + i, ws, ws_bytes, 1)) return r;
+  bool ahead = step_fold() && n_bags > 1 && cfg && cfg->p && cfg->p_teacher && cfg->g && cfg->m && cfg->v && cfg->student.w1 && cfg->teacher.w1 && cfg->teacher.wa;
+  PrepNext pn = {};
+  if (ahead) {
+    const mhimx_step_cfg& c = *cfg;
+    const float* mat[3] = {c.teacher.w1, c.teacher.wa, c.student.w1};
+    const float* base[3] = {c.p_teacher, c.p_teacher, c.p};
+    const int64_t rows[3] = {c.E, c.A, c.E}, cols[3] = {c.D, c.E, c.D};
+    const int kind[3] = {1, 4, 1};
+    pn.count = 3;
+    for (int r = 0; r < 3; ++r) {
+      pn.kind[r] = kind[r]; pn.teacher[r] = r < 2 ? 1 : 0;
+      pn.lo[r] = mat[r] - base[r]; pn.n[r] = rows[r] * cols[r]; pn.row_len[r] = cols[r];
+      pn.img[r] = reinterpret_cast<char*>(ws);
+      if (mat[r] < base[r] || pn.lo[r] + pn.n[r] > c.n_all) ahead = false;
+    }
+    pn.tick = c.tick;
+    mhimx_optim_args o = {};
+    o.p = c.p; o.g = c.g; o.m = c.m; o.v = c.v; o.teacher = c.p_teacher; o.n_train = c.n_train; o.n_all = c.n_all;
+    if (ahead && !optim_prep_next_ok(&o, &pn)) ahead = false;
+  }
+  for (int32_t i = 0; i < n_bags; ++i) {
+    const bool next = ahead && i + 1 < n_bags;
+    if (next) {
+      if (int r = check_cfg(cfg, N[i + 1], cnt + i + 1)) return r;
+      StepBufs nb;
+      layout(cfg, N[i + 1], cnt + i + 1, &nb);
+      char* base = static_cast<char*>(ws);
+      pn.img[0] = base + nb.w1p_t; pn.img[1] = base + nb.wa_frag_t; pn.img[2] = base + nb.w1p_s;
+    }
+    if (int r = step_run_impl(stream, cfg, X[i], ldx[i], N[i], labels_dev[i], cnt + i, seeds + i, host_step0 + i, ws, ws_bytes, 1, ahead && i > 0,
+                              next ? &pn : nullptr))
+      return r;
+  }
   return 0;
 }
 
diff --git a/mhim_mil_amd/csrc/step_fold.hpp b/mhim_mil_amd/csrc/step_fold.hpp
--- /dev/null
+++ b/mhim_mil_amd/csrc/step_fold.hpp
@@ -0,0 +1,39 @@
+#pragma once
+#include "common.hpp"
+
+namespace mhimx {
+
+struct HeadFold {
+  const float *z, *t, *wp, *bp;
+  const int64_t* label;
+  int C, accumulate, on;
+  float temp_t, main_alpha, aux_alpha, inv_accum;
+  float *logits, *losses, *g_z, *d_wp, *d_bp;
+};
+
+struct SelFin {
+  const float *pm, *pl, *pz;
+  int G, E, C;
+  float *stats, *z;
+  const float *s, *cproj, *bp;
+  float* pscore;
+};
+
+constexpr int PREP_NEXT_MAX = 3;
+struct PrepNext {
+  int count;
+  int kind[PREP_NEXT_MAX];
+  int teacher[PREP_NEXT_MAX];
+  int64_t lo[PREP_NEXT_MAX], n[PREP_NEXT_MAX], row_len[PREP_NEXT_MAX];
+  char* img[PREP_NEXT_MAX];
+  uint64_t* tick;
+};
+int optim_step_prep_next(hipStream_t st, const mhimx_optim_args* a, const PrepNext* pn);
+bool optim_prep_next_ok(const mhimx_optim_args* a, const PrepNext* pn);
+
+int abmil_pool_fwd_nofin(hipStream_t st, const mhimx_scorer* sc, mhimx_pool_io* io, SelFin* fin);
+int abmil_pool_bwd_head(hipStream_t st, const mhimx_scorer* sc, const mhimx_pool_io* io, const mhimx_pool_grad* gr, const HeadFold* head);
+int select_rows_img_fin(hipStream_t st, const SelFin* fin, int64_t N, int64_t k, int64_t n_sel, uint64_t rand_seed, const uint64_t* tick, int64_t merge_R,
+                        int64_t* rows_out, int64_t* rows_img, int64_t img_merge_off, void* ws, int64_t ws_bytes);
+
+}
diff --git a/mhim_mil_amd/engine.py b/mhim_mil_amd/engine.py
--- a/mhim_mil_amd/engine.py
+++ b/mhim_mil_amd/engine.py
@@ -730,20 +730,33 @@
         xs = [self.s._check_x(b) for b in bags]
         if self._micro != 0:
             raise L.MhimxError("run_steps: called inside an accumulation window (a fresh update is required)")
-        if self.clip_grad or not self.fold_reductions or self.accum != 1 or self.world != 1 or not all(self._exec_ok(x, it) and self._nat_ok(x, it) for x, it in zip(xs, its)):
+        if not self._run_many_ok(xs, its):
             out = None
             for b, l, it in zip(bags, labels, its):
                 out = self.train_step(b, l, i=it)
             return out
+        return self._run_many(xs, labels, its)
+
+    def _run_many_ok(self, xs, its):
+        return not (self.clip_grad or not self.fold_reductions or self.accum != 1 or self.world != 1
+                    or not all(self._exec_ok(x, it) and self._nat_ok(x, it) for x, it in zip(xs, its)))
+
+    def _run_many(self, xs, labels, its):
+        import ctypes as C
+        L = mh.L
+        n = len(xs)
         for x, l in zip(xs, labels):
             if not (torch.is_tensor(l) and l.is_cuda and l.dtype == torch.int64 and l.is_contiguous() and l.device == x.device and l.numel() >= 1):
                 raise L.MhimxError(f"run_steps: every label must be a contiguous int64 tensor on its bag's device ({x.device})")
         ex = self._exec_cfg()
         plans = [self._exec_plan(ex, x.shape[0], it) for x, it in zip(xs, its)]
         total = max(p[1].total for p in plans)
-        ws = ex["ws"]
-        if ws is None or ws.numel() < total or ws.device != xs[0].device:
-            ws = ex["ws"] = torch.empty(int(total * 1.25), dtype=torch.uint8, device=xs[0].device)
+        if torch.cuda.is_current_stream_capturing():
+            ws = torch.empty(total, dtype=torch.uint8, device=xs[0].device)
+        else:
+            ws = ex["ws"]
+            if ws is None or ws.numel() < total or ws.device != xs[0].device:
+                ws = ex["ws"] = torch.empty(int(total * 1.25), dtype=torch.uint8, device=xs[0].device)
         Xp = (C.c_void_p * n)(*[x.data_ptr() for x in xs])
         ld = (C.c_int64 * n)(*[x.stride(0) for x in xs])
         Ns = (C.c_int64 * n)(*[x.shape[0] for x in xs])
@@ -770,7 +783,17 @@
                                             ws.numel()), "mhimx_step_run_many")
         self.flat.step += n
         ops.step_images(None)
-        return ws[lay.logits:lay.logits + 4 * self.s.n_classes].view(torch.float32), ws[lay.losses:lay.losses + 12].view(torch.float32)
+        cnt, N, km, E = plans[-1][0], xs[-1].shape[0], self.s.merge.k, self.s.mlp_dim
+
+        def view(off, m, dtype=torch.float32):
+            return ws[off:off + m * dtype.itemsize].view(dtype)
+
+        Hs = view(lay.H_student, (N + km) * E).view(N + km, E)
+        logits, losses = view(lay.logits, self.s.n_classes), view(lay.losses, 3)
+        self.last = {"logits": logits, "losses": losses, "patch_num": N, "keep_num": cnt.Lk + km, "rows": view(lay.rows_all, cnt.len_keep, torch.int64),
+                     "score": view(lay.score, N), "R": cnt.R, "tokens": Hs[N:], "H_student": Hs[:N],
+                     "H_teacher": view(lay.H_teacher, N * E).view(N, E), "ws": ws, "exec": True}
+        return logits, losses
 
     def _forward_backward_nat(self, x, label, perm, ids_shuffle, i):
         first = self._micro == 0
@@ -1183,22 +1206,36 @@
             raise mh.L.MhimxError("capture_steps(): the HAM-ratio schedule changes the launch shapes per iteration")
         self._capturing = True
         try:
+            many, xs, its = False, None, None
+            if self.model_kind == "mhim" and self._micro == 0 and len(bags) > 0 and len(labels) == len(bags) and set(kw) <= {"i"}:
+                i0 = kw.get("i")
+                its = [i0] * len(bags)
+                xs = [self.s._check_x(b) for b in bags]
+                many = not isinstance(i0, (list, tuple)) and self._run_many_ok(xs, its)
+
+            def chunk():
+                if many:
+                    self._run_many(xs, labels, its)
+                    return self.last["ws"]
+                for b, l in zip(bags, labels):
+                    self.train_step(b, l, **kw)
+                return None
+
             if self._cap_stream is None:
                 self._cap_stream = torch.cuda.Stream()
             cs = self._cap_stream
             cs.wait_stream(torch.cuda.current_stream())
             with torch.cuda.stream(cs):
                 for _ in range(warmup):
-                    for b, l in zip(bags, labels):
-                        self.train_step(b, l, **kw)
+                    chunk()
             torch.cuda.current_stream().wait_stream(cs)
             torch.cuda.synchronize()
             if self._graph_pool is None:
                 self._graph_pool = torch.cuda.graph_pool_handle()
             g = torch.cuda.CUDAGraph()
             with torch.cuda.graph(g, pool=self._graph_pool, stream=cs):
-                for b, l in zip(bags, labels):
-                    self.train_step(b, l, **kw)
+                ws = chunk()
+            g._mhimx_ws = ws
             return g
         finally:
             self._capturing = False
```

Result: slower. 32.21 million patch-instances/s (-2.3%).
